# NVlabs/nvbio

Measured on NVIDIA H100. Metric: Mreads/s (150bp) seed+extend, higher is better.
Workload: dtype int32

## Files before the change

### include/nvbio_b200.h

```cpp
#ifndef NVBIO_B200_H
#define NVBIO_B200_H

#include <stddef.h>
#include <stdint.h>

#ifdef __cplusplus
extern "C" {
#endif

#define NVB_VERSION 100

#define NVB_OK              0
#define NVB_E_INVALID      -1
#define NVB_E_TEMP_SIZE    -2
#define NVB_E_CAPACITY     -3
#define NVB_E_UNSUPPORTED  -4

typedef struct nvb_uint2 { uint32_t x, y; } nvb_uint2;

#define NVB_SINK_MIN (-(1 << 30))


typedef struct nvb_fm_index {
    const void*     d_bwt_occ;
    const uint32_t* d_ssa;
    uint32_t        length;
    uint32_t        primary;
    uint32_t        L2[5];
    uint32_t        sa_interval;
    const nvb_uint2* d_ktab;
    uint32_t        ktab_k;
    uint32_t        ktab_located;
    const nvb_uint2* d_rows;
} nvb_fm_index;

typedef struct nvb_string_set {
    const uint32_t* d_words;
    uint32_t        bits;
    uint32_t        big_endian;
    const uint32_t* d_offsets;
    const uint32_t* d_lengths;
    uint32_t        stride;
    uint32_t        length;
} nvb_string_set;

#define NVB_GLOBAL      0
#define NVB_LOCAL       1
#define NVB_SEMI_GLOBAL 2

typedef struct nvb_gotoh_scheme {
    int32_t        match, mismatch;
    int32_t        pattern_gap_open, pattern_gap_ext;
    int32_t        text_gap_open, text_gap_ext;
    const int32_t* d_qual_table;
    int32_t        qual_table_min;
    int32_t        qual_table_max;
} nvb_gotoh_scheme;

int         nvb_version(void);
const char* nvb_error_string(int err);


int nvb_fm_rank(const nvb_fm_index* fmi, const uint32_t* d_k, const uint8_t* d_c, uint32_t n,
                uint32_t* d_out, void* stream);

int nvb_fm_rank4(const nvb_fm_index* fmi, const uint32_t* d_k, uint32_t n, uint32_t* d_out4, void* stream);

int nvb_dict_rank(const void* d_text, uint32_t word_bits, const void* d_occ, uint32_t index_bits, uint32_t K,
                  const void* d_i, const uint8_t* d_c, uint32_t n, void* d_out, void* stream);
int nvb_dict_rank4(const void* d_text, uint32_t word_bits, const void* d_occ, uint32_t index_bits, uint32_t K,
                   const void* d_i, uint32_t n, void* d_out4, void* stream);
int nvb_dict_build_occ(const void* d_text, uint32_t word_bits, uint64_t n_symbols, uint32_t K, uint32_t index_bits, void* d_occ, uint64_t h_counts[4],
                       void* d_temp, size_t* temp_bytes, void* stream);

#define NVB_MATCH_FORWARD_ORDER 1u
#define NVB_MATCH_COMPLEMENT    2u

int nvb_fm_match(const nvb_fm_index* fmi, const nvb_string_set* queries, uint32_t n, uint32_t flags,
                 nvb_uint2* d_ranges, void* stream);

int nvb_fm_match_approx(const nvb_fm_index* fmi, const nvb_string_set* queries, uint32_t n, uint32_t flags,
                        uint32_t exact_len, int find_exact, uint32_t max_out,
                        nvb_uint2* d_ranges, uint32_t* d_counts, uint32_t* d_range_sums, void* stream);

typedef struct nvb_seed_hit {
    uint32_t range_begin;
    uint32_t bits;
} nvb_seed_hit;
#define NVB_MAP_EXACT  0u
#define NVB_MAP_APPROX 1u
#define NVB_MAP_MAX_PUSHES 100u
typedef struct nvb_map_params {
    uint32_t algorithm;
    uint32_t seed_len, seed_freq;
    uint32_t max_hits, max_reseed, rep_seeds, subseed_len, min_read_len;
    uint32_t fw, rc;
} nvb_map_params;
int nvb_map_seeds(const nvb_fm_index* fmi, const nvb_string_set* reads, const uint32_t* d_queue, uint32_t n_queue, uint32_t retry,
                  const nvb_map_params* params, const uint32_t* d_seed_freq,
                  nvb_seed_hit* d_hits, uint32_t* d_counts, uint8_t* d_reseed, uint32_t* d_range_stats, void* stream);

int nvb_fm_locate_init(const nvb_fm_index* fmi, const uint32_t* d_rows, const uint32_t* d_idx, uint32_t n,
                       uint32_t* d_sampled_row, uint32_t* d_steps, void* stream);
int nvb_fm_locate_lookup(const nvb_fm_index* fmi, const uint32_t* d_sampled_row, const uint32_t* d_steps, const uint32_t* d_idx, uint32_t n,
                         uint32_t* d_pos, void* stream);
int nvb_fm_locate_sorted(const nvb_fm_index* fmi, const uint32_t* d_rows, uint32_t n, uint32_t* d_pos,
                         void* d_temp, size_t* temp_bytes, void* stream);

int nvb_fm_locate(const nvb_fm_index* fmi, const uint32_t* d_rows, uint32_t n, uint32_t* d_pos, void* stream);

int nvb_fm_filter_rank(const nvb_fm_index* fmi, const nvb_string_set* queries, uint32_t n, uint32_t flags,
                       nvb_uint2* d_ranges, uint64_t* d_slots, uint64_t* h_n_hits,
                       void* d_temp, size_t* temp_bytes, void* stream);

int nvb_fm_filter_locate(const nvb_fm_index* fmi, const nvb_uint2* d_ranges, const uint64_t* d_slots,
                         uint32_t n_queries, uint64_t begin, uint64_t end, nvb_uint2* d_hits, void* stream);


int nvb_banded_gotoh_score(int band_len, int type, const nvb_gotoh_scheme* scheme,
                           const nvb_string_set* patterns, const uint8_t* d_quals,
                           const nvb_string_set* texts, uint32_t n,
                           int32_t* d_score, nvb_uint2* d_sink,
                           void* d_temp, size_t* temp_bytes, void* stream);

int nvb_banded_gotoh_score_indirect(int band_len, int type, const nvb_gotoh_scheme* scheme,
                           const nvb_string_set* patterns, const uint8_t* d_quals,
                           const nvb_string_set* texts, const uint32_t* d_n, uint32_t n_max,
                           int32_t* d_score, nvb_uint2* d_sink,
                           void* d_temp, size_t* temp_bytes, void* stream);

int nvb_banded_gotoh_score_window(int band_len, int type, const nvb_gotoh_scheme* scheme,
                                  const nvb_string_set* patterns, const uint8_t* d_quals, const nvb_string_set* texts, uint32_t n,
                                  uint32_t window_begin, uint32_t window_end, const int32_t* d_min_score,
                                  int16_t* d_checkpoints, int32_t* d_score, nvb_uint2* d_sink, uint8_t* d_alive, void* stream);

int nvb_banded_gotoh_score_best2(int band_len, int type, const nvb_gotoh_scheme* scheme,
                                 const nvb_string_set* patterns, const uint8_t* d_quals, const nvb_string_set* texts, uint32_t n,
                                 uint32_t distinct_dist, int32_t* d_out6, void* stream);

int nvb_gotoh_score(int type, const nvb_gotoh_scheme* scheme, const nvb_string_set* patterns, const uint8_t* d_quals, const nvb_string_set* texts, uint32_t n,
                    int32_t* d_score, nvb_uint2* d_sink, void* d_temp, size_t* temp_bytes, void* stream);

int nvb_gotoh_score_indirect(int type, const nvb_gotoh_scheme* scheme, const nvb_string_set* patterns, const uint8_t* d_quals, const nvb_string_set* texts,
                             const uint32_t* d_n, uint32_t n_max,
                             int32_t* d_score, nvb_uint2* d_sink, void* d_temp, size_t* temp_bytes, void* stream);

int nvb_gotoh_traceback(int type, const nvb_gotoh_scheme* scheme, const nvb_string_set* patterns, const uint8_t* d_quals, const nvb_string_set* texts, uint32_t n,
                        int32_t* d_score, nvb_uint2* d_sink, nvb_uint2* d_source,
                        uint8_t* d_ops, uint32_t max_ops, uint32_t* d_n_ops,
                        void* d_temp, size_t* temp_bytes, void* stream);

int nvb_banded_gotoh_traceback(int band_len, int type, const nvb_gotoh_scheme* scheme,
                               const nvb_string_set* patterns, const uint8_t* d_quals, const nvb_string_set* texts, uint32_t n,
                               int32_t* d_score, nvb_uint2* d_sink, nvb_uint2* d_source,
                               uint8_t* d_ops, uint32_t max_ops, uint32_t* d_n_ops,
                               void* d_temp, size_t* temp_bytes, void* stream);


int nvb_fm_build_occ(const uint32_t* d_bwt, uint32_t n, void* d_bwt_occ, uint32_t h_L2[5],
                     void* d_temp, size_t* temp_bytes, void* stream);

int nvb_fm_build_bwt(const uint32_t* d_text, uint32_t n, uint32_t* d_bwt, uint32_t* h_primary,
                     uint32_t* d_ssa, uint32_t sa_interval, uint32_t* d_sa,
                     void* d_temp, size_t* temp_bytes, void* stream);

int nvb_fm_build_ktab(const nvb_fm_index* fmi, uint32_t k, nvb_uint2* d_ktab, void* stream);

int nvb_fm_build_ktab_located(const nvb_fm_index* fmi, uint32_t k, void* d_ktab16, void* stream);

int nvb_fm_build_ktab_context(const nvb_fm_index* fmi, uint32_t k, const uint32_t* d_text, void* d_ktab16, void* stream);

int nvb_fm_build_ktab_wide(const nvb_fm_index* fmi, uint32_t k, const uint32_t* d_text, void* d_ktab32, void* stream);

int nvb_fm_build_rows(const nvb_fm_index* fmi, const uint32_t* d_text, nvb_uint2* d_rows, void* stream);

typedef struct nvb_seed_extend_params {
    uint32_t seed_len;
    uint32_t seed_interval;
    uint32_t band_len;
    uint32_t type;
    uint32_t both_strands;
    uint32_t max_seed_hits;
    uint32_t dedup_jobs;
    nvb_gotoh_scheme scheme;
    const uint8_t* d_read_quals;
} nvb_seed_extend_params;

int nvb_seed_extend(const nvb_fm_index* fmi, const uint32_t* d_genome,
                    const nvb_string_set* reads, uint32_t n_reads,
                    const nvb_seed_extend_params* params, uint32_t hit_capacity,
                    int32_t* d_best_score, uint32_t* d_best_pos,
                    uint32_t* d_n_hits, uint32_t* d_hit_read, nvb_uint2* d_hit_window,
                    int32_t* d_hit_score, nvb_uint2* d_hit_sink,
                    void* d_temp, size_t* temp_bytes, void* stream);

typedef struct nvb_best_alignment_out {
    uint8_t*   d_ops;
    uint32_t   max_ops;
    uint32_t*  d_n_ops;
    nvb_uint2* d_begin;
    uint8_t*   d_strand;
} nvb_best_alignment_out;

int nvb_seed_extend_traceback(const nvb_fm_index* fmi, const uint32_t* d_genome,
                    const nvb_string_set* reads, uint32_t n_reads,
                    const nvb_seed_extend_params* params, uint32_t hit_capacity,
                    int32_t* d_best_score, uint32_t* d_best_pos,
                    uint32_t* d_n_hits, uint32_t* d_hit_read, nvb_uint2* d_hit_window,
                    int32_t* d_hit_score, nvb_uint2* d_hit_sink,
                    const nvb_best_alignment_out* best_alignment,
                    void* d_temp, size_t* temp_bytes, void* stream);

typedef struct nvb_mapq_params {
    const int32_t* d_min_score;
    uint32_t       max_read_len;
    int32_t        match_bonus;
} nvb_mapq_params;
typedef struct nvb_mapq_out {
    int32_t*  d_second_score;
    uint32_t* d_second_pos;
    uint8_t*  d_second_strand;
    uint8_t*  d_mapq;
} nvb_mapq_out;

int nvb_seed_extend_mapq(const nvb_fm_index* fmi, const uint32_t* d_genome,
                    const nvb_string_set* reads, uint32_t n_reads,
                    const nvb_seed_extend_params* params, uint32_t hit_capacity,
                    int32_t* d_best_score, uint32_t* d_best_pos,
                    uint32_t* d_n_hits, uint32_t* d_hit_read, nvb_uint2* d_hit_window,
                    int32_t* d_hit_score, nvb_uint2* d_hit_sink,
                    const nvb_best_alignment_out* best_alignment,
                    const nvb_mapq_params* mapq, const nvb_mapq_out* mapq_out,
                    void* d_temp, size_t* temp_bytes, void* stream);

typedef struct nvb_pair_params {
    uint32_t min_frag, max_frag;
    int32_t  min_mate_score;
    uint32_t rescue_capacity;
} nvb_pair_params;
typedef struct nvb_pair_out {
    int32_t*  d_pair_score;
    uint32_t* d_pair_flags;
    int32_t*  d_mate_score;
    uint32_t* d_mate_pos;
    uint8_t*  d_mate_strand;
    uint32_t* d_n_rescue;
} nvb_pair_out;
#define NVB_PAIR_UNPAIRED       0u
#define NVB_PAIR_CONCORDANT     1u
#define NVB_PAIR_RESCUED_MATE1  2u
#define NVB_PAIR_RESCUED_MATE2  4u

int nvb_seed_extend_paired(const nvb_fm_index* fmi, const uint32_t* d_genome,
                    const nvb_string_set* reads, uint32_t n_pairs,
                    const nvb_seed_extend_params* params, uint32_t hit_capacity,
                    const nvb_pair_params* pair_params, const nvb_pair_out* out,
                    uint32_t* d_n_hits, void* d_temp, size_t* temp_bytes, void* stream);

typedef struct nvb_pair_mapq_out {
    int32_t*  d_second_pair_score;
    uint32_t* d_second_mate_pos;
    uint8_t*  d_second_mate_strand;
    int32_t*  d_mate_second_score;
    uint8_t*  d_mate_mapq;
} nvb_pair_mapq_out;

int nvb_seed_extend_paired_mapq(const nvb_fm_index* fmi, const uint32_t* d_genome,
                    const nvb_string_set* reads, uint32_t n_pairs,
                    const nvb_seed_extend_params* params, uint32_t hit_capacity,
                    const nvb_pair_params* pair_params, const nvb_pair_out* out,
                    const nvb_mapq_params* mapq, const nvb_pair_mapq_out* mapq_out,
                    uint32_t* d_n_hits, void* d_temp, size_t* temp_bytes, void* stream);

int nvb_seed_extend_paired_traceback(const nvb_fm_index* fmi, const uint32_t* d_genome,
                    const nvb_string_set* reads, uint32_t n_pairs,
                    const nvb_seed_extend_params* params, uint32_t hit_capacity,
                    const nvb_pair_params* pair_params, const nvb_pair_out* out,
                    const nvb_best_alignment_out* mate_alignment,
                    const nvb_mapq_params* mapq, const nvb_pair_mapq_out* mapq_out,
                    uint32_t* d_n_hits, void* d_temp, size_t* temp_bytes, void* stream);

typedef struct nvb_finish_out {
    uint32_t* d_cigar;
    uint32_t  max_cigar;
    uint32_t* d_n_cigar;
    char*     d_md;
    uint32_t  max_md;
    uint32_t* d_md_len;
    uint32_t* d_edits;
} nvb_finish_out;

int nvb_finish_alignments(const uint32_t* d_genome, uint32_t genome_len,
                          const nvb_string_set* reads, uint32_t n,
                          const nvb_best_alignment_out* alignment,
                          const nvb_finish_out* out, void* stream);

typedef struct nvb_bam_in {
    nvb_string_set   reads;
    const uint8_t*   d_read_quals;
    const uint32_t*  d_n_ops;
    const nvb_uint2* d_begin;
    const uint8_t*   d_strand;
    nvb_finish_out   finish;
    const int32_t*   d_score;
    const uint8_t*   d_mapq;
    const int32_t*   d_second_score;
    const uint32_t*  d_pair_flags;
    const uint32_t*  d_contig_begin;
    uint32_t         n_contigs;
    const char*      d_names;
    const uint32_t*  d_name_offsets;
} nvb_bam_in;
typedef struct nvb_bam_out {
    uint8_t*  d_records;
    uint64_t  capacity;
    uint64_t* d_offsets;
    uint32_t* d_counts;
} nvb_bam_out;

int nvb_bam_records(const nvb_bam_in* in, uint32_t n, const nvb_bam_out* out, void* d_temp, size_t* temp_bytes, void* stream);

typedef struct nvb_bgzf_out {
    uint8_t*  d_out;
    uint64_t  capacity;
    uint64_t* d_block_offsets;
} nvb_bgzf_out;

// ... 32 lines not shown
```

### include/nvbio_b200_debug.h

```cpp
#ifndef NVBIO_B200_DEBUG_H
#define NVBIO_B200_DEBUG_H
#include <stdint.h>
#ifdef __cplusplus
extern "C" {
#endif

void nvb_debug_force_gotoh_path(int path);
int nvb_debug_gotoh_last_route(int* packed, uint32_t* n_int32);
void nvb_debug_full_minb(int minb);
void nvb_debug_full_warp(int mode);
void nvb_debug_full_traceback_warp(int on);
void nvb_debug_pair_format(int on);
void nvb_debug_pair_rows2(int on);
void nvb_debug_traceback_fast(int on);
void nvb_debug_pair_extra_smem(int bytes);

void nvb_debug_pipeline_path(int path);

void nvb_debug_seed_split(int on);

void nvb_debug_perfect_shortcut(int on);
int nvb_debug_dp_jobs(uint32_t* n);

int nvb_debug_mapq_eval(const int32_t* d_best, const uint8_t* d_has_second, const int32_t* d_second, const uint32_t* d_len,
                        const int32_t* d_match_bonus, const int32_t* d_min_score, uint32_t n, uint8_t* d_mapq, void* stream);

void nvb_debug_bgzf_grid(uint32_t ctas);

#ifdef __cplusplus
}
#endif
#endif
```

### nvbio_b200/_lib.py

```python
import ctypes as C
import os

_HERE = os.path.dirname(os.path.abspath(__file__))
LIB_PATH = os.environ.get("NVBIO_B200_LIB") or os.path.join(_HERE, "libnvbio_b200.so")

EXPORTS = [
    "nvb_version", "nvb_error_string",
    "nvb_fm_rank", "nvb_fm_rank4", "nvb_fm_match", "nvb_fm_match_approx", "nvb_fm_locate", "nvb_fm_filter_rank", "nvb_fm_filter_locate",
    "nvb_banded_gotoh_score", "nvb_banded_gotoh_score_indirect", "nvb_banded_gotoh_traceback", "nvb_gotoh_score", "nvb_gotoh_score_indirect", "nvb_banded_gotoh_score_window", "nvb_banded_gotoh_score_best2", "nvb_gotoh_traceback", "nvb_seed_extend_paired",
    "nvb_fm_build_occ", "nvb_fm_build_bwt", "nvb_fm_build_ktab", "nvb_fm_build_ktab_located", "nvb_fm_build_ktab_context", "nvb_fm_build_ktab_wide", "nvb_fm_build_rows", "nvb_seed_extend", "nvb_seed_extend_traceback", "nvb_seed_extend_mapq", "nvb_seed_extend_paired_mapq", "nvb_seed_extend_paired_traceback",
    "nvb_seed_extend_stage_ms",
    "nvb_dict_rank", "nvb_dict_rank4", "nvb_dict_build_occ",
    "nvb_map_seeds", "nvb_fm_locate_init", "nvb_fm_locate_lookup", "nvb_fm_locate_sorted",
    "nvb_pipeline_create", "nvb_pipeline_submit", "nvb_pipeline_wait", "nvb_pipeline_traffic", "nvb_pipeline_destroy",
    "nvb_finish_alignments", "nvb_bam_records", "nvb_bgzf_compress",
]
DEBUG_EXPORTS = [
    "nvb_debug_gotoh_last_route", "nvb_debug_force_gotoh_path", "nvb_debug_full_minb", "nvb_debug_full_warp", "nvb_debug_full_traceback_warp",
    "nvb_debug_pair_format", "nvb_debug_pair_rows2", "nvb_debug_traceback_fast", "nvb_debug_pair_extra_smem",
    "nvb_debug_pipeline_path", "nvb_debug_seed_split", "nvb_debug_perfect_shortcut", "nvb_debug_dp_jobs", "nvb_debug_mapq_eval",
    "nvb_debug_bgzf_grid",
]


class NvbError(RuntimeError):
    pass


class FmIndexStruct(C.Structure):
    _fields_ = [("d_bwt_occ", C.c_void_p), ("d_ssa", C.c_void_p), ("length", C.c_uint32),
                ("primary", C.c_uint32), ("L2", C.c_uint32 * 5), ("sa_interval", C.c_uint32),
                ("d_ktab", C.c_void_p), ("ktab_k", C.c_uint32), ("ktab_located", C.c_uint32), ("d_rows", C.c_void_p)]


class StringSetStruct(C.Structure):
    _fields_ = [("d_words", C.c_void_p), ("bits", C.c_uint32), ("big_endian", C.c_uint32),
                ("d_offsets", C.c_void_p), ("d_lengths", C.c_void_p), ("stride", C.c_uint32),
                ("length", C.c_uint32)]


class GotohSchemeStruct(C.Structure):
    _fields_ = [("match", C.c_int32), ("mismatch", C.c_int32), ("pattern_gap_open", C.c_int32),
                ("pattern_gap_ext", C.c_int32), ("text_gap_open", C.c_int32), ("text_gap_ext", C.c_int32),
                ("d_qual_table", C.c_void_p), ("qual_table_min", C.c_int32), ("qual_table_max", C.c_int32)]


class SeedExtendParamsStruct(C.Structure):
    _fields_ = [("seed_len", C.c_uint32), ("seed_interval", C.c_uint32), ("band_len", C.c_uint32),
                ("type", C.c_uint32), ("both_strands", C.c_uint32), ("max_seed_hits", C.c_uint32),
                ("dedup_jobs", C.c_uint32), ("scheme", GotohSchemeStruct), ("d_read_quals", C.c_void_p)]


class BestAlignmentOutStruct(C.Structure):
    _fields_ = [("d_ops", C.c_void_p), ("max_ops", C.c_uint32), ("d_n_ops", C.c_void_p), ("d_begin", C.c_void_p),
                ("d_strand", C.c_void_p)]


class FinishOutStruct(C.Structure):
    _fields_ = [("d_cigar", C.c_void_p), ("max_cigar", C.c_uint32), ("d_n_cigar", C.c_void_p), ("d_md", C.c_void_p), ("max_md", C.c_uint32),
                ("d_md_len", C.c_void_p), ("d_edits", C.c_void_p)]


class BamInStruct(C.Structure):
    _fields_ = [("reads", StringSetStruct), ("d_read_quals", C.c_void_p), ("d_n_ops", C.c_void_p), ("d_begin", C.c_void_p),
                ("d_strand", C.c_void_p), ("finish", FinishOutStruct), ("d_score", C.c_void_p), ("d_mapq", C.c_void_p),
                ("d_second_score", C.c_void_p), ("d_pair_flags", C.c_void_p), ("d_contig_begin", C.c_void_p), ("n_contigs", C.c_uint32),
                ("d_names", C.c_void_p), ("d_name_offsets", C.c_void_p)]


class BamOutStruct(C.Structure):
    _fields_ = [("d_records", C.c_void_p), ("capacity", C.c_uint64), ("d_offsets", C.c_void_p), ("d_counts", C.c_void_p)]


class BgzfOutStruct(C.Structure):
    _fields_ = [("d_out", C.c_void_p), ("capacity", C.c_uint64), ("d_block_offsets", C.c_void_p)]


class MapqParamsStruct(C.Structure):
    _fields_ = [("d_min_score", C.c_void_p), ("max_read_len", C.c_uint32), ("match_bonus", C.c_int32)]


class MapqOutStruct(C.Structure):
    _fields_ = [("d_second_score", C.c_void_p), ("d_second_pos", C.c_void_p), ("d_second_strand", C.c_void_p), ("d_mapq", C.c_void_p)]


class PairParamsStruct(C.Structure):
    _fields_ = [("min_frag", C.c_uint32), ("max_frag", C.c_uint32), ("min_mate_score", C.c_int32), ("rescue_capacity", C.c_uint32)]


class PairOutStruct(C.Structure):
    _fields_ = [("d_pair_score", C.c_void_p), ("d_pair_flags", C.c_void_p), ("d_mate_score", C.c_void_p), ("d_mate_pos", C.c_void_p),
                ("d_mate_strand", C.c_void_p), ("d_n_rescue", C.c_void_p)]


class PairMapqOutStruct(C.Structure):
    _fields_ = [("d_second_pair_score", C.c_void_p), ("d_second_mate_pos", C.c_void_p), ("d_second_mate_strand", C.c_void_p),
                ("d_mate_second_score", C.c_void_p), ("d_mate_mapq", C.c_void_p)]


class PipelineResultStruct(C.Structure):
    _fields_ = [("best_score", C.c_void_p), ("best_pos", C.c_void_p), ("n_hits", C.c_void_p), ("pair_score", C.c_void_p),
                ("pair_flags", C.c_void_p), ("mate_score", C.c_void_p), ("mate_pos", C.c_void_p), ("mate_strand", C.c_void_p),
                ("n_rescue", C.c_void_p), ("device_ms", C.c_float)]


_lib = None


def lib():
    global _lib
    if _lib is None:
        if not os.path.exists(LIB_PATH):
            raise NvbError("nvbio_b200: %s is missing -- run `python -m nvbio_b200.build` "
                           "(there is no CPU fallback)" % LIB_PATH)
        _lib = C.CDLL(LIB_PATH)
        _lib.nvb_error_string.restype = C.c_char_p
        _lib.nvb_pipeline_destroy.restype = None
        _lib.nvb_pipeline_traffic.restype = None
        for name in EXPORTS + DEBUG_EXPORTS:
            getattr(_lib, name)
    return _lib


def check(err, what=""):
    if err != 0:
        msg = lib().nvb_error_string(C.c_int(err)).decode()
        raise NvbError("%s failed: %s (%d)" % (what or "nvbio_b200 call", msg, err))
```

### nvbio_b200/csrc/fm_core.cuh

```cuda
#pragma once
#include "common.cuh"

namespace nvb {

struct __align__(32) FmBlock {
    uint32_t bwt[4];
    uint32_t occ[4];
};

struct FmIndex {
    const FmBlock*  blocks;
    const uint32_t* ssa;
    const uint2*    ktab;
    uint32_t n, primary;
    uint32_t L2[5];
    uint32_t sa_mask, sa_shift;
    uint32_t ktab_k;
    uint32_t ktab_located;
    const uint2*    rows;
    uint32_t ktab_wide;
    __host__ __device__ __forceinline__ uint32_t l2(uint32_t c) const {
        return (c == 0) ? L2[0] : (c == 1) ? L2[1] : (c == 2) ? L2[2] : L2[3];
    }
    __host__ __device__ __forceinline__ uint32_t count(uint32_t c) const {
        return (c == 0) ? L2[1] - L2[0] : (c == 1) ? L2[2] - L2[1] : (c == 2) ? L2[3] - L2[2] : L2[4] - L2[3];
    }
};

static inline bool valid_fmindex(const nvb_fm_index* f) {
    if (!f || !f->d_bwt_occ) return false;
    const uint32_t I = f->sa_interval;
    if (I != 0 && (I & (I - 1)) != 0) return false;
    if (f->d_ktab && (f->ktab_k < 1 || f->ktab_k > 16 || f->ktab_located > 5u)) return false;
    if (f->d_ktab && f->ktab_located >= 3u && (f->sa_interval != 1u || !f->d_ssa)) return false;
    if (f->d_ktab && f->ktab_located >= 4u && ((uintptr_t)f->d_ktab & 31u)) return false;
    if (f->d_ktab && (f->ktab_located == 3u || f->ktab_located == 5u) && !f->d_rows) return false;
    return true;
}
static inline FmIndex make_fmindex(const nvb_fm_index* f) {
    FmIndex r;
    r.blocks = (const FmBlock*)f->d_bwt_occ; r.ssa = f->d_ssa; r.n = f->length; r.primary = f->primary;
    for (int i = 0; i < 5; ++i) r.L2[i] = f->L2[i];
    const uint32_t I = f->sa_interval ? f->sa_interval : 16u;
    r.sa_shift = 0; while ((1u << r.sa_shift) < I) ++r.sa_shift;
    r.sa_mask = (1u << r.sa_shift) - 1u;
    r.ktab = (const uint2*)f->d_ktab; r.ktab_k = f->d_ktab ? f->ktab_k : 0u;
    const bool with_rows = f->d_ktab && (f->ktab_located == 3u || f->ktab_located == 5u);
    r.ktab_wide = (f->d_ktab && f->ktab_located >= 4u) ? 1u : 0u;
    r.ktab_located = f->d_ktab ? (f->ktab_located >= 2u ? 2u : f->ktab_located) : 0u;
    r.rows = with_rows ? (const uint2*)f->d_rows : nullptr;
    return r;
}

__host__ __device__ __forceinline__ uint32_t nvb_popc(uint32_t x) {
#ifdef __CUDA_ARCH__
    return __popc(x);
#else
    return (uint32_t)__builtin_popcount(x);
#endif
}

#ifndef NVB_FM_LD_QUAL
#define NVB_FM_LD_QUAL ".L2::64B"
#endif
__host__ __device__ __forceinline__ FmBlock load_block(const FmBlock* __restrict__ blocks, uint32_t k) {
#ifdef __CUDA_ARCH__
    FmBlock b;
    asm volatile("ld.global.nc" NVB_FM_LD_QUAL ".v4.u32 {%0,%1,%2,%3}, [%8];\n\t"
                 "ld.global.nc" NVB_FM_LD_QUAL ".v4.u32 {%4,%5,%6,%7}, [%8+16];"
                 : "=r"(b.bwt[0]), "=r"(b.bwt[1]), "=r"(b.bwt[2]), "=r"(b.bwt[3]),
                   "=r"(b.occ[0]), "=r"(b.occ[1]), "=r"(b.occ[2]), "=r"(b.occ[3])
                 : "l"(blocks + k));
    return b;
#else
    return blocks[k];
#endif
}
__host__ __device__ __forceinline__ void load_block_if(FmBlock& b, const FmBlock* __restrict__ blocks, uint32_t k, bool pred) {
#ifdef __CUDA_ARCH__
    asm volatile("{\n\t.reg .pred p;\n\tsetp.ne.u32 p, %9, 0;\n\t"
                 "@p ld.global.nc" NVB_FM_LD_QUAL ".v4.u32 {%0,%1,%2,%3}, [%8];\n\t"
                 "@p ld.global.nc" NVB_FM_LD_QUAL ".v4.u32 {%4,%5,%6,%7}, [%8+16];\n\t}"
                 : "+r"(b.bwt[0]), "+r"(b.bwt[1]), "+r"(b.bwt[2]), "+r"(b.bwt[3]),
                   "+r"(b.occ[0]), "+r"(b.occ[1]), "+r"(b.occ[2]), "+r"(b.occ[3])
                 : "l"(blocks + k), "r"((uint32_t)pred));
#else
    if (pred) b = blocks[k];
#endif
}

__host__ __device__ __forceinline__ uint32_t gather_u32(const uint32_t* __restrict__ p) {
#ifdef __CUDA_ARCH__
    uint32_t v; asm volatile("ld.global.nc" NVB_FM_LD_QUAL ".u32 %0, [%1];" : "=r"(v) : "l"(p)); return v;
#else
    return *p;
#endif
}
__host__ __device__ __forceinline__ uint4 gather_u4(const uint4* __restrict__ p) {
#ifdef __CUDA_ARCH__
    uint4 v; asm volatile("ld.global.nc" NVB_FM_LD_QUAL ".v4.u32 {%0,%1,%2,%3}, [%4];" : "=r"(v.x), "=r"(v.y), "=r"(v.z), "=r"(v.w) : "l"(p)); return v;
#else
    return *p;
#endif
}
__host__ __device__ __forceinline__ uint2 gather_u2(const uint2* __restrict__ p) {
#ifdef __CUDA_ARCH__
    uint2 v; asm volatile("ld.global.nc" NVB_FM_LD_QUAL ".v2.u32 {%0,%1}, [%2];" : "=r"(v.x), "=r"(v.y) : "l"(p)); return v;
#else
    return *p;
#endif
}

__host__ __device__ __forceinline__ uint32_t eq_flags(uint32_t w, uint32_t pat) {
    const uint32_t d = w ^ pat;
    return ~(d | (d >> 1)) & 0x55555555u;
}

__host__ __device__ __forceinline__ uint32_t block_rank(const FmBlock& b, uint32_t r, uint32_t c) {
    const uint32_t pat = c * 0x55555555u;
    const uint32_t nsym = r + 1;
    uint32_t cnt = (c == 0) ? b.occ[0] : (c == 1) ? b.occ[1] : (c == 2) ? b.occ[2] : b.occ[3];
#pragma unroll
    for (int q = 0; q < 4; ++q) {
        const int keep = (int)nsym - 16 * q;
        const uint32_t k = keep < 0 ? 0u : (keep > 16 ? 16u : (uint32_t)keep);
        const uint32_t mask = (uint32_t)(0xFFFFFFFF00000000ull >> (2 * k));
        cnt += nvb_popc(eq_flags(b.bwt[q], pat) & mask);
    }
    return cnt;
}

__host__ __device__ __forceinline__ uint32_t block_symbol(const FmBlock& b, uint32_t r) {
    const uint32_t q = r >> 4;
    const uint32_t w = (q == 0) ? b.bwt[0] : (q == 1) ? b.bwt[1] : (q == 2) ? b.bwt[2] : b.bwt[3];
    return (w >> (30u - 2u * (r & 15u))) & 3u;
}

template <typename W> struct dict_word {};
template <> struct dict_word<uint32_t> { static constexpr uint32_t SPW = 16u; static constexpr uint32_t ODD = 0x55555555u; };
template <> struct dict_word<uint64_t> { static constexpr uint32_t SPW = 32u; static constexpr uint64_t ODD = 0x5555555555555555ull; };

template <typename W>
__host__ __device__ __forceinline__ uint32_t word_rank(W w, uint32_t c, uint32_t keep) {
    constexpr uint32_t SPW = dict_word<W>::SPW;
    const W pat = (W)c * dict_word<W>::ODD;
    const W d = w ^ pat;
    W flags = ~(d | (d >> 1)) & dict_word<W>::ODD;
    flags &= (W)(~(W)0) << (2u * (SPW - keep));
#ifdef __CUDA_ARCH__
    return sizeof(W) == 8 ? (uint32_t)__popcll((unsigned long long)flags) : (uint32_t)__popc((uint32_t)flags);
#else
    return (uint32_t)__builtin_popcountll((unsigned long long)flags);
#endif
}
template <typename W, typename I>
__host__ __device__ __forceinline__ I dict_rank(const W* __restrict__ text, const I* __restrict__ occ, uint32_t K, I i, uint32_t c) {
    if (i == (I)(~(I)0)) return (I)0;
    constexpr uint32_t SPW = dict_word<W>::SPW;
    const uint64_t k = (uint64_t)(i / K);
    const uint32_t r = (uint32_t)(i - (I)(k * K));
    const uint32_t m = r / SPW;
    const uint64_t off = k * (K / SPW);
    I out = occ[k * 4u + c];
    for (uint32_t j = 0; j < m; ++j) out += word_rank<W>(text[off + j], c, SPW);
    return out + word_rank<W>(text[off + m], c, (r % SPW) + 1u);
}

__host__ __device__ __forceinline__ uint32_t fm_rank1(const FmIndex& f, uint32_t k, uint32_t c) {
    if (k == 0xFFFFFFFFu) return 0u;
    if (k == f.n) return f.count(c);
    if (k >= f.primary) --k;
    const FmBlock b = load_block(f.blocks, k >> 6);
    return block_rank(b, k & 63u, c);
}

__host__ __device__ __forceinline__ uint4 fm_rank4(const FmIndex& f, uint32_t k) {
    if (k == 0xFFFFFFFFu) return make_uint4(0u, 0u, 0u, 0u);
    if (k == f.n) return make_uint4(f.count(0), f.count(1), f.count(2), f.count(3));
    if (k >= f.primary) --k;
    const FmBlock b = load_block(f.blocks, k >> 6);
    const uint32_t r = k & 63u;
    return make_uint4(block_rank(b, r, 0), block_rank(b, r, 1), block_rank(b, r, 2), block_rank(b, r, 3));
}

__host__ __device__ __forceinline__ void fm_rank2(const FmIndex& f, uint32_t kx, uint32_t ky, uint32_t c,
                                                  uint32_t& rx, uint32_t& ry) {
    const bool need_x = (kx != 0xFFFFFFFFu) && (kx != f.n);
    const bool need_y = (ky != 0xFFFFFFFFu) && (ky != f.n);
    const uint32_t cnt = f.count(c);
    rx = (kx == f.n) ? cnt : 0u;
    ry = (ky == f.n) ? cnt : 0u;
    const uint32_t ax = kx - (kx >= f.primary ? 1u : 0u);
    const uint32_t ay = ky - (ky >= f.primary ? 1u : 0u);
    if (need_x || need_y) {
        const uint32_t bx = ax >> 6, by = ay >> 6;
        FmBlock b0 = load_block(f.blocks, need_x ? bx : by);
        FmBlock b1 = b0;
        load_block_if(b1, f.blocks, by, need_x && need_y && bx != by);
        const uint32_t tx = block_rank(b0, ax & 63u, c);
        const uint32_t ty = block_rank(b1, ay & 63u, c);
        if (need_x) rx = tx;
        if (need_y) ry = ty;
    }
// ... 165 lines not shown

constexpr uint32_t FM_ROWS_MAX = 8;

enum { FM_EMPTY = 0, FM_RANGE = 1, FM_LOCATED = 2, FM_DEFERRED = 3 };
enum { FM_WHOLE = 0, FM_DEFER = 1, FM_RESUME = 2 };
template <int BITS, bool BE, int MODE = FM_WHOLE>
__host__ __device__ __forceinline__ uint32_t fm_match_locate_one(const FmIndex& f, const uint32_t* __restrict__ genome,
                                                                 const uint32_t* __restrict__ words, uint32_t off, uint32_t len,
                                                                 uint32_t& ox, uint32_t& oy)
{
    SymReader<BITS, BE> rd(words);
    uint32_t x = 0, y = f.n, s = 0;
    uint32_t known_pos = 0u, known_pos2 = 0u, ctx2 = 0u; bool have_pos = false, have_two = false, two_ctx = false;
    uint4 e = make_uint4(0u, 0u, 0u, 0u), e_hi = make_uint4(0u, 0u, 0u, 0u);
    if (MODE == FM_RESUME) { x = ox; y = oy; s = (x == 0u && y == f.n) ? 0u : f.ktab_k; }
    if (MODE != FM_RESUME && f.ktab_k && len >= f.ktab_k) {
        uint32_t u = 0; bool has_n = false;
        if (BITS == 2 && BE) {
            u = be2_window(words, off + len - f.ktab_k, f.ktab_k) >> (32u - 2u * f.ktab_k);
        } else if (BITS == 4 && BE) {
            u = be4_window(words, off + len - f.ktab_k, f.ktab_k, has_n) >> (32u - 2u * f.ktab_k);
        } else {
            for (uint32_t j = 0; j < f.ktab_k; ++j) {
                const uint32_t c = rd.get(off + len - 1u - j);
                has_n |= (c > 3u);
                u |= (c & 3u) << (2u * j);
            }
        }
        if (!has_n) {
            if (f.ktab_located) {
                gather_ktab_entry(f, u, e, e_hi);
                x = e.x; y = e.y; known_pos = e.z; known_pos2 = e.w;
                if (ktab_two_row_marker(f, y)) { ctx2 = y; y = x + 1u; two_ctx = true; }
                have_pos = (x == y); have_two = (y == x + 1u);
            } else {
                const uint2 r = gather_u2(f.ktab + u);
                x = r.x; y = r.y;
            }
            s = f.ktab_k;
        }
    }
    const bool full_sa = (f.sa_shift == 0u) && genome != nullptr;
    auto prefix_matches = [&](const uint32_t pos, const uint32_t rem) -> bool {
        if (pos == 0xFFFFFFFFu || pos < rem) return false;
        const uint32_t p0 = pos - rem;
        bool same = true;
        if (BITS == 2 && BE) {
            for (uint32_t i = 0; i < rem; i += 16u) {
                const uint32_t cnt = rem - i < 16u ? rem - i : 16u;
                same &= ((be2_window(words, off + i, cnt) ^ be2_window(genome, p0 + i, cnt)) >> (32u - 2u * cnt)) == 0u;
            }
        } else if (BITS == 4 && BE) {
            bool n_left = false;
            for (uint32_t i = 0; i < rem; i += 16u) {
                const uint32_t cnt = rem - i < 16u ? rem - i : 16u;
                same &= ((be4_window(words, off + i, cnt, n_left) ^ be2_window(genome, p0 + i, cnt)) >> (32u - 2u * cnt)) == 0u;
            }
            same &= !n_left;
        } else {
            SymReader<2, true> tr(genome);
            for (uint32_t i = 0; i < rem; ++i) same &= (rd.get(off + i) == tr.get(p0 + i));
        }
        return same;
    };
    if (have_two && full_sa && s < len) {
        const uint32_t rem = len - s;
        bool m0, m1;
        if (two_ctx && rem <= 7u) {
            bool n_left = false;
            const uint32_t qw = unread_context<BITS, BE>(words, off, rem, n_left);
            m0 = !n_left && context_matches(qw, ctx2, known_pos, rem);
            m1 = !n_left && context_matches(qw, ctx2 >> 14, known_pos2, rem);
        } else {
            m0 = prefix_matches(known_pos, rem); m1 = prefix_matches(known_pos2, rem);
        }
        if (!m0 && !m1) return FM_EMPTY;
        if (m0 != m1) { ox = (m0 ? known_pos : known_pos2) - rem; oy = 0xFFFFFFFFu; return FM_LOCATED; }
    }
    if (MODE != FM_RESUME && f.ktab_wide && full_sa && s == f.ktab_k && s < len && y - x >= 2u && y - x < KTAB_WIDE_ROWS) {
        const uint32_t rem = len - s, cnt = rem < 16u ? rem : 16u;
        const bool three = (y - x == 2u);
        const uint32_t width = three ? 16u : 8u, wc = cnt < width ? cnt : width;
        bool n_left = false;
        const uint32_t qw = unread_context<BITS, BE>(words, off + rem - cnt, cnt, n_left);
        if (!n_left) {
            uint32_t full = 0u, near = 0u, hit = 0u;
#pragma unroll
            for (uint32_t i = 0; i < KTAB_WIDE_ROWS; ++i) {
                if (i > y - x) continue;
                const uint32_t c = ktab_wide_context(e, e_hi, three, i);
                if (context_equal(qw, c, wc)) { ++full; hit = i; }
                near += context_equal(qw, c, wc - 1u) ? 1u : 0u;
            }
            if (full == 0u) return FM_EMPTY;
            if (full == 1u && near == 1u && y - x <= 3u && rem <= width) {
                const uint32_t pos = ktab_wide_sa(e, e_hi, three, hit);
                if (pos == 0xFFFFFFFFu || pos < rem) return FM_EMPTY;
                ox = pos - rem; oy = 0xFFFFFFFFu;
                return FM_LOCATED;
            }
        }
    }
    if (MODE != FM_DEFER && f.rows && full_sa && s == f.ktab_k && s < len && y - x >= 2u && y - x < FM_ROWS_MAX && len - s <= 16u) {
        const uint32_t rem = len - s;
        bool n_left = false;
        const uint32_t qw = unread_context<BITS, BE>(words, off, rem, n_left);
        if (!n_left) {
            const uint32_t* ctx = (const uint32_t*)(f.rows + x) + 1;
            uint32_t c[FM_ROWS_MAX];
#pragma unroll
            for (uint32_t i = 0; i < FM_ROWS_MAX; ++i) c[i] = (i <= y - x) ? gather_u32(ctx + 2u * i) : 0u;
            uint32_t full = 0u, near = 0u, hit = 0u;
#pragma unroll
            for (uint32_t i = 0; i < FM_ROWS_MAX; ++i) {
                if (i > y - x) continue;
                if (context_equal(qw, c[i], rem)) { ++full; hit = i; }
                near += context_equal(qw, c[i], rem - 1u) ? 1u : 0u;
            }
            if (full == 0u) return FM_EMPTY;
            if (full == 1u && near == 1u) {
                const uint32_t pos = gather_u32((const uint32_t*)(f.rows + x + hit));
                if (pos == 0xFFFFFFFFu || pos < rem) return FM_EMPTY;
                ox = pos - rem; oy = 0xFFFFFFFFu;
                return FM_LOCATED;
            }
        }
    }
    if (MODE == FM_DEFER && s < len && x < y) { ox = x; oy = y; return FM_DEFERRED; }
    for (; s < len && x <= y; ++s) {
        if (full_sa && x == y) {
            const uint32_t rem = len - s;
            const uint32_t pos = have_pos ? known_pos : gather_u32(f.ssa + x);
            if (have_pos && f.ktab_located == 2u && rem <= 16u) {
                bool n_left = false;
                const uint32_t qw = unread_context<BITS, BE>(words, off, rem, n_left);
                if (n_left || !context_matches(qw, known_pos2, pos, rem)) return FM_EMPTY;
                ox = pos - rem; oy = 0xFFFFFFFFu;
                return FM_LOCATED;
            }
            if (!prefix_matches(pos, rem)) return FM_EMPTY;
            ox = pos - rem; oy = 0xFFFFFFFFu;
            return FM_LOCATED;
        }
        if (MODE == FM_DEFER) { ox = x; oy = y; return FM_DEFERRED; }
        const uint32_t c = rd.get(off + len - 1u - s);
        if (c > 3u) return FM_EMPTY;
        fm_step(f, c, x, y);
    }
    if (x > y) return FM_EMPTY;
    ox = x; oy = y;
    return FM_RANGE;
}

template <int BITS, bool BE>
__host__ __device__ inline uint32_t fm_map_approx_one(const FmIndex& f, const uint32_t* __restrict__ words,
                                                      uint32_t off, uint32_t len2, uint32_t len1, uint32_t flags, bool find_exact,
                                                      uint2* __restrict__ out, uint32_t max_out, uint32_t& range_sum)
{
    const bool fwd = (flags & NVB_MATCH_FORWARD_ORDER) != 0;
    const bool comp = (flags & NVB_MATCH_COMPLEMENT) != 0;
    SymReader<BITS, BE> rd(words);
    auto sym = [&](uint32_t i) -> uint32_t {
        const uint32_t c = rd.get(off + (fwd ? i : (len2 - 1u - i)));
        return (comp && c < 4u) ? 3u - c : c;
    };
    range_sum = 0;
    uint32_t n_out = 0;
    if (len1 > len2) len1 = len2;
    uint32_t n_pos = 0, n_cnt = 0;
    for (uint32_t i = 0; i < len2; ++i) {
        if (sym(i) > 3u) {
            if (i < len1 || n_cnt) return 0u;
            n_pos = i; ++n_cnt;
        }
    }
    if (n_cnt) len1 = n_pos;

    uint32_t bx = 0, by = f.n;
    for (uint32_t i = 0; i < len1 && bx <= by; ++i) fm_step(f, sym(i), bx, by);

    for (uint32_t i = len1; i < len2 && bx <= by; ++i) {
        const uint32_t c = sym(i);
        const uint4 lo = fm_rank4(f, bx - 1u), hi = fm_rank4(f, by);
        const uint32_t los[4] = { lo.x, lo.y, lo.z, lo.w }, his[4] = { hi.x, hi.y, hi.z, hi.w };
#pragma unroll
        for (uint32_t sub = 0; sub < 4; ++sub) {
            if (sub != c && his[sub] > los[sub]) {
                uint32_t x = f.l2(sub) + los[sub] + 1u, y = f.l2(sub) + his[sub];
                for (uint32_t k = i + 1u; k < len2 && x <= y; ++k) {
                    const uint32_t ck = sym(k);
                    if (ck > 3u) { x = 1u; y = 0u; break; }
                    fm_step(f, ck, x, y);
                }
                if (x <= y) {
                    if (n_out < max_out) out[n_out] = make_uint2(x, y);
                    ++n_out; range_sum += y - x + 1u;
                }
            }
        }
        if (c < 4u) { bx = f.l2(c) + los[c] + 1u; by = f.l2(c) + his[c]; }
        else { bx = 1u; by = 0u; break; }
    }
    if (find_exact && bx <= by) {
        if (n_out < max_out) out[n_out] = make_uint2(bx, by);
        ++n_out; range_sum += by - bx + 1u;
    }
    return n_out;
}

__host__ __device__ __forceinline__ uint32_t fm_locate_one(const FmIndex& f, uint32_t row) {
    uint32_t j = row, t = 0;
    while ((j & f.sa_mask) != 0u) {
        if (j != f.primary) {
            const uint32_t k = j < f.primary ? j : j - 1u;
            const FmBlock b = load_block(f.blocks, k >> 6);
            const uint32_t c = block_symbol(b, k & 63u);
            j = f.l2(c) + block_rank(b, k & 63u, c);
        } else {
            j = 0u;
        }
        ++t;
    }
    return gather_u32(f.ssa + (j >> f.sa_shift)) + t;
}

}
```

### nvbio_b200/csrc/fm_kernels.cu

```cuda
#include "fm_core.cuh"
#include <cub/device/device_scan.cuh>
#include <cub/iterator/transform_input_iterator.cuh>

namespace nvb {

constexpr int FM_BLOCKDIM = 128;

__global__ void __launch_bounds__(FM_BLOCKDIM)
fm_rank_kernel(const FmIndex f, const uint32_t* __restrict__ k, const uint8_t* __restrict__ c, uint32_t n,
               uint32_t* __restrict__ out)
{
    const uint32_t i = blockIdx.x * FM_BLOCKDIM + threadIdx.x;
    if (i >= n) return;
    out[i] = fm_rank1(f, k[i], c[i] & 3u);
}

__global__ void __launch_bounds__(FM_BLOCKDIM)
fm_rank4_kernel(const FmIndex f, const uint32_t* __restrict__ k, uint32_t n, uint4* __restrict__ out)
{
    const uint32_t i = blockIdx.x * FM_BLOCKDIM + threadIdx.x;
    if (i >= n) return;
    out[i] = fm_rank4(f, k[i]);
}

template <int BITS, bool BE>
__global__ void __launch_bounds__(FM_BLOCKDIM)
fm_match_kernel(const FmIndex f, const StrSet q, uint32_t n, uint32_t flags, uint2* __restrict__ out)
{
    const uint32_t i = blockIdx.x * FM_BLOCKDIM + threadIdx.x;
    if (i >= n) return;
    uint32_t x, y;
    fm_match_one<BITS, BE>(f, q.words, str_off(q, i), str_len(q, i), flags, x, y);
    out[i] = make_uint2(x, y);
}

template <int BITS, bool BE>
__global__ void __launch_bounds__(FM_BLOCKDIM)
fm_match_approx_kernel(const FmIndex f, const StrSet q, uint32_t n, uint32_t flags, uint32_t exact_len, bool find_exact, uint32_t max_out,
                       uint2* __restrict__ out, uint32_t* __restrict__ counts, uint32_t* __restrict__ sums)
{
    const uint32_t i = blockIdx.x * FM_BLOCKDIM + threadIdx.x;
    if (i >= n) return;
    uint32_t sum = 0;
    const uint32_t cnt = fm_map_approx_one<BITS, BE>(f, q.words, str_off(q, i), str_len(q, i), exact_len, flags, find_exact,
                                                     out + (size_t)i * max_out, max_out, sum);
    counts[i] = cnt;
    if (sums) sums[i] = sum;
}

__global__ void __launch_bounds__(FM_BLOCKDIM)
fm_locate_kernel(const FmIndex f, const uint32_t* __restrict__ rows, uint32_t n, uint32_t* __restrict__ out)
{
    const uint32_t i = blockIdx.x * FM_BLOCKDIM + threadIdx.x;
    if (i >= n) return;
    out[i] = fm_locate_one(f, rows[i]);
}

template <typename W, typename I>
__global__ void __launch_bounds__(FM_BLOCKDIM)
dict_rank_kernel(const W* __restrict__ text, const I* __restrict__ occ, uint32_t K, const I* __restrict__ idx, const uint8_t* __restrict__ c, uint32_t n,
                 I* __restrict__ out, int all4)
{
    const uint32_t t = blockIdx.x * FM_BLOCKDIM + threadIdx.x;
    if (t >= n) return;
    if (all4) { for (uint32_t s = 0; s < 4u; ++s) out[4u * (size_t)t + s] = dict_rank<W, I>(text, occ, K, idx[t], s); }
    else out[t] = dict_rank<W, I>(text, occ, K, idx[t], c[t] & 3u);
}

template <typename W, typename I>
__global__ void __launch_bounds__(256)
dict_block_counts_kernel(const W* __restrict__ text, uint64_t n_symbols, uint32_t K, uint64_t n_blocks, uint64_t lane_len, I* __restrict__ counts )
{
    const uint64_t k = (uint64_t)blockIdx.x * 256 + threadIdx.x;
    if (k > n_blocks) return;
    I cnt[4] = { 0, 0, 0, 0 };
    if (k < n_blocks) {
        constexpr uint32_t SPW = dict_word<W>::SPW;
        const uint64_t first = k * K;
        const uint64_t valid = (n_symbols - first) < K ? (n_symbols - first) : K;
        for (uint32_t j = 0; j * SPW < valid; ++j) {
            const uint32_t keep = (valid - (uint64_t)j * SPW) < SPW ? (uint32_t)(valid - (uint64_t)j * SPW) : SPW;
            const W w = text[k * (K / SPW) + j];
            for (uint32_t s = 0; s < 4u; ++s) cnt[s] += word_rank<W>(w, s, keep);
        }
    }
    for (uint32_t s = 0; s < 4u; ++s) counts[s * lane_len + k] = cnt[s];
}
template <typename I>
__global__ void __launch_bounds__(256)
dict_interleave_occ_kernel(const I* __restrict__ scan, uint64_t n_blocks, uint64_t lane_len, I* __restrict__ occ)
{
    const uint64_t k = (uint64_t)blockIdx.x * 256 + threadIdx.x;
    if (k >= n_blocks) return;
    for (uint32_t c = 0; c < 4u; ++c) occ[4u * k + c] = scan[c * lane_len + k];
}

__global__ void __launch_bounds__(FM_BLOCKDIM)
fm_ktab_level_kernel(const FmIndex f, uint2* __restrict__ tab, uint32_t prev_entries)
{
    const uint32_t v = blockIdx.x * FM_BLOCKDIM + threadIdx.x;
    if (v >= prev_entries) return;
    const uint2 r = tab[v];
#pragma unroll
    for (int c = 3; c >= 0; --c) {
        uint32_t x = r.x, y = r.y;
        if (x <= y) fm_step(f, (uint32_t)c, x, y);
        tab[(uint32_t)c * prev_entries + v] = make_uint2(x, y);
    }
}

template <uint32_t STRIDE>
__global__ void __launch_bounds__(FM_BLOCKDIM)
fm_ktab16_level_kernel(const FmIndex f, uint4* __restrict__ tab, uint32_t prev_entries)
{
    const uint32_t v = blockIdx.x * FM_BLOCKDIM + threadIdx.x;
    if (v >= prev_entries) return;
    const uint4 r = tab[(size_t)v * STRIDE];
#pragma unroll
    for (int c = 3; c >= 0; --c) {
        uint32_t x = r.x, y = r.y;
        if (x <= y) fm_step(f, (uint32_t)c, x, y);
        tab[((size_t)c * prev_entries + v) * STRIDE] = make_uint4(x, y, 0u, 0u);
    }
}
__global__ void __launch_bounds__(FM_BLOCKDIM)
fm_ktab16_locate_kernel(const FmIndex f, uint4* __restrict__ tab, uint64_t entries)
{
    const uint64_t v = (uint64_t)blockIdx.x * FM_BLOCKDIM + threadIdx.x;
    if (v >= entries) return;
    const uint4 e = tab[v];
    if (e.x == e.y)           tab[v].z = f.ssa[e.x];
    else if (e.y == e.x + 1u) { tab[v].z = f.ssa[e.x]; tab[v].w = f.ssa[e.y]; }
}

__global__ void __launch_bounds__(FM_BLOCKDIM)
fm_ktab16_context_kernel(const uint32_t* __restrict__ text, uint4* __restrict__ tab, uint64_t entries, uint32_t n_rows)
{
    const uint64_t v = (uint64_t)blockIdx.x * FM_BLOCKDIM + threadIdx.x;
    if (v >= entries) return;
    const uint4 e = tab[v];
    if (e.x == e.y) tab[v].w = text_before(text, e.z, 16u);
    else if (e.y == e.x + 1u && n_rows < KTAB_TWO_ROW_MARK)
        tab[v].y = KTAB_TWO_ROW_MARK | text_before(text, e.z, 7u) | (text_before(text, e.w, 7u) << 14);
}

__global__ void __launch_bounds__(FM_BLOCKDIM)
fm_rows_kernel(const uint32_t* __restrict__ sa, const uint32_t* __restrict__ text, uint2* __restrict__ rows, uint64_t n_rows)
{
    const uint64_t r = (uint64_t)blockIdx.x * FM_BLOCKDIM + threadIdx.x;
    if (r >= n_rows) return;
    const uint32_t pos = sa[r];
    rows[r] = make_uint2(pos, text_before(text, pos, 16u));
}

__global__ void __launch_bounds__(FM_BLOCKDIM)
fm_ktab32_fill_kernel(const uint32_t* __restrict__ sa, const uint32_t* __restrict__ text, uint4* __restrict__ tab, uint64_t entries, uint32_t n)
{
    const uint64_t v = (uint64_t)blockIdx.x * FM_BLOCKDIM + threadIdx.x;
    if (v >= entries) return;
    const uint4 e = tab[2u * v];
    uint32_t w[8];
    ktab_wide_fill(sa, text, n, e.x, e.y, w);
    tab[2u * v] = make_uint4(w[0], w[1], w[2], w[3]);
    tab[2u * v + 1u] = make_uint4(w[4], w[5], w[6], w[7]);
}

struct RangeSize {
    __host__ __device__ __forceinline__ uint64_t operator()(const uint2& r) const { return (uint64_t)(uint32_t)(1u + r.y - r.x); }
};

__device__ __forceinline__ uint32_t upper_bound_u64(const uint64_t* __restrict__ a, uint32_t n, uint64_t v)
{
    uint32_t lo = 0, hi = n;
    while (lo < hi) {
        const uint32_t mid = (lo + hi) >> 1;
        if (a[mid] <= v) lo = mid + 1; else hi = mid;
    }
    return lo;
}

__global__ void __launch_bounds__(FM_BLOCKDIM)
fm_filter_locate_kernel(const FmIndex f, const uint2* __restrict__ ranges, const uint64_t* __restrict__ slots,
                        uint32_t n_queries, uint64_t begin, uint64_t count, uint2* __restrict__ hits)
{
    const uint64_t t = (uint64_t)blockIdx.x * FM_BLOCKDIM + threadIdx.x;
    if (t >= count) return;
    const uint64_t h = begin + t;
    const uint32_t slot = upper_bound_u64(slots, n_queries, h);
    if (slot >= n_queries) { hits[t] = make_uint2(0xFFFFFFFFu, 0xFFFFFFFFu); return; }
    const uint64_t base = slot ? slots[slot - 1] : 0ull;
    const uint32_t row = ranges[slot].x + (uint32_t)(h - base);
    hits[t] = make_uint2(fm_locate_one(f, row), slot);
}

struct U4Add { __host__ __device__ __forceinline__ uint4 operator()(const uint4& a, const uint4& b) const {
    return make_uint4(a.x + b.x, a.y + b.y, a.z + b.z, a.w + b.w); } };

__global__ void __launch_bounds__(256)
occ_block_counts_kernel(const uint32_t* __restrict__ bwt, uint32_t n, uint32_t n_blocks, uint4* __restrict__ counts)
{
    const uint32_t k = blockIdx.x * 256 + threadIdx.x;
    if (k >= n_blocks) return;
    const uint4 w = reinterpret_cast<const uint4*>(bwt)[k];
    const uint32_t ws[4] = { w.x, w.y, w.z, w.w };
    const uint32_t valid = (n - k * 64u) < 64u ? (n - k * 64u) : 64u;
    uint32_t cnt[4] = { 0, 0, 0, 0 };
#pragma unroll
    for (int q = 0; q < 4; ++q) {
        const int keep = (int)valid - 16 * q;
        const uint32_t kk = keep < 0 ? 0u : (keep > 16 ? 16u : (uint32_t)keep);
        const uint32_t mask = (uint32_t)(0xFFFFFFFF00000000ull >> (2 * kk));
#pragma unroll
        for (uint32_t c = 0; c < 4; ++c) cnt[c] += __popc(eq_flags(ws[q], c * 0x55555555u) & mask);
    }
    counts[k] = make_uint4(cnt[0], cnt[1], cnt[2], cnt[3]);
}

__global__ void __launch_bounds__(256)
occ_interleave_kernel(const uint32_t* __restrict__ bwt, const uint4* __restrict__ occ_excl, uint32_t n, uint32_t n_blocks,
                      FmBlock* __restrict__ out)
{
    const uint32_t k = blockIdx.x * 256 + threadIdx.x;
    if (k >= n_blocks) return;
    uint4 w = reinterpret_cast<const uint4*>(bwt)[k];
    const uint32_t valid = (n - k * 64u) < 64u ? (n - k * 64u) : 64u;
    uint32_t ws[4] = { w.x, w.y, w.z, w.w };
#pragma unroll
    for (int q = 0; q < 4; ++q) {
        const int keep = (int)valid - 16 * q;
        const uint32_t kk = keep < 0 ? 0u : (keep > 16 ? 16u : (uint32_t)keep);
        ws[q] &= (uint32_t)(0xFFFFFFFF00000000ull >> (2 * kk));
    }
    const uint4 o = occ_excl[k];
    FmBlock b;
    b.bwt[0] = ws[0]; b.bwt[1] = ws[1]; b.bwt[2] = ws[2]; b.bwt[3] = ws[3];
    b.occ[0] = o.x; b.occ[1] = o.y; b.occ[2] = o.z; b.occ[3] = o.w;
    out[k] = b;
}

template <typename W, typename I>
static int dict_rank_launch(const void* text, const void* occ, uint32_t K, const void* idx, const uint8_t* c, uint32_t n, void* out, int all4, cudaStream_t s)
{
    dict_rank_kernel<W, I><<<(n + FM_BLOCKDIM - 1) / FM_BLOCKDIM, FM_BLOCKDIM, 0, s>>>((const W*)text, (const I*)occ, K, (const I*)idx, c, n, (I*)out, all4);
    NVB_LAUNCH_CHECK();
    return NVB_OK;
}
template <typename W, typename I>
static int dict_build_occ_impl(const void* d_text, uint64_t n_symbols, uint32_t K, void* d_occ, uint64_t h_counts[4], void* d_temp, size_t* temp_bytes, cudaStream_t s)
{
    const uint64_t n_blocks = (n_symbols + K - 1) / K;
    const uint64_t lane_len = n_blocks + 1;
    TempCarver tc(d_temp);
    I* counts = tc.take<I>(4 * lane_len);
    I* scan   = tc.take<I>(4 * lane_len);
    size_t scan_bytes = 0;
    NVB_CUDA_TRY(cub::DeviceScan::ExclusiveSum(nullptr, scan_bytes, counts, scan, (long long)lane_len, s));
    char* scan_tmp = tc.take<char>(scan_bytes);
    const size_t need = tc.total();
    if (!d_temp || *temp_bytes < need) { *temp_bytes = need; return NVB_E_TEMP_SIZE; }
    const uint32_t grid = (uint32_t)((lane_len + 255) / 256);
    dict_block_counts_kernel<W, I><<<grid, 256, 0, s>>>((const W*)d_text, n_symbols, K, n_blocks, lane_len, counts);
    NVB_LAUNCH_CHECK();
    for (uint32_t c = 0; c < 4u; ++c)
        NVB_CUDA_TRY(cub::DeviceScan::ExclusiveSum(scan_tmp, scan_bytes, counts + c * lane_len, scan + c * lane_len, (long long)lane_len, s));
    dict_interleave_occ_kernel<I><<<grid, 256, 0, s>>>(scan, n_blocks, lane_len, (I*)d_occ);
    NVB_LAUNCH_CHECK();
    if (h_counts) {
        for (int c = 0; c < 4; ++c) {
            I tot;
            NVB_CUDA_TRY(cudaMemcpyAsync(&tot, scan + c * lane_len + n_blocks, sizeof(I), cudaMemcpyDeviceToHost, s));
            NVB_CUDA_TRY(cudaStreamSynchronize(s));
            h_counts[c] = (uint64_t)tot;
        }
    }
    return NVB_OK;
}

}

using namespace nvb;

extern "C" {

int nvb_version(void) { return NVB_VERSION; }

const char* nvb_error_string(int err)
{
    switch (err) {
    case NVB_OK:            return "success";
    case NVB_E_INVALID:     return "nvbio_b200: invalid argument";
    case NVB_E_TEMP_SIZE:   return "nvbio_b200: temp storage missing or too small";
    case NVB_E_CAPACITY:    return "nvbio_b200: output capacity exceeded";
    case NVB_E_UNSUPPORTED: return "nvbio_b200: unsupported configuration";
    }
    return err > 0 ? cudaGetErrorString((cudaError_t)err) : "nvbio_b200: unknown error";
}

int nvb_fm_build_ktab(const nvb_fm_index* fmi, uint32_t k, nvb_uint2* d_ktab, void* stream)
{
    if (!valid_fmindex(fmi) || k < 1 || k > 16 || !d_ktab) return NVB_E_INVALID;
    nvb_fm_index plain = *fmi; plain.d_ktab = nullptr; plain.ktab_k = 0; plain.ktab_located = 0;
    const FmIndex f = make_fmindex(&plain);
    cudaStream_t s = as_stream(stream);
    const uint2 root = make_uint2(0u, fmi->length);
    NVB_CUDA_TRY(cudaMemcpyAsync(d_ktab, &root, sizeof(uint2), cudaMemcpyHostToDevice, s));
    NVB_CUDA_TRY(cudaStreamSynchronize(s));
    uint32_t prev = 1;
    for (uint32_t t = 1; t <= k; ++t, prev *= 4u) {
        fm_ktab_level_kernel<<<(prev + FM_BLOCKDIM - 1) / FM_BLOCKDIM, FM_BLOCKDIM, 0, s>>>(f, (uint2*)d_ktab, prev);
        NVB_LAUNCH_CHECK();
    }
    return NVB_OK;
}

int nvb_fm_build_ktab_located(const nvb_fm_index* fmi, uint32_t k, void* d_ktab16, void* stream)
{
    if (!valid_fmindex(fmi) || k < 1 || k > 16 || !d_ktab16 || ((uintptr_t)d_ktab16 & 15u)) return NVB_E_INVALID;
    if (fmi->sa_interval != 1u || !fmi->d_ssa) return NVB_E_UNSUPPORTED;
    nvb_fm_index plain = *fmi; plain.d_ktab = nullptr; plain.ktab_k = 0; plain.ktab_located = 0;
    const FmIndex f = make_fmindex(&plain);
    cudaStream_t s = as_stream(stream);
    const uint4 root = make_uint4(0u, fmi->length, 0u, 0u);
    NVB_CUDA_TRY(cudaMemcpyAsync(d_ktab16, &root, sizeof(uint4), cudaMemcpyHostToDevice, s));
    NVB_CUDA_TRY(cudaStreamSynchronize(s));
    uint32_t prev = 1;
    for (uint32_t t = 1; t <= k; ++t, prev *= 4u) {
        fm_ktab16_level_kernel<1><<<(prev + FM_BLOCKDIM - 1) / FM_BLOCKDIM, FM_BLOCKDIM, 0, s>>>(f, (uint4*)d_ktab16, prev);
        NVB_LAUNCH_CHECK();
    }
    const uint64_t entries = 1ull << (2u * k);
    fm_ktab16_locate_kernel<<<(uint32_t)((entries + FM_BLOCKDIM - 1) / FM_BLOCKDIM), FM_BLOCKDIM, 0, s>>>(f, (uint4*)d_ktab16, entries);
    NVB_LAUNCH_CHECK();
    return NVB_OK;
}

int nvb_fm_build_ktab_context(const nvb_fm_index* fmi, uint32_t k, const uint32_t* d_text, void* d_ktab16, void* stream)
{
    if (!d_text) return NVB_E_INVALID;
    const int r = nvb_fm_build_ktab_located(fmi, k, d_ktab16, stream);
    if (r != NVB_OK) return r;
    const uint64_t entries = 1ull << (2u * k);
    fm_ktab16_context_kernel<<<(uint32_t)((entries + FM_BLOCKDIM - 1) / FM_BLOCKDIM), FM_BLOCKDIM, 0, as_stream(stream)>>>(d_text, (uint4*)d_ktab16, entries, fmi->length);
    NVB_LAUNCH_CHECK();
    return NVB_OK;
}

int nvb_fm_build_ktab_wide(const nvb_fm_index* fmi, uint32_t k, const uint32_t* d_text, void* d_ktab32, void* stream)
{
    if (!valid_fmindex(fmi) || k < 1 || k > 16 || !d_text || !d_ktab32 || ((uintptr_t)d_ktab32 & 31u)) return NVB_E_INVALID;
    if (fmi->sa_interval != 1u || !fmi->d_ssa) return NVB_E_UNSUPPORTED;
    nvb_fm_index plain = *fmi; plain.d_ktab = nullptr; plain.ktab_k = 0; plain.ktab_located = 0;
    const FmIndex f = make_fmindex(&plain);
    cudaStream_t s = as_stream(stream);
    const uint4 root = make_uint4(0u, fmi->length, 0u, 0u);
    NVB_CUDA_TRY(cudaMemcpyAsync(d_ktab32, &root, sizeof(uint4), cudaMemcpyHostToDevice, s));
    NVB_CUDA_TRY(cudaStreamSynchronize(s));
    uint32_t prev = 1;
    for (uint32_t t = 1; t <= k; ++t, prev *= 4u) {
        fm_ktab16_level_kernel<2><<<(prev + FM_BLOCKDIM - 1) / FM_BLOCKDIM, FM_BLOCKDIM, 0, s>>>(f, (uint4*)d_ktab32, prev);
        NVB_LAUNCH_CHECK();
    }
    const uint64_t entries = 1ull << (2u * k);
    fm_ktab32_fill_kernel<<<(uint32_t)((entries + FM_BLOCKDIM - 1) / FM_BLOCKDIM), FM_BLOCKDIM, 0, s>>>(fmi->d_ssa, d_text, (uint4*)d_ktab32, entries, fmi->length);
    NVB_LAUNCH_CHECK();
    return NVB_OK;
}

int nvb_fm_build_rows(const nvb_fm_index* fmi, const uint32_t* d_text, nvb_uint2* d_rows, void* stream)
{
    if (!fmi || !fmi->d_bwt_occ || !d_text || !d_rows || ((uintptr_t)d_rows & 7u)) return NVB_E_INVALID;
    if (fmi->sa_interval != 1u || !fmi->d_ssa) return NVB_E_UNSUPPORTED;
    const uint64_t n_rows = (uint64_t)fmi->length + 1u;
    fm_rows_kernel<<<(uint32_t)((n_rows + FM_BLOCKDIM - 1) / FM_BLOCKDIM), FM_BLOCKDIM, 0, as_stream(stream)>>>(fmi->d_ssa, d_text, (uint2*)d_rows, n_rows);
    NVB_LAUNCH_CHECK();
    return NVB_OK;
}

int nvb_fm_rank(const nvb_fm_index* fmi, const uint32_t* d_k, const uint8_t* d_c, uint32_t n,
                uint32_t* d_out, void* stream)
{
    if (!valid_fmindex(fmi) || (n && (!d_k || !d_c || !d_out))) return NVB_E_INVALID;
    if (n == 0) return NVB_OK;
    fm_rank_kernel<<<(n + FM_BLOCKDIM - 1) / FM_BLOCKDIM, FM_BLOCKDIM, 0, as_stream(stream)>>>(make_fmindex(fmi), d_k, d_c, n, d_out);
    NVB_LAUNCH_CHECK();
    return NVB_OK;
}

int nvb_fm_rank4(const nvb_fm_index* fmi, const uint32_t* d_k, uint32_t n, uint32_t* d_out4, void* stream)
{
    if (!valid_fmindex(fmi) || (n && (!d_k || !d_out4))) return NVB_E_INVALID;
    if (n == 0) return NVB_OK;
    fm_rank4_kernel<<<(n + FM_BLOCKDIM - 1) / FM_BLOCKDIM, FM_BLOCKDIM, 0, as_stream(stream)>>>(make_fmindex(fmi), d_k, n, (uint4*)d_out4);
    NVB_LAUNCH_CHECK();
    return NVB_OK;
}

int nvb_fm_match(const nvb_fm_index* fmi, const nvb_string_set* queries, uint32_t n, uint32_t flags,
                 nvb_uint2* d_ranges, void* stream)
{
    if (!valid_fmindex(fmi) || !valid_strset(queries) || (n && !d_ranges)) return NVB_E_INVALID;
    if (n == 0) return NVB_OK;
    const FmIndex f = make_fmindex(fmi);
    const StrSet q = make_strset(queries);
    const uint32_t grid = (n + FM_BLOCKDIM - 1) / FM_BLOCKDIM;
#define CALL(B, E) fm_match_kernel<B, E><<<grid, FM_BLOCKDIM, 0, as_stream(stream)>>>(f, q, n, flags, (uint2*)d_ranges)
    NVB_DISPATCH_STREAM(q.bits, q.big_endian, CALL);
#undef CALL
    NVB_LAUNCH_CHECK();
    return NVB_OK;
}

int nvb_fm_match_approx(const nvb_fm_index* fmi, const nvb_string_set* queries, uint32_t n, uint32_t flags,
                        uint32_t exact_len, int find_exact, uint32_t max_out,
                        nvb_uint2* d_ranges, uint32_t* d_counts, uint32_t* d_range_sums, void* stream)
{
    if (!valid_fmindex(fmi) || !valid_strset(queries) || max_out == 0 || (n && (!d_ranges || !d_counts))) return NVB_E_INVALID;
    if (n == 0) return NVB_OK;
    nvb_fm_index plain = *fmi; plain.d_ktab = nullptr; plain.ktab_k = 0;
    const FmIndex f = make_fmindex(&plain);
    const StrSet q = make_strset(queries);
    const uint32_t grid = (n + FM_BLOCKDIM - 1) / FM_BLOCKDIM;
#define CALL(B, E) fm_match_approx_kernel<B, E><<<grid, FM_BLOCKDIM, 0, as_stream(stream)>>>(f, q, n, flags, exact_len, find_exact != 0, max_out, \
                                                                                           (uint2*)d_ranges, d_counts, d_range_sums)
    NVB_DISPATCH_STREAM(q.bits, q.big_endian, CALL);
#undef CALL
    NVB_LAUNCH_CHECK();
    return NVB_OK;
}

int nvb_fm_locate(const nvb_fm_index* fmi, const uint32_t* d_rows, uint32_t n, uint32_t* d_pos, void* stream)
{
    if (!valid_fmindex(fmi) || !fmi->d_ssa || (n && (!d_rows || !d_pos))) return NVB_E_INVALID;
    if (n == 0) return NVB_OK;
    fm_locate_kernel<<<(n + FM_BLOCKDIM - 1) / FM_BLOCKDIM, FM_BLOCKDIM, 0, as_stream(stream)>>>(make_fmindex(fmi), d_rows, n, d_pos);
    NVB_LAUNCH_CHECK();
    return NVB_OK;
}

int nvb_fm_filter_rank(const nvb_fm_index* fmi, const nvb_string_set* queries, uint32_t n, uint32_t flags,
                       nvb_uint2* d_ranges, uint64_t* d_slots, uint64_t* h_n_hits,
                       void* d_temp, size_t* temp_bytes, void* stream)
{
    if (!temp_bytes || (n && (!d_ranges || !d_slots))) return NVB_E_INVALID;
    if (h_n_hits) *h_n_hits = 0;
    if (n == 0) { *temp_bytes = 0; return NVB_OK; }
    cub::TransformInputIterator<uint64_t, RangeSize, const uint2*> sizes((const uint2*)d_ranges, RangeSize());
    size_t need = 0;
    NVB_CUDA_TRY(cub::DeviceScan::InclusiveSum(nullptr, need, sizes, d_slots, (int)n, as_stream(stream)));
    if (!d_temp || *temp_bytes < need) { *temp_bytes = need; return NVB_E_TEMP_SIZE; }
    const int r = nvb_fm_match(fmi, queries, n, flags, d_ranges, stream);
    if (r != NVB_OK) return r;
    NVB_CUDA_TRY(cub::DeviceScan::InclusiveSum(d_temp, need, sizes, d_slots, (int)n, as_stream(stream)));
    if (h_n_hits) {
        NVB_CUDA_TRY(cudaMemcpyAsync(h_n_hits, d_slots + (n - 1), sizeof(uint64_t), cudaMemcpyDeviceToHost, as_stream(stream)));
        NVB_CUDA_TRY(cudaStreamSynchronize(as_stream(stream)));
    }
    return NVB_OK;
}

int nvb_fm_filter_locate(const nvb_fm_index* fmi, const nvb_uint2* d_ranges, const uint64_t* d_slots,
                         uint32_t n_queries, uint64_t begin, uint64_t end, nvb_uint2* d_hits, void* stream)
{
    if (!valid_fmindex(fmi) || !fmi->d_ssa || !d_ranges || !d_slots || end < begin) return NVB_E_INVALID;
    const uint64_t count = end - begin;
    if (count == 0) return NVB_OK;
    if (!d_hits || count > 0x7FFFFFFFull * FM_BLOCKDIM) return NVB_E_INVALID;
    const uint32_t grid = (uint32_t)((count + FM_BLOCKDIM - 1) / FM_BLOCKDIM);
    fm_filter_locate_kernel<<<grid, FM_BLOCKDIM, 0, as_stream(stream)>>>(make_fmindex(fmi), (const uint2*)d_ranges, d_slots,
                                                                        n_queries, begin, count, (uint2*)d_hits);
    NVB_LAUNCH_CHECK();
    return NVB_OK;
}

static bool dict_args_ok(uint32_t word_bits, uint32_t index_bits, uint32_t K)
{
    if (!(word_bits == 32 || word_bits == 64) || !(index_bits == 32 || index_bits == 64)) return false;
    return K != 0 && K % (word_bits / 2u) == 0;
}
int nvb_dict_rank(const void* d_text, uint32_t word_bits, const void* d_occ, uint32_t index_bits, uint32_t K,
                  const void* d_i, const uint8_t* d_c, uint32_t n, void* d_out, void* stream)
{
    if (!dict_args_ok(word_bits, index_bits, K) || (n && (!d_text || !d_occ || !d_i || !d_c || !d_out))) return NVB_E_INVALID;
    if (n == 0) return NVB_OK;
    cudaStream_t s = as_stream(stream);
    if (word_bits == 32) return index_bits == 32 ? dict_rank_launch<uint32_t, uint32_t>(d_text, d_occ, K, d_i, d_c, n, d_out, 0, s)
                                                 : dict_rank_launch<uint32_t, uint64_t>(d_text, d_occ, K, d_i, d_c, n, d_out, 0, s);
    return index_bits == 32 ? dict_rank_launch<uint64_t, uint32_t>(d_text, d_occ, K, d_i, d_c, n, d_out, 0, s)
                            : dict_rank_launch<uint64_t, uint64_t>(d_text, d_occ, K, d_i, d_c, n, d_out, 0, s);
}
int nvb_dict_rank4(const void* d_text, uint32_t word_bits, const void* d_occ, uint32_t index_bits, uint32_t K,
                   const void* d_i, uint32_t n, void* d_out4, void* stream)
{
    if (!dict_args_ok(word_bits, index_bits, K) || (n && (!d_text || !d_occ || !d_i || !d_out4))) return NVB_E_INVALID;
    if (n == 0) return NVB_OK;
    cudaStream_t s = as_stream(stream);
    if (word_bits == 32) return index_bits == 32 ? dict_rank_launch<uint32_t, uint32_t>(d_text, d_occ, K, d_i, nullptr, n, d_out4, 1, s)
                                                 : dict_rank_launch<uint32_t, uint64_t>(d_text, d_occ, K, d_i, nullptr, n, d_out4, 1, s);
    return index_bits == 32 ? dict_rank_launch<uint64_t, uint32_t>(d_text, d_occ, K, d_i, nullptr, n, d_out4, 1, s)
                            : dict_rank_launch<uint64_t, uint64_t>(d_text, d_occ, K, d_i, nullptr, n, d_out4, 1, s);
}

int nvb_dict_build_occ(const void* d_text, uint32_t word_bits, uint64_t n_symbols, uint32_t K, uint32_t index_bits, void* d_occ, uint64_t h_counts[4],
                       void* d_temp, size_t* temp_bytes, void* stream)
{
    if (!dict_args_ok(word_bits, index_bits, K) || !temp_bytes || (n_symbols && (!d_text || !d_occ))) return NVB_E_INVALID;
    cudaStream_t s = as_stream(stream);
    if (word_bits == 32) return index_bits == 32 ? dict_build_occ_impl<uint32_t, uint32_t>(d_text, n_symbols, K, d_occ, h_counts, d_temp, temp_bytes, s)
                                                 : dict_build_occ_impl<uint32_t, uint64_t>(d_text, n_symbols, K, d_occ, h_counts, d_temp, temp_bytes, s);
    return index_bits == 32 ? dict_build_occ_impl<uint64_t, uint32_t>(d_text, n_symbols, K, d_occ, h_counts, d_temp, temp_bytes, s)
                            : dict_build_occ_impl<uint64_t, uint64_t>(d_text, n_symbols, K, d_occ, h_counts, d_temp, temp_bytes, s);
}

int nvb_fm_build_occ(const uint32_t* d_bwt, uint32_t n, void* d_bwt_occ, uint32_t h_L2[5],
                     void* d_temp, size_t* temp_bytes, void* stream)
{
    if (!temp_bytes || !h_L2 || (n && (!d_bwt || !d_bwt_occ))) return NVB_E_INVALID;
    const uint32_t n_blocks = (n + 63u) / 64u;
    TempCarver tc(d_temp);
    uint4* counts = tc.take<uint4>(n_blocks + 1);
    uint4* excl   = tc.take<uint4>(n_blocks + 1);
    size_t scan_bytes = 0;
    NVB_CUDA_TRY(cub::DeviceScan::ExclusiveScan(nullptr, scan_bytes, counts, excl, U4Add(), make_uint4(0, 0, 0, 0), (int)(n_blocks + 1), as_stream(stream)));
    char* scan_tmp = tc.take<char>(scan_bytes);
    const size_t need = tc.total();
    if (!d_temp || *temp_bytes < need) { *temp_bytes = need; return NVB_E_TEMP_SIZE; }
    cudaStream_t s = as_stream(stream);
    NVB_CUDA_TRY(cudaMemsetAsync(counts + n_blocks, 0, sizeof(uint4), s));
    if (n_blocks) {
        occ_block_counts_kernel<<<(n_blocks + 255) / 256, 256, 0, s>>>(d_bwt, n, n_blocks, counts);
        NVB_LAUNCH_CHECK();
// ... 15 lines not shown
```

### nvbio_b200/csrc/pipeline.cu

```cuda
#include "fm_core.cuh"
#include "gotoh_core.cuh"
#include "pipeline_core.cuh"
#include "gotoh_full_core.cuh"
#include <cub/agent/single_pass_scan_operators.cuh>
#include <cub/block/block_scan.cuh>
#include <cub/device/device_scan.cuh>
#include <cub/device/device_segmented_sort.cuh>
#include <mutex>

namespace nvb {

struct PipeGeom {
    uint32_t n_reads;
    uint32_t n_strings;
    uint32_t strands;
    uint32_t stride;
    uint32_t bits;
    uint32_t seeds_per_string;
    uint32_t seed_len, seed_interval;
    uint32_t band;
    uint32_t max_seed_hits;
    uint32_t genome_len;
};

template <int BITS>
__global__ void __launch_bounds__(256)
pipe_make_strings_kernel(const StrSet reads, const PipeGeom g, uint32_t* __restrict__ out_words, uint32_t* __restrict__ out_len)
{
    constexpr uint32_t SPW = 32 / BITS;
    const uint32_t words_per_string = g.stride / SPW;
    const uint64_t t = (uint64_t)blockIdx.x * 256 + threadIdx.x;
    if (t >= (uint64_t)g.n_strings * words_per_string) return;
    const uint32_t s = (uint32_t)(t / words_per_string), w = (uint32_t)(t % words_per_string);
    const uint32_t read = s / g.strands, strand = s % g.strands;
    const uint32_t off = str_off(reads, read), len = str_len(reads, read);
    if (w == 0) out_len[s] = len;
    uint32_t word = 0;
    for (uint32_t k = 0; k < SPW; ++k) {
        const uint32_t p = w * SPW + k;
        uint32_t c = 0;
        if (p < len) {
            if (strand == 0) c = sym_at_rt(reads.words, reads.bits, reads.big_endian, off + p);
            else { c = sym_at_rt(reads.words, reads.bits, reads.big_endian, off + (len - 1u - p)); c = (c < 4u) ? 3u - c : c; }
        }
        word |= c << (32u - BITS - BITS * k);
    }
    out_words[t] = word;
}

__global__ void __launch_bounds__(256)
pipe_make_quals_kernel(const StrSet reads, const PipeGeom g, const uint8_t* __restrict__ quals, uint8_t* __restrict__ out)
{
    const uint64_t t = (uint64_t)blockIdx.x * 256 + threadIdx.x;
    if (t >= (uint64_t)g.n_strings * g.stride) return;
    const uint32_t s = (uint32_t)(t / g.stride), p = (uint32_t)(t % g.stride);
    const uint32_t read = s / g.strands, strand = s % g.strands;
    const uint32_t off = str_off(reads, read), len = str_len(reads, read);
    out[t] = (p < len) ? quals[off + (strand == 0 ? p : len - 1u - p)] : (uint8_t)0;
}

__device__ __forceinline__ uint32_t load16_2bit_be(const uint32_t* __restrict__ words, uint32_t p , uint32_t cnt )
{
    const uint32_t w = p >> 4, sh = 2u * (p & 15u);
    const uint32_t a = words[w];
    if (sh == 0) return a;
    const uint32_t b = ((p & 15u) + cnt > 16u) ? words[w + 1] : 0u;
    return (a << sh) | (b >> (32u - sh));
}
__device__ __forceinline__ uint32_t revcomp16_2bit(uint32_t x)
{
    uint32_t y = __brev(~x);
    return ((y >> 1) & 0x55555555u) | ((y & 0x55555555u) << 1);
}
__global__ void __launch_bounds__(256)
pipe_make_strings_2bit_be_kernel(const StrSet reads, const PipeGeom g, uint32_t* __restrict__ out_words, uint32_t* __restrict__ out_len)
{
    const uint32_t words_per_string = g.stride / 16u;
    const uint64_t t = (uint64_t)blockIdx.x * 256 + threadIdx.x, total = (uint64_t)g.n_strings * words_per_string;
    if (t >= total) return;
    uint32_t s, w;
    if (total <= 0xFFFFFFFFull) { s = (uint32_t)t / words_per_string; w = (uint32_t)t - s * words_per_string; }
    else                        { s = (uint32_t)(t / words_per_string); w = (uint32_t)(t % words_per_string); }
    const uint32_t read = s / g.strands, strand = s % g.strands;
    const uint32_t off = str_off(reads, read), len = str_len(reads, read);
    if (w == 0) out_len[s] = len;
    const uint32_t first = w * 16u;
    uint32_t word = 0;
    if (first < len) {
        const uint32_t cnt = (len - first) < 16u ? (len - first) : 16u;
        if (strand == 0) {
            word = load16_2bit_be(reads.words, off + first, cnt);
        } else {
            const uint32_t lo = len - first - cnt;
            uint32_t x = load16_2bit_be(reads.words, off + lo, cnt);
            x = revcomp16_2bit(x);
            word = x << (2u * (16u - cnt));
        }
        if (cnt < 16u) word &= ~(0xFFFFFFFFu >> (2u * cnt));
    }
    out_words[t] = word;
}

__device__ __forceinline__ uint32_t seed_range_hits(uint2 range, uint32_t max_seed_hits)
{
    const uint32_t sz = (range.y == 0xFFFFFFFFu) ? 1u : ((range.x <= range.y) ? (range.y - range.x + 1u) : 0u);
    return sz < max_seed_hits ? sz : max_seed_hits;
}

__device__ __forceinline__ uint2 hit_window(uint32_t pos, uint32_t seed_begin, uint32_t len, const PipeGeom& g)
{
    const uint32_t diag = pos > seed_begin ? pos - seed_begin : 0u;
    const uint32_t gb = diag > g.band / 2u ? diag - g.band / 2u : 0u;
    const uint64_t ge64 = (uint64_t)gb + len + g.band;
    return make_uint2(gb, ge64 < g.genome_len ? (uint32_t)ge64 : g.genome_len);
}

__device__ __forceinline__ unsigned long long make_best_key(int32_t score, uint32_t index)
{
    return ((unsigned long long)((uint32_t)score ^ 0x80000000u) << 32) | (unsigned long long)(0xFFFFFFFFu - index);
}
__device__ __forceinline__ int32_t  best_key_score(unsigned long long key) { return (int32_t)((uint32_t)(key >> 32) ^ 0x80000000u); }
__device__ __forceinline__ uint32_t best_key_index(unsigned long long key) { return 0xFFFFFFFFu - (uint32_t)(key & 0xFFFFFFFFull); }

__device__ __forceinline__ bool job_aligned(uint2 sink) { return sink.x != 0xFFFFFFFFu; }

constexpr uint32_t SEED_BLOCK = 128;
constexpr uint32_t SEED_TODO_LISTS = 64;
constexpr uint32_t SEED_TODO_PITCH = 32;
constexpr uint32_t SEED_ITER = 8;
template <int BITS, bool DEFER>
__global__ void __launch_bounds__(SEED_BLOCK, 2048 / SEED_BLOCK)
pipe_seed_match_kernel(const FmIndex f, const PipeGeom g, const uint32_t* __restrict__ words, const uint32_t* __restrict__ slen,
                       const uint32_t* __restrict__ genome, uint2* __restrict__ ranges, uint32_t* __restrict__ sizes,
                       uint32_t* __restrict__ todo, uint32_t* __restrict__ todo_count)
{
    constexpr uint32_t ITER = DEFER ? SEED_ITER : 1u;
#pragma unroll 1
    for (uint32_t it = 0; it < ITER; ++it) {
        const uint32_t q = (blockIdx.x * ITER + it) * SEED_BLOCK + threadIdx.x;
        const bool live = q < g.n_strings * g.seeds_per_string;
        if (!DEFER && !live) return;
        uint32_t x = 1, y = 0;
        bool deferred = false;
        if (live) {
            const uint32_t s = q / g.seeds_per_string, k = q % g.seeds_per_string;
            const uint32_t len = slen[s];
            const uint32_t pos = k * g.seed_interval;
            if (pos + g.seed_len <= len) {
                if (genome) {
                    const uint32_t st = fm_match_locate_one<BITS, true, DEFER ? FM_DEFER : FM_WHOLE>(f, genome, words, s * g.stride + pos, g.seed_len, x, y);
                    if (st == FM_EMPTY) { x = 1; y = 0; }
                    deferred = DEFER && st == FM_DEFERRED;
                } else
                    fm_match_one<BITS, true>(f, words, s * g.stride + pos, g.seed_len, 0u, x, y);
            }
            ranges[q] = make_uint2(x, y);
            if (sizes && !deferred) sizes[q] = seed_range_hits(make_uint2(x, y), g.max_seed_hits);
        }
        if (DEFER) {
            const uint32_t m = __ballot_sync(0xFFFFFFFFu, deferred);
            if (m) {
                const uint32_t lane = threadIdx.x & 31u, list = blockIdx.x % SEED_TODO_LISTS;
                const uint32_t cap = ((gridDim.x + SEED_TODO_LISTS - 1u) / SEED_TODO_LISTS) * SEED_BLOCK * SEED_ITER;
                uint32_t base = 0;
                if (lane == 0) base = atomicAdd(todo_count + list * SEED_TODO_PITCH, (uint32_t)__popc(m));
                base = __shfl_sync(0xFFFFFFFFu, base, 0);
                if (deferred) todo[(size_t)list * cap + base + __popc(m & ((1u << lane) - 1u))] = q;
            }
        }
    }
}
template <int BITS>
__global__ void __launch_bounds__(SEED_BLOCK, 2048 / SEED_BLOCK)
pipe_seed_match_wide_kernel(const FmIndex f, const PipeGeom g, const uint32_t* __restrict__ words,
                            const uint32_t* __restrict__ genome, uint2* __restrict__ ranges, uint32_t* __restrict__ sizes,
                            const uint32_t* __restrict__ todo, const uint32_t* __restrict__ todo_count, const uint32_t seed_grid)
{
    const uint32_t list = blockIdx.x % SEED_TODO_LISTS, per_list = gridDim.x / SEED_TODO_LISTS;
    const uint32_t cap = ((seed_grid + SEED_TODO_LISTS - 1u) / SEED_TODO_LISTS) * SEED_BLOCK * SEED_ITER;
    const uint32_t n = todo_count[list * SEED_TODO_PITCH];
    for (uint32_t t = (blockIdx.x / SEED_TODO_LISTS) * SEED_BLOCK + threadIdx.x; t < n; t += per_list * SEED_BLOCK) {
        const uint32_t q = todo[(size_t)list * cap + t];
        const uint32_t s = q / g.seeds_per_string, k = q % g.seeds_per_string;
        const uint2 r = ranges[q];
        uint32_t x = r.x, y = r.y;
        if (fm_match_locate_one<BITS, true, FM_RESUME>(f, genome, words, s * g.stride + k * g.seed_interval, g.seed_len, x, y) == FM_EMPTY) { x = 1; y = 0; }
        ranges[q] = make_uint2(x, y);
        if (sizes) sizes[q] = seed_range_hits(make_uint2(x, y), g.max_seed_hits);
    }
}

__device__ __forceinline__ uint32_t upper_bound_u32(const uint32_t* __restrict__ a, uint32_t n, uint32_t v)
{
    uint32_t lo = 0, hi = n;
    while (lo < hi) { const uint32_t mid = (lo + hi) >> 1; if (a[mid] <= v) lo = mid + 1; else hi = mid; }
    return lo;
}

__global__ void pipe_count_kernel(const uint32_t* __restrict__ excl, const uint32_t* __restrict__ sizes, uint32_t n_queries, uint32_t capacity,
                                  uint32_t* __restrict__ counts)
{
    if (threadIdx.x == 0 && blockIdx.x == 0) {
        const uint32_t total = n_queries ? excl[n_queries - 1] + sizes[n_queries - 1] : 0u;
        counts[1] = total;
        counts[0] = total < capacity ? total : capacity;
    }
}

__global__ void __launch_bounds__(256)
pipe_expand_hits_kernel(const FmIndex f, const PipeGeom g, const uint2* __restrict__ ranges, const uint32_t* __restrict__ sizes,
                        const uint32_t* __restrict__ excl, const uint32_t* __restrict__ slen, const uint32_t* __restrict__ counts,
                        uint32_t* __restrict__ hit_string, uint32_t* __restrict__ p_off, uint32_t* __restrict__ p_len,
                        uint32_t* __restrict__ t_off, uint32_t* __restrict__ t_len)
{
    const uint32_t q = blockIdx.x * 256 + threadIdx.x;
    if (q >= g.n_strings * g.seeds_per_string) return;
    const uint32_t sz = sizes[q];
    if (sz == 0) return;
    const uint32_t base = excl[q], kept = counts[0];
    const uint32_t x = ranges[q].x;
    const uint32_t s = q / g.seeds_per_string, k = q % g.seeds_per_string;
    const uint32_t seed_begin = k * g.seed_interval;
    const uint32_t len = slen[s];
    for (uint32_t j = 0; j < sz; ++j) {
        const uint32_t h = base + j;
        if (h >= kept) break;
        const uint2 w = hit_window(fm_locate_one(f, x + j), seed_begin, len, g);
        hit_string[h] = s;
        p_off[h] = s * g.stride; p_len[h] = len;
        t_off[h] = w.x;          t_len[h] = w.y - w.x;
    }
}

struct Jobs { uint32_t *p_off, *p_len, *t_off, *t_len; };

constexpr uint32_t RJ_BLOCK = 128;
constexpr uint32_t RJ_STAGE = 640;
constexpr int      RJ_LOCAL = 6;
constexpr uint32_t RJ_CLAIMED = 0xFFFFFFFFu, RJ_CLAIMED_EMPTY = 0xFFFFFFFEu;
using RjTileState = cub::ScanTileState<uint32_t>;
using RjPrefixOp  = cub::TilePrefixCallbackOp<uint32_t, ::cuda::std::plus<uint32_t>, RjTileState>;

__global__ void __launch_bounds__(256)
pipe_resolve_init_kernel(RjTileState tiles, const uint32_t n_tiles, uint32_t* __restrict__ counts, uint32_t* __restrict__ dp_count)
{
    tiles.InitializeStatus((int)n_tiles);
    if (blockIdx.x == 0 && threadIdx.x == 0) { counts[2] = 0u; counts[3] = 0u; *dp_count = 0u; }
}

__global__ void __launch_bounds__(RJ_BLOCK, 8)
pipe_resolve_reads_kernel(const FmIndex f, const PipeGeom g, const uint2* __restrict__ ranges, const uint32_t* __restrict__ slen,
                          const uint32_t hit_capacity, RjTileState tiles, const uint32_t n_tiles, uint32_t* __restrict__ counts,
                          const int shortcut, const int32_t match, const int32_t mismatch, const int32_t max_gap_open,
                          const uint32_t* __restrict__ str_words, const uint32_t* __restrict__ genome,
                          uint32_t* __restrict__ j_string, uint32_t* __restrict__ j_first, const Jobs jobs,
                          int32_t* __restrict__ job_score, uint2* __restrict__ job_sink,
                          const Jobs dp, uint32_t* __restrict__ dp_job, uint32_t* __restrict__ dp_count,
                          unsigned long long* __restrict__ best_key, int32_t* best_score, uint32_t* best_pos, uint8_t* __restrict__ best_strand)
{
    using BlockScan = cub::BlockScan<uint32_t, RJ_BLOCK>;
    __shared__ struct { typename RjPrefixOp::TempStorage prefix; typename BlockScan::TempStorage scan; } s_tmp;
    __shared__ uint32_t st_string[RJ_STAGE], st_first[RJ_STAGE], st_toff[RJ_STAGE], st_tlen[RJ_STAGE], st_slot[RJ_STAGE];
    __shared__ unsigned long long s_key[RJ_BLOCK];
    __shared__ int32_t s_score[RJ_BLOCK];
    __shared__ uint32_t s_pos[RJ_BLOCK];
    __shared__ uint8_t s_strand[RJ_BLOCK];
    __shared__ uint32_t s_tile, s_cnt, s_base, s_dp_cnt, s_dp_base;
    if (threadIdx.x == 0) { s_tile = atomicAdd(counts + 3, 1u); s_cnt = 0u; s_dp_cnt = 0u; }
    s_key[threadIdx.x] = 0ull;
    __syncthreads();
    const uint32_t tile = s_tile, r0 = tile * RJ_BLOCK, r = r0 + threadIdx.x;
    const uint32_t per_read = g.strands * g.seeds_per_string;
    const bool live = r < g.n_reads;
    const uint2* rr = ranges + (size_t)r * per_read;

    uint32_t hits = 0, run = 0;
    if (live)
        for (uint32_t q = 0; q < per_read; ++q) hits += seed_range_hits(rr[q], g.max_seed_hits);
    if (tile == 0) {
        uint32_t aggregate;
        BlockScan(s_tmp.scan).ExclusiveSum(hits, run, aggregate);
        if (threadIdx.x == 0) tiles.SetInclusive(0, aggregate);
    } else {
        RjPrefixOp prefix(tiles, s_tmp.prefix, ::cuda::std::plus<uint32_t>{}, (int)tile);
        BlockScan(s_tmp.scan).ExclusiveSum(hits, run, prefix);
    }
    if (tile == n_tiles - 1u && threadIdx.x == RJ_BLOCK - 1u) {
        const uint32_t total = run + hits;
        counts[1] = total;
        counts[0] = total < hit_capacity ? total : hit_capacity;
    }

    if (live) {
        uint32_t lk_s[RJ_LOCAL], lk_b[RJ_LOCAL], lk_e[RJ_LOCAL];
        int n_local = 0;
        for (uint32_t strand = 0; strand < g.strands; ++strand) {
            const uint32_t s = r * g.strands + strand;
            const uint32_t len = slen[s];
            for (uint32_t k = 0; k < g.seeds_per_string; ++k) {
                const uint2 rq = rr[strand * g.seeds_per_string + k];
                const bool located = rq.y == 0xFFFFFFFFu;
                const uint32_t sz = seed_range_hits(rq, g.max_seed_hits);
                if (sz == 0u) continue;
                const uint32_t base = run, x = rq.x, seed_begin = k * g.seed_interval;
                run += sz;
                for (uint32_t j = 0; j < sz; ++j) {
                    const uint32_t h = base + j;
                    if (h >= hit_capacity) break;
                    const uint2 w = hit_window(located ? x : fm_locate_one(f, x + j), seed_begin, len, g);
                    bool seen = false;
#pragma unroll
                    for (int e = 0; e < RJ_LOCAL; ++e) seen |= (e < n_local) && lk_s[e] == s && lk_b[e] == w.x && lk_e[e] == w.y;
                    if (seen) continue;
#pragma unroll
                    for (int e = 0; e < RJ_LOCAL; ++e) if (e == n_local) { lk_s[e] = s; lk_b[e] = w.x; lk_e[e] = w.y; }
                    if (n_local < RJ_LOCAL) ++n_local;
                    const uint32_t slot = atomicAdd(&s_cnt, 1u);
                    if (slot < RJ_STAGE) { st_string[slot] = s; st_first[slot] = h; st_toff[slot] = w.x; st_tlen[slot] = w.y - w.x; }
                    else {
                        const uint32_t o = atomicAdd(counts + 2, 1u), d = atomicAdd(dp_count, 1u);
                        j_string[o] = s; j_first[o] = h;
                        jobs.p_off[o] = s * g.stride; jobs.p_len[o] = len; jobs.t_off[o] = w.x; jobs.t_len[o] = w.y - w.x;
                        dp.p_off[d] = s * g.stride; dp.p_len[d] = len; dp.t_off[d] = w.x; dp.t_len[d] = w.y - w.x; dp_job[d] = o;
                    }
// ... 410 lines not shown
    const uint32_t f = pair_flags[p];
    if (!pair_rescued(f)) return;
    const uint32_t r = (f == NVB_PAIR_RESCUED_MATE1 ? 0u : n_pairs) + p;
    bp_len[r] = 0; bt_len[r] = 0;
}

__global__ void __launch_bounds__(256)
pair_rescue_items_kernel(const uint32_t n_pairs, const uint32_t* __restrict__ pair_flags, const uint32_t* __restrict__ job_idx,
                         const uint8_t* __restrict__ mate_strand, uint2* __restrict__ items, uint32_t* __restrict__ n_items, uint8_t* __restrict__ ba_strand)
{
    const uint32_t p = blockIdx.x * 256 + threadIdx.x, lane = threadIdx.x & 31u;
    const uint32_t f = p < n_pairs ? pair_flags[p] : 0u;
    const bool rescued = pair_rescued(f);
    const uint32_t m = __ballot_sync(0xFFFFFFFFu, rescued);
    if (!m) return;
    uint32_t base = 0;
    if (lane == 0) base = atomicAdd(n_items, (uint32_t)__popc(m));
    base = __shfl_sync(0xFFFFFFFFu, base, 0);
    if (!rescued) return;
    const uint32_t o = f == NVB_PAIR_RESCUED_MATE1 ? 0u : 1u, out = o * n_pairs + p;
    items[base + __popc(m & ((1u << lane) - 1u))] = make_uint2(job_idx[2u * p + (1u - o)], out);
    if (ba_strand) ba_strand[out] = mate_strand[out];
}


__global__ void __launch_bounds__(256)
pair_cand_scatter_kernel(const PipeGeom g, const uint32_t* __restrict__ count, const uint32_t* __restrict__ c_string,
                         const uint32_t* __restrict__ t_off, const int32_t* __restrict__ score, const uint2* __restrict__ sink,
                         const uint32_t* __restrict__ str_len, const int32_t* __restrict__ min_score, const uint32_t* __restrict__ seg,
                         uint32_t* __restrict__ cursor, unsigned long long* __restrict__ key, uint32_t* __restrict__ val)
{
    const uint32_t n = *count;
    for (uint32_t j = blockIdx.x * 256 + threadIdx.x; j < n; j += gridDim.x * 256) {
        const uint32_t s = c_string[j], read = s / g.strands;
        if (!job_aligned(sink[j]) || score[j] < min_score[str_len[s]]) continue;
        const uint32_t slot = atomicAdd(cursor + read, 1u);
        if (!seg) continue;
        key[seg[read] + slot] = ((unsigned long long)(s % g.strands) << 32) | (t_off[j] + sink[j].x);
        val[seg[read] + slot] = j;
    }
}

__global__ void __launch_bounds__(256)
pair_cand_merge_kernel(const uint32_t n_reads, const uint32_t* __restrict__ seg, const uint32_t* __restrict__ cnt,
                       const unsigned long long* __restrict__ key, const uint32_t* __restrict__ val, const uint32_t* __restrict__ index,
                       const int32_t* __restrict__ score, uint32_t* __restrict__ m_end, int32_t* __restrict__ m_score, uint32_t* __restrict__ m_tie,
                       uint32_t* __restrict__ n_fw, uint32_t* __restrict__ n_merged)
{
    const uint32_t r = blockIdx.x * 256 + threadIdx.x;
    if (r >= n_reads) return;
    const uint32_t b = seg[r], n = cnt[r];
    uint32_t m = 0, fw = 0; unsigned long long prev = ~0ull;
    for (uint32_t k = b; k < b + n; ++k) {
        const unsigned long long kk = key[k];
        const uint32_t j = val[k], tie = index ? index[j] : j;
        const int32_t sc = score[j];
        if (kk == prev) {
            const uint32_t o = b + m - 1u;
            if (sc > m_score[o] || (sc == m_score[o] && tie < m_tie[o])) { m_score[o] = sc; m_tie[o] = tie; }
            continue;
        }
        prev = kk;
        m_end[b + m] = (uint32_t)kk; m_score[b + m] = sc; m_tie[b + m] = tie;
        ++m; if ((kk >> 32) == 0ull) ++fw;
    }
    n_fw[r] = fw; n_merged[r] = m;
}

__global__ void __launch_bounds__(256)
pair_second_kernel(const uint32_t n_pairs, const nvb_pair_params pp, const nvb_mapq_params mp, const uint32_t* __restrict__ str_len,
                   const uint32_t* __restrict__ seg, const uint32_t* __restrict__ n_fw, const uint32_t* __restrict__ n_merged,
                   const uint32_t* __restrict__ m_end, const int32_t* __restrict__ m_score, const uint32_t* __restrict__ m_tie,
                   const uint32_t* __restrict__ se_pos, const uint8_t* __restrict__ se_strand, const unsigned long long* __restrict__ best_key,
                   const uint32_t* __restrict__ want, const uint32_t* __restrict__ job_idx, const uint32_t* __restrict__ w_toff,
                   const int32_t* __restrict__ rs_score, const uint2* __restrict__ rs_sink,
                   const int32_t* __restrict__ pair_score, const uint32_t* __restrict__ pair_flags,
                   const uint32_t* __restrict__ mate_pos, const uint8_t* __restrict__ mate_strand,
                   int32_t* __restrict__ second_pair_score, uint32_t* __restrict__ second_mate_pos, uint8_t* __restrict__ second_mate_strand,
                   uint8_t* __restrict__ mate_mapq)
{
    const uint32_t p = blockIdx.x * 256 + threadIdx.x;
    if (p >= n_pairs) return;
    const uint32_t r0 = p, r1 = n_pairs + p;
    const uint32_t len[2] = {str_len[2u * r0], str_len[2u * r1]};
    PairSecond ps;
    ps.init(mate_pos[r0], mate_strand[r0], len[0], mate_pos[r1], mate_strand[r1], len[1]);
    const uint32_t flags = pair_flags[p];
    if (flags != NVB_PAIR_UNPAIRED) {
        MateCands m[2];
#pragma unroll
        for (int k = 0; k < 2; ++k) {
            const uint32_t r = k ? r1 : r0, b = seg[r];
            m[k].end = m_end + b; m[k].score = m_score + b; m[k].tie = m_tie + b; m[k].n_fw = n_fw[r]; m[k].n = n_merged[r]; m[k].len = len[k];
        }
        pair_combinations(m, pp.min_frag, pp.max_frag, ps);
        for (int a = 0; a < 2; ++a) {
            const uint32_t i = 2u * p + a, ra = a ? r1 : r0;
            if (!want[i]) continue;
            const uint32_t j = job_idx[i];
            if (j >= pp.rescue_capacity) continue;
            const int32_t rs = rs_score[j];
            if (rs < pp.min_mate_score || rs < mp.d_min_score[len[1 - a]]) continue;
            const unsigned long long key = best_key[ra];
            ps.offer_rescue(a, best_key_score(key) + rs, se_pos[ra], se_strand[ra], best_key_index(key), w_toff[i] + rs_sink[j].x);
        }
        const uint8_t q = (uint8_t)bowtie_mapq2(pair_score[p], ps.has, ps.score, (int32_t)(len[0] + len[1]) * mp.match_bonus,
                                                mp.d_min_score[len[0]] + mp.d_min_score[len[1]], mp.match_bonus == 0);
        mate_mapq[r0] = q; mate_mapq[r1] = q;
    }
    second_pair_score[p] = ps.score;
#pragma unroll
    for (int k = 0; k < 2; ++k) {
        if (second_mate_pos) second_mate_pos[k * n_pairs + p] = ps.end[k];
        if (second_mate_strand) second_mate_strand[k * n_pairs + p] = (uint8_t)ps.strand[k];
    }
}

}

using namespace nvb;

struct StageEvents { cudaEvent_t ev[8]; bool ready, valid; };
static StageEvents g_stage[NVB_MAX_DEVICES];
static std::mutex  g_stage_mutex;
static int default_stage_events(StageEvents** out)
{
    int dev = 0;
    NVB_CUDA_TRY(cudaGetDevice(&dev));
    if (dev < 0 || dev >= NVB_MAX_DEVICES) return NVB_E_UNSUPPORTED;
    std::lock_guard<std::mutex> lock(g_stage_mutex);
    StageEvents& S = g_stage[dev];
    if (!S.ready) {
        for (int i = 0; i < 8; ++i) NVB_CUDA_TRY(cudaEventCreate(&S.ev[i]));
        S.ready = true;
    }
    *out = &S;
    return NVB_OK;
}

extern "C" int nvb_seed_extend_stage_ms(float ms[7])
{
    if (!ms) return NVB_E_INVALID;
    StageEvents* SE = nullptr;
    { const int r = default_stage_events(&SE); if (r != NVB_OK) return r; }
    if (!SE->valid) return NVB_E_INVALID;
    NVB_CUDA_TRY(cudaEventSynchronize(SE->ev[7]));
    for (int i = 0; i < 7; ++i) NVB_CUDA_TRY(cudaEventElapsedTime(&ms[i], SE->ev[i], SE->ev[i + 1]));
    return NVB_OK;
}

static int g_perfect_shortcut = 1;
static const uint32_t* g_last_dp_count = nullptr;
static int g_seed_split = 1;
static int g_pipe_path = 0;

#define NVB_TRY(expr) do { const int _r = (expr); if (_r != NVB_OK) return _r; } while (0)
static int size_only(int r) { return r == NVB_E_TEMP_SIZE ? NVB_OK : r; }
static int launched() { return (int)cudaGetLastError(); }

static Jobs take_jobs(TempCarver& tc, size_t n) { return Jobs{tc.take<uint32_t>(n), tc.take<uint32_t>(n), tc.take<uint32_t>(n), tc.take<uint32_t>(n)}; }
struct JobViews { nvb_string_set pats, txts; };

struct PipeCall {
    PipeGeom g; cudaStream_t s; const nvb_seed_extend_params* P; FmIndex f; StrSet rd; const uint32_t* genome;
    uint32_t nq, hit_capacity;
    bool dedup, per_read, eligible;
    bool seed_split;
    int32_t* best_score; uint32_t* best_pos; int32_t* hit_score; nvb_uint2* hit_sink;
    const nvb_best_alignment_out* BA; const nvb_pair_params* PP; const nvb_pair_out* PO;
    const nvb_mapq_params* MP; const nvb_mapq_out* MO; const nvb_pair_mapq_out* PMO;
    nvb_mapq_out se_mo;
    StageEvents* SE;
    uint32_t *str_words, *str_len; uint8_t* str_quals;
    uint2* ranges; uint32_t *sizes, *excl, *counts, *seed_todo, *seed_todo_n;
    char* rj_tiles; size_t rj_tile_bytes;
    uint32_t *j_string, *j_first;
    uint32_t *leader, *flag, *job_idx;
    Jobs jobs; int32_t* job_score; uint2* job_sink;
    Jobs dp; uint32_t *dp_job, *dp_count; int32_t* dp_score; uint2* dp_sink;
    uint32_t* hit_string; Jobs hits; int32_t* h_score; uint2* h_sink;
    unsigned long long* best_key; uint8_t* rb_strand;
    char *scan_tmp, *gotoh_tmp; size_t scan_bytes, gotoh_bytes;
    Jobs best; int32_t* b_score; uint2 *b_sink, *b_source; char* tb_tmp; size_t tb_bytes;
    uint32_t *pw_want, *pw_idx, *pw_pstr, *pw_toff, *pw_tlen, *pcounts;
    Jobs rescue; int32_t* rs_score; uint2* rs_sink; char *pscan_tmp, *full_tmp; size_t pscan_bytes, full_bytes;
    uint2* rt_items; uint32_t* rt_count; char* rt_pool; size_t rt_pool_bytes;
    unsigned long long* second_key;
    uint32_t *pc_cnt, *pc_seg, *pc_fw, *pc_n, *pc_val[2], *pc_end, *pc_tie, *se_pos;
    unsigned long long* pc_key[2]; int32_t* pc_score; char *pc_scan_tmp, *pc_sort_tmp; size_t pc_scan_bytes, pc_sort_bytes;

    int stage(int i) const { return (int)cudaEventRecord(SE->ev[i], s); }

    JobViews job_views(const Jobs& j, uint32_t txt_len) const
    {
        return {{str_words ? str_words : (const uint32_t*)16,  g.bits, 1u,         j.p_off,   j.p_len,   0u,     rd.length},
                {genome,                                       2u,     1u,         j.t_off,   j.t_len,   0u,     txt_len}};
    }

    int score_jobs(const Jobs& j, const uint32_t* d_n, int32_t* score, uint2* sink) const
    {
        const JobViews v = job_views(j, rd.length + g.band);
        size_t bytes = gotoh_bytes;
        return nvb_banded_gotoh_score_indirect(g.band, P->type, &P->scheme, &v.pats, str_quals, &v.txts, d_n, hit_capacity,
                                               score, (nvb_uint2*)sink, gotoh_tmp, &bytes, s);
    }

    int carve(void* d_temp, size_t& need)
    {
        const uint32_t cap = hit_capacity, n_reads = g.n_reads;
        const JobViews sv = job_views(Jobs{}, rd.length + g.band);
        NVB_TRY(size_only(nvb_banded_gotoh_score(g.band, P->type, &P->scheme, &sv.pats, nullptr, &sv.txts, cap, nullptr, nullptr, nullptr,
                                                 &gotoh_bytes, s)));
        TempCarver tc(d_temp);
        str_words = tc.take<uint32_t>((size_t)g.n_strings * (g.stride / (32u / g.bits)) + 4);
        str_len   = tc.take<uint32_t>(g.n_strings);
        str_quals = P->d_read_quals ? tc.take<uint8_t>((size_t)g.n_strings * g.stride + 16) : nullptr;
        ranges = tc.take<uint2>(nq);
        if (!per_read) { sizes = tc.take<uint32_t>(nq); excl = tc.take<uint32_t>(nq); }
        if (seed_split) seed_todo = tc.take<uint32_t>((size_t)nq + (SEED_TODO_LISTS + 1u) * SEED_BLOCK * SEED_ITER);
        counts = tc.take<uint32_t>(4); seed_todo_n = tc.take<uint32_t>(SEED_TODO_LISTS * SEED_TODO_PITCH);
        if (per_read) {
            NVB_CUDA_TRY(RjTileState::AllocationSize((int)((n_reads + RJ_BLOCK - 1u) / RJ_BLOCK), rj_tile_bytes));
            rj_tiles = tc.take<char>(rj_tile_bytes);
        }
        if (per_read) { j_string = tc.take<uint32_t>(cap); j_first = tc.take<uint32_t>(cap); }
        else if (dedup) { leader = tc.take<uint32_t>(cap); flag = tc.take<uint32_t>(cap); job_idx = tc.take<uint32_t>(cap); }
        if (dedup) { jobs = take_jobs(tc, cap); job_score = tc.take<int32_t>(cap); job_sink = tc.take<uint2>(cap); }
        if (per_read) {
            dp = take_jobs(tc, cap); dp_job = tc.take<uint32_t>(cap); dp_score = tc.take<int32_t>(cap); dp_sink = tc.take<uint2>(cap);
            dp_count = tc.take<uint32_t>(4);
        }
        if (!per_read) { hit_string = tc.take<uint32_t>(cap); hits = take_jobs(tc, cap); }
        h_score = hit_score ? hit_score : (per_read ? nullptr : tc.take<int32_t>(cap));
        h_sink  = hit_sink ? (uint2*)hit_sink : (per_read ? nullptr : tc.take<uint2>(cap));
        best_key = tc.take<unsigned long long>(n_reads); rb_strand = tc.take<uint8_t>((size_t)n_reads + 16);
        scan_bytes = 0;
        if (!per_read) NVB_CUDA_TRY(cub::DeviceScan::ExclusiveSum(nullptr, scan_bytes, sizes, excl, (int)nq, s));
        if (dedup && !per_read && cap) {
            size_t scan2_bytes = 0;
            NVB_CUDA_TRY(cub::DeviceScan::ExclusiveSum(nullptr, scan2_bytes, flag, job_idx, (int)cap, s));
            if (scan2_bytes > scan_bytes) scan_bytes = scan2_bytes;
        }
        scan_tmp  = tc.take<char>(scan_bytes);
        gotoh_tmp = tc.take<char>(gotoh_bytes);
        if (BA) {
            best = take_jobs(tc, n_reads);
            b_score = tc.take<int32_t>(n_reads); b_sink = tc.take<uint2>(n_reads); b_source = tc.take<uint2>(n_reads);
            NVB_TRY(size_only(nvb_banded_gotoh_traceback(g.band, P->type, &P->scheme, &sv.pats, nullptr, &sv.txts, n_reads,
                                                         nullptr, nullptr, nullptr, nullptr, BA->max_ops, nullptr, nullptr, &tb_bytes, s)));
            tb_tmp = tc.take<char>(tb_bytes);
        }
        if (PP) {
            const uint32_t rcap = PP->rescue_capacity;
            pw_want = tc.take<uint32_t>(n_reads); pw_idx = tc.take<uint32_t>(n_reads); pw_pstr = tc.take<uint32_t>(n_reads);
            pw_toff = tc.take<uint32_t>(n_reads); pw_tlen = tc.take<uint32_t>(n_reads); pcounts = tc.take<uint32_t>(4);
            rescue = take_jobs(tc, rcap); rs_score = tc.take<int32_t>(rcap); rs_sink = tc.take<uint2>(rcap);
            NVB_CUDA_TRY(cub::DeviceScan::ExclusiveSum(nullptr, pscan_bytes, pw_want, pw_idx, (int)n_reads, s));
            pscan_tmp = tc.take<char>(pscan_bytes);
            const JobViews v = job_views(Jobs{}, PP->max_frag);
            NVB_TRY(size_only(nvb_gotoh_score_indirect(P->type, &P->scheme, &v.pats, nullptr, &v.txts, (const uint32_t*)16, rcap, nullptr, nullptr,
                                                       nullptr, &full_bytes, s)));
            full_tmp = tc.take<char>(full_bytes);
            if (BA) {
                NVB_TRY(full_warp_traceback(P->type, rd.length, PP->max_frag, nullptr, &rt_pool_bytes, s));
                rt_items = tc.take<uint2>((size_t)n_reads / 2u + 1u); rt_count = tc.take<uint32_t>(4); rt_pool = tc.take<char>(rt_pool_bytes);
            }
        }
        if (MO) second_key = tc.take<unsigned long long>(n_reads);
        if (PMO) {
            if (!PMO->d_mate_second_score) se_mo.d_second_score = tc.take<int32_t>(n_reads);
            pc_cnt = tc.take<uint32_t>((size_t)n_reads + 1); pc_seg = tc.take<uint32_t>((size_t)n_reads + 1);
            pc_fw = tc.take<uint32_t>(n_reads); pc_n = tc.take<uint32_t>(n_reads); se_pos = tc.take<uint32_t>(n_reads);
            for (int k = 0; k < 2; ++k) { pc_key[k] = tc.take<unsigned long long>(cap); pc_val[k] = tc.take<uint32_t>(cap); }
            pc_end = tc.take<uint32_t>(cap); pc_score = tc.take<int32_t>(cap); pc_tie = tc.take<uint32_t>(cap);
            NVB_CUDA_TRY(cub::DeviceScan::ExclusiveSum(nullptr, pc_scan_bytes, pc_cnt, pc_seg, (int)n_reads + 1, s));
            pc_scan_tmp = tc.take<char>(pc_scan_bytes);
            pc_sort_bytes = 0;
            if (cap) NVB_CUDA_TRY(cub::DeviceSegmentedSort::SortPairs(nullptr, pc_sort_bytes, pc_key[0], pc_key[1], pc_val[0], pc_val[1], (int)cap,
                                                                     (int)n_reads, pc_seg, pc_seg + 1, s));
            pc_sort_tmp = tc.take<char>(pc_sort_bytes);
        }
        need = tc.total();
        return NVB_OK;
    }

    int make_strings() const
    {
        const uint32_t grid = (uint32_t)(((uint64_t)g.n_strings * (g.stride / (32u / g.bits)) + 255) / 256);
        if (g.bits == 2 && rd.big_endian) pipe_make_strings_2bit_be_kernel<<<grid, 256, 0, s>>>(rd, g, str_words, str_len);
        else if (g.bits == 2)             pipe_make_strings_kernel<2><<<grid, 256, 0, s>>>(rd, g, str_words, str_len);
        else                              pipe_make_strings_kernel<4><<<grid, 256, 0, s>>>(rd, g, str_words, str_len);
        NVB_LAUNCH_CHECK();
        if (str_quals) pipe_make_quals_kernel<<<(uint32_t)(((uint64_t)g.n_strings * g.stride + 255) / 256), 256, 0, s>>>(rd, g, P->d_read_quals, str_quals);
        return launched();
    }

    int match_seeds() const
    {
        const uint32_t grid = (nq + SEED_BLOCK - 1) / SEED_BLOCK;
        const uint32_t* loc_genome = (per_read && f.sa_shift == 0u) ? genome : nullptr;
        if (seed_split) {
            NVB_CUDA_TRY(cudaMemsetAsync(seed_todo_n, 0, SEED_TODO_LISTS * SEED_TODO_PITCH * sizeof(uint32_t), s));
            const uint32_t grid1 = (grid + SEED_ITER - 1u) / SEED_ITER;
            if (g.bits == 2) pipe_seed_match_kernel<2, true><<<grid1, SEED_BLOCK, 0, s>>>(f, g, str_words, str_len, loc_genome, ranges, sizes, seed_todo, seed_todo_n);
            else             pipe_seed_match_kernel<4, true><<<grid1, SEED_BLOCK, 0, s>>>(f, g, str_words, str_len, loc_genome, ranges, sizes, seed_todo, seed_todo_n);
            NVB_LAUNCH_CHECK();
            const uint32_t wgrid = (sm_count() * 16u + SEED_TODO_LISTS - 1u) / SEED_TODO_LISTS * SEED_TODO_LISTS;
            if (g.bits == 2) pipe_seed_match_wide_kernel<2><<<wgrid, SEED_BLOCK, 0, s>>>(f, g, str_words, loc_genome, ranges, sizes, seed_todo, seed_todo_n, grid1);
            else             pipe_seed_match_wide_kernel<4><<<wgrid, SEED_BLOCK, 0, s>>>(f, g, str_words, loc_genome, ranges, sizes, seed_todo, seed_todo_n, grid1);
        } else {
            if (g.bits == 2) pipe_seed_match_kernel<2, false><<<grid, SEED_BLOCK, 0, s>>>(f, g, str_words, str_len, loc_genome, ranges, sizes, nullptr, nullptr);
            else             pipe_seed_match_kernel<4, false><<<grid, SEED_BLOCK, 0, s>>>(f, g, str_words, str_len, loc_genome, ranges, sizes, nullptr, nullptr);
        }
        return launched();
    }

    int extend_per_read() const
    {
        const nvb_gotoh_scheme& SC = P->scheme;
        const uint32_t cap = hit_capacity, n_tiles = (g.n_reads + RJ_BLOCK - 1u) / RJ_BLOCK;
        RjTileState tiles;
        NVB_CUDA_TRY(tiles.Init((int)n_tiles, rj_tiles, rj_tile_bytes));
        pipe_resolve_init_kernel<<<(n_tiles + 255u) / 256u, 256, 0, s>>>(tiles, n_tiles, counts, dp_count);
        NVB_LAUNCH_CHECK();
        const int shortcut = eligible ? g_perfect_shortcut : 0;
        const int32_t max_gap_open = SC.pattern_gap_open > SC.text_gap_open ? SC.pattern_gap_open : SC.text_gap_open;
        pipe_resolve_reads_kernel<<<n_tiles, RJ_BLOCK, 0, s>>>(f, g, ranges, str_len, cap, tiles, n_tiles, counts, shortcut, SC.match,
                SC.mismatch, max_gap_open, str_words, genome, j_string, j_first, jobs, job_score, job_sink, dp, dp_job, dp_count,
                best_key, best_score, best_pos, rb_strand);
        NVB_LAUNCH_CHECK();
        g_last_dp_count = dp_count;
        NVB_TRY(stage(4)); NVB_TRY(stage(5));
        const uint32_t hgrid = (cap + 255) / 256, jgrid = hgrid < sm_count() * 16u ? hgrid : sm_count() * 16u;
        if (cap) {
            NVB_TRY(score_jobs(dp, dp_count, dp_score, dp_sink));
            pipe_scatter_dp_kernel<<<jgrid, 256, 0, s>>>(g, dp_count, dp_job, dp_score, dp_sink, j_string, j_first, job_score, job_sink, best_key);
            NVB_LAUNCH_CHECK();
        }
        NVB_TRY(stage(6));
        if (cap) {
            pipe_finalize_dp_kernel<<<jgrid, 256, 0, s>>>(g, dp_count, dp_job, dp_score, dp_sink, dp.t_off, j_string, j_first, best_key,
                                                          best_score, best_pos, rb_strand);
            NVB_LAUNCH_CHECK();
        }
        return launched();
    }

    int extend_per_hit() const
    {
        const uint32_t cap = hit_capacity, hgrid = (cap + 255) / 256;
        if (cap) {
            pipe_expand_hits_kernel<<<(nq + 255) / 256, 256, 0, s>>>(f, g, ranges, sizes, excl, str_len, counts,
                                                                     hit_string, hits.p_off, hits.p_len, hits.t_off, hits.t_len);
            NVB_LAUNCH_CHECK();
        }
        NVB_TRY(stage(4));
        if (dedup && cap) {
            pipe_find_leaders_kernel<<<hgrid, 256, 0, s>>>(counts, hit_string, hits.t_off, hits.t_len, leader, flag);
            NVB_LAUNCH_CHECK();
            size_t bytes = scan_bytes;
            NVB_CUDA_TRY(cub::DeviceScan::ExclusiveSum(scan_tmp, bytes, flag, job_idx, (int)cap, s));
            pipe_job_count_kernel<<<1, 32, 0, s>>>(job_idx, flag, counts);
            NVB_LAUNCH_CHECK();
            pipe_compact_jobs_kernel<<<hgrid, 256, 0, s>>>(counts, flag, job_idx, hits.p_off, hits.p_len, hits.t_off, hits.t_len,
                                                           jobs.p_off, jobs.p_len, jobs.t_off, jobs.t_len);
            NVB_LAUNCH_CHECK();
        }
        NVB_TRY(stage(5));
        NVB_CUDA_TRY(cudaMemsetAsync(best_key, 0, sizeof(unsigned long long) * g.n_reads, s));
        if (cap && dedup) {
            NVB_TRY(score_jobs(jobs, counts + 2, job_score, job_sink));
            pipe_scatter_scores_kernel<<<hgrid, 256, 0, s>>>(g, counts, leader, job_idx, job_score, job_sink, hit_string, h_score, h_sink, best_key);
            NVB_LAUNCH_CHECK();
        } else if (cap)
            NVB_TRY(score_jobs(hits, counts, h_score, h_sink));
        NVB_TRY(stage(6));
        if (cap && !dedup) {
            pipe_reduce_kernel<<<hgrid, 256, 0, s>>>(g, counts, hit_string, h_score, h_sink, best_key);
            NVB_LAUNCH_CHECK();
        }
        pipe_finalize_kernel<<<(g.n_reads + 255) / 256, 256, 0, s>>>(g, best_key, hits.t_off, h_sink, hit_string, best_score, best_pos, rb_strand);
        return launched();
    }

    int best_traceback() const
    {
        const uint32_t rgrid = (g.n_reads + 255) / 256;
        if (per_read) {
            pipe_empty_jobs_kernel<<<rgrid, 256, 0, s>>>(g.n_reads, best.p_off, best.p_len, best.t_off, best.t_len, BA->d_strand);
            NVB_LAUNCH_CHECK();
            const uint32_t hgrid = (hit_capacity + 255) / 256, jgrid = hgrid < sm_count() * 16u ? hgrid : sm_count() * 16u;
            if (jgrid) {
                pipe_read_best_jobs_kernel<<<jgrid, 256, 0, s>>>(g, counts, j_string, j_first, job_score, best_key, jobs.p_off, jobs.p_len,
                                                                 jobs.t_off, jobs.t_len, best.p_off, best.p_len, best.t_off, best.t_len, BA->d_strand);
                NVB_LAUNCH_CHECK();
            }
        } else {
            pipe_best_jobs_kernel<<<rgrid, 256, 0, s>>>(g, best_key, hit_string, hits.p_off, hits.p_len, hits.t_off, hits.t_len,
                                                        best.p_off, best.p_len, best.t_off, best.t_len, BA->d_strand);
            NVB_LAUNCH_CHECK();
        }
        if (PP) {
            const uint32_t n_pairs = g.n_reads / 2u;
            pair_empty_rescued_jobs_kernel<<<(n_pairs + 255) / 256, 256, 0, s>>>(n_pairs, PO->d_pair_flags, best.p_len, best.t_len);
            NVB_LAUNCH_CHECK();
        }
        const JobViews v = job_views(best, rd.length + g.band);
        size_t bytes = tb_bytes;
        NVB_TRY(nvb_banded_gotoh_traceback(g.band, P->type, &P->scheme, &v.pats, str_quals, &v.txts, g.n_reads, b_score, (nvb_uint2*)b_sink,
                                           (nvb_uint2*)b_source, BA->d_ops, BA->max_ops, BA->d_n_ops, tb_tmp, &bytes, s));
        pipe_best_begin_kernel<<<rgrid, 256, 0, s>>>(g, best_key, best.t_off, b_source, BA->d_n_ops, (uint2*)BA->d_begin);
        return launched();
    }

    int second_best() const
    {
        const uint32_t cap = hit_capacity, hgrid = (cap + 255) / 256;
        NVB_CUDA_TRY(cudaMemsetAsync(second_key, 0, sizeof(unsigned long long) * g.n_reads, s));
        if (cap) {
            const uint32_t* n   = per_read ? counts + 2 : counts;
            const uint32_t* cs  = per_read ? j_string : hit_string;
            const uint32_t* idx = per_read ? j_first : nullptr;
            const uint32_t* to  = per_read ? jobs.t_off : hits.t_off;
            const int32_t* sc   = per_read ? job_score : h_score;
            const uint2* sk     = per_read ? job_sink : h_sink;
            const uint32_t grid = hgrid < sm_count() * 16u ? hgrid : sm_count() * 16u;
            pipe_second_reduce_kernel<<<grid, 256, 0, s>>>(g, n, cs, idx, to, sc, sk, str_len, best_pos, rb_strand, MP->d_min_score, second_key);
            NVB_LAUNCH_CHECK();
            if (MO->d_second_pos || MO->d_second_strand) {
                pipe_second_finalize_kernel<<<grid, 256, 0, s>>>(g, n, cs, idx, to, sc, sk, second_key, MO->d_second_pos, MO->d_second_strand);
                NVB_LAUNCH_CHECK();
            }
        }
        pipe_mapq_kernel<<<(g.n_reads + 255) / 256, 256, 0, s>>>(g, *MP, str_len, best_score, second_key, MO->d_second_score, MO->d_second_pos,
                                                                MO->d_second_strand, MO->d_mapq);
        return launched();
    }

    int pair_candidates() const
    {
        const uint32_t cap = hit_capacity, n_reads = g.n_reads;
        NVB_CUDA_TRY(cudaMemcpyAsync(se_pos, best_pos, sizeof(uint32_t) * n_reads, cudaMemcpyDeviceToDevice, s));
        NVB_CUDA_TRY(cudaMemsetAsync(pc_cnt, 0, sizeof(uint32_t) * ((size_t)n_reads + 1), s));
        if (cap) {
            const uint32_t* n  = per_read ? counts + 2 : counts;
            const uint32_t* cs = per_read ? j_string : hit_string;
            const uint32_t* to = per_read ? jobs.t_off : hits.t_off;
            const int32_t* sc  = per_read ? job_score : h_score;
            const uint2* sk    = per_read ? job_sink : h_sink;
            const uint32_t hgrid = (cap + 255) / 256, grid = hgrid < sm_count() * 16u ? hgrid : sm_count() * 16u;
            pair_cand_scatter_kernel<<<grid, 256, 0, s>>>(g, n, cs, to, sc, sk, str_len, MP->d_min_score, nullptr, pc_cnt, nullptr, nullptr);
            NVB_LAUNCH_CHECK();
            size_t bytes = pc_scan_bytes;
            NVB_CUDA_TRY(cub::DeviceScan::ExclusiveSum(pc_scan_tmp, bytes, pc_cnt, pc_seg, (int)n_reads + 1, s));
            NVB_CUDA_TRY(cudaMemsetAsync(pc_cnt, 0, sizeof(uint32_t) * n_reads, s));
            pair_cand_scatter_kernel<<<grid, 256, 0, s>>>(g, n, cs, to, sc, sk, str_len, MP->d_min_score, pc_seg, pc_cnt, pc_key[0], pc_val[0]);
            NVB_LAUNCH_CHECK();
            bytes = pc_sort_bytes;
            NVB_CUDA_TRY(cub::DeviceSegmentedSort::SortPairs(pc_sort_tmp, bytes, pc_key[0], pc_key[1], pc_val[0], pc_val[1], (int)cap, (int)n_reads,
                                                             pc_seg, pc_seg + 1, s));
        } else
            NVB_CUDA_TRY(cudaMemsetAsync(pc_seg, 0, sizeof(uint32_t) * ((size_t)n_reads + 1), s));
        pair_cand_merge_kernel<<<(n_reads + 255) / 256, 256, 0, s>>>(n_reads, pc_seg, pc_cnt, pc_key[1], pc_val[1], per_read ? j_first : nullptr,
                                                                      per_read ? job_score : h_score, pc_end, pc_score, pc_tie, pc_fw, pc_n);
        return launched();
    }

    int pair_second() const
    {
        const uint32_t n_pairs = g.n_reads / 2u;
        pair_second_kernel<<<(n_pairs + 255) / 256, 256, 0, s>>>(n_pairs, *PP, *MP, str_len, pc_seg, pc_fw, pc_n, pc_end, pc_score, pc_tie,
                                                                  se_pos, rb_strand, best_key, pw_want, pw_idx, pw_toff, rs_score, rs_sink,
                                                                  PO->d_pair_score, PO->d_pair_flags, PO->d_mate_pos, PO->d_mate_strand,
                                                                  PMO->d_second_pair_score, PMO->d_second_mate_pos, PMO->d_second_mate_strand,
                                                                  PMO->d_mate_mapq);
        return launched();
    }

    int paired_rescue() const
    {
        const uint32_t n_reads = g.n_reads, n_pairs = n_reads / 2u, cap = PP->rescue_capacity;
        const uint32_t pgrid = (n_pairs + 255) / 256, sgrid = (n_reads + 255) / 256;
        pair_classify_kernel<<<pgrid, 256, 0, s>>>(g, n_pairs, *PP, best_score, best_pos, rb_strand, str_len, pw_want, pw_pstr, pw_toff, pw_tlen,
                                                    PO->d_pair_score, PO->d_pair_flags, PO->d_mate_score, PO->d_mate_pos, PO->d_mate_strand);
        NVB_LAUNCH_CHECK();
        size_t bytes = pscan_bytes;
        NVB_CUDA_TRY(cub::DeviceScan::ExclusiveSum(pscan_tmp, bytes, pw_want, pw_idx, (int)n_reads, s));
        pipe_count_kernel<<<1, 32, 0, s>>>(pw_idx, pw_want, n_reads, cap, pcounts);
        NVB_LAUNCH_CHECK();
        if (cap) {
            pair_compact_kernel<<<sgrid, 256, 0, s>>>(g, n_reads, cap, pw_want, pw_idx, pw_pstr, pw_toff, pw_tlen, str_len,
                                                      rescue.p_off, rescue.p_len, rescue.t_off, rescue.t_len);
            NVB_LAUNCH_CHECK();
            const JobViews v = job_views(rescue, PP->max_frag);
            size_t fb = full_bytes;
            NVB_TRY(nvb_gotoh_score_indirect(P->type, &P->scheme, &v.pats, str_quals, &v.txts, pcounts, cap, rs_score, (nvb_uint2*)rs_sink, full_tmp, &fb, s));
        }
        pair_finalize_kernel<<<pgrid, 256, 0, s>>>(n_pairs, *PP, pw_want, pw_idx, pw_toff, rs_score, rs_sink, PO->d_pair_score, PO->d_pair_flags,
                                                    PO->d_mate_score, PO->d_mate_pos, PO->d_mate_strand);
        NVB_LAUNCH_CHECK();
        if (PO->d_n_rescue) NVB_CUDA_TRY(cudaMemcpyAsync(PO->d_n_rescue, pcounts, 2 * sizeof(uint32_t), cudaMemcpyDeviceToDevice, s));
        return NVB_OK;
    }

    int rescue_traceback() const
    {
        const uint32_t n_pairs = g.n_reads / 2u;
        NVB_CUDA_TRY(cudaMemsetAsync(rt_count, 0, sizeof(uint32_t), s));
        pair_rescue_items_kernel<<<(n_pairs + 255) / 256, 256, 0, s>>>(n_pairs, PO->d_pair_flags, pw_idx, PO->d_mate_strand, rt_items, rt_count,
                                                                       BA->d_strand);
        NVB_LAUNCH_CHECK();
        const JobViews v = job_views(rescue, PP->max_frag);
        FullTbArgs a;
        a.S = make_scheme(&P->scheme); a.pat = make_strset(&v.pats); a.txt = make_strset(&v.txts); a.quals = str_quals;
        a.score = rs_score; a.sink = rs_sink; a.items = rt_items; a.n_items = rt_count;
        a.o.ops = BA->d_ops; a.o.n_ops = BA->d_n_ops; a.o.source = (uint2*)BA->d_begin; a.o.max_ops = BA->max_ops; a.o.absolute = 1u;
        a.pool = rt_pool;
        size_t bytes = rt_pool_bytes;
        return full_warp_traceback(P->type, rd.length, PP->max_frag, &a, &bytes, s);
    }
};

static int seed_extend_impl(const nvb_fm_index* fmi, const uint32_t* d_genome,
                    const nvb_string_set* reads, uint32_t n_reads,
                    const nvb_seed_extend_params* P, uint32_t hit_capacity,
                    int32_t* d_best_score, uint32_t* d_best_pos,
                    uint32_t* d_n_hits, uint32_t* d_hit_read, nvb_uint2* d_hit_window,
                    int32_t* d_hit_score, nvb_uint2* d_hit_sink,
                    const nvb_best_alignment_out* BA,
                    const nvb_pair_params* PP, const nvb_pair_out* PO,
                    const nvb_mapq_params* MP, const nvb_mapq_out* MO, const nvb_pair_mapq_out* PMO,
                    void* d_temp, size_t* temp_bytes, void* stream)
{
    if (PP) {
        if (!PO || !PO->d_pair_score || !PO->d_pair_flags || !PO->d_mate_score || !PO->d_mate_pos || !PO->d_mate_strand) return NVB_E_INVALID;
        if (!P || !P->both_strands || (n_reads & 1u) || PP->max_frag == 0 || PP->min_frag > PP->max_frag) return NVB_E_INVALID;
    }
    if (BA && (!BA->d_ops || !BA->d_n_ops || !BA->d_begin || BA->max_ops == 0)) return NVB_E_INVALID;
    if (!valid_fmindex(fmi) || !fmi->d_ssa || !d_genome || !valid_strset(reads) || !P || !temp_bytes) return NVB_E_INVALID;
    if (reads->bits == 8) return NVB_E_UNSUPPORTED;
    if (P->seed_len == 0 || P->seed_interval == 0 || P->max_seed_hits == 0) return NVB_E_INVALID;
    if (n_reads && (!d_best_score || !d_best_pos)) return NVB_E_INVALID;
    const uint32_t max_len = reads->length;
    if (max_len < P->seed_len) return NVB_E_INVALID;

    PipeCall c = {};
    PipeGeom& g = c.g;
    g.n_reads = n_reads; g.strands = P->both_strands ? 2u : 1u; g.n_strings = n_reads * g.strands;
    g.bits = reads->bits;
    const uint32_t spw = 32u / g.bits;
    g.stride = (max_len + spw - 1u) / spw * spw;
    g.seeds_per_string = (max_len - P->seed_len) / P->seed_interval + 1u;
    g.seed_len = P->seed_len; g.seed_interval = P->seed_interval; g.band = P->band_len;
    g.max_seed_hits = P->max_seed_hits; g.genome_len = fmi->length;
    if ((uint64_t)g.n_strings * g.stride > 0xFFFFFFFFull) return NVB_E_UNSUPPORTED;
    const uint64_t nq64 = (uint64_t)g.n_strings * g.seeds_per_string;
    if (nq64 > 0x7FFFFFFFull) return NVB_E_UNSUPPORTED;
    if (nq64 * (uint64_t)P->max_seed_hits > 0xFFFFFFFFull) return NVB_E_UNSUPPORTED;

    const cudaStream_t s = c.s = as_stream(stream);
    c.P = P; c.f = make_fmindex(fmi); c.rd = make_strset(reads); c.genome = d_genome; c.nq = (uint32_t)nq64; c.hit_capacity = hit_capacity;
    c.best_score = d_best_score; c.best_pos = d_best_pos; c.hit_score = d_hit_score; c.hit_sink = d_hit_sink; c.BA = BA; c.PP = PP; c.PO = PO; c.MP = MP; c.MO = MO;
    if (PMO) {
        c.PMO = PMO;
        c.se_mo.d_second_score = PMO->d_mate_second_score; c.se_mo.d_mapq = PMO->d_mate_mapq;
        c.MO = &c.se_mo;
    }
    c.dedup = P->dedup_jobs != 0;
    c.per_read = c.dedup && g_pipe_path != 1 && !d_hit_read && !d_hit_window && !d_hit_score && !d_hit_sink;
    const nvb_gotoh_scheme& SC = P->scheme;
    c.eligible = c.per_read && P->type == NVB_LOCAL && g.bits == 2 && P->band_len <= 32 && !SC.d_qual_table && SC.match > 0 && SC.mismatch < 0 &&
                 SC.pattern_gap_open < 0 && SC.pattern_gap_ext <= 0 && SC.text_gap_open < 0 && SC.text_gap_ext <= 0;
    c.seed_split = c.per_read && c.f.sa_shift == 0u && c.f.ktab_k && g.seed_len > c.f.ktab_k && g_seed_split;
    size_t need = 0;
    NVB_TRY(c.carve(d_temp, need));
    if (!d_temp || *temp_bytes < need) { *temp_bytes = need; return NVB_E_TEMP_SIZE; }
    if (n_reads == 0) return NVB_OK;

    NVB_TRY(default_stage_events(&c.SE));
    NVB_TRY(c.stage(0));
    NVB_TRY(c.make_strings()); NVB_TRY(c.stage(1));
    NVB_TRY(c.match_seeds());  NVB_TRY(c.stage(2));
    if (!c.per_read) {
        size_t scan_bytes = c.scan_bytes;
        NVB_CUDA_TRY(cub::DeviceScan::ExclusiveSum(c.scan_tmp, scan_bytes, c.sizes, c.excl, (int)c.nq, s));
        pipe_count_kernel<<<1, 32, 0, s>>>(c.excl, c.sizes, c.nq, hit_capacity, c.counts);
        NVB_LAUNCH_CHECK();
    }
    NVB_TRY(c.stage(3));
    NVB_TRY(c.per_read ? c.extend_per_read() : c.extend_per_hit());
    if (hit_capacity && (d_hit_read || d_hit_window)) {
        pipe_export_hits_kernel<<<(hit_capacity + 255) / 256, 256, 0, s>>>(g, c.counts, c.hit_string, c.hits.t_off, c.hits.t_len, d_hit_read, (uint2*)d_hit_window);
        NVB_LAUNCH_CHECK();
    }
    if (BA && !PP) NVB_TRY(c.best_traceback());
    if (c.MO) NVB_TRY(c.second_best());
    if (PMO) NVB_TRY(c.pair_candidates());
    if (PP) NVB_TRY(c.paired_rescue());
    if (BA && PP) { NVB_TRY(c.best_traceback()); NVB_TRY(c.rescue_traceback()); }
    if (PMO) NVB_TRY(c.pair_second());
    if (!c.dedup) NVB_CUDA_TRY(cudaMemcpyAsync(c.counts + 2, c.counts, sizeof(uint32_t), cudaMemcpyDeviceToDevice, s));
    if (d_n_hits) NVB_CUDA_TRY(cudaMemcpyAsync(d_n_hits, c.counts, 3 * sizeof(uint32_t), cudaMemcpyDeviceToDevice, s));
    NVB_TRY(c.stage(7));
    c.SE->valid = true;
    return NVB_OK;
}

extern "C" void nvb_debug_pipeline_path(int path) { g_pipe_path = path; }
extern "C" void nvb_debug_seed_split(int on) { g_seed_split = on; }
extern "C" void nvb_debug_perfect_shortcut(int on) { g_perfect_shortcut = on; }
extern "C" int nvb_debug_dp_jobs(uint32_t* n)
{
    if (!n || !g_last_dp_count) return NVB_E_INVALID;
    NVB_CUDA_TRY(cudaDeviceSynchronize());
    NVB_CUDA_TRY(cudaMemcpy(n, g_last_dp_count, sizeof(uint32_t), cudaMemcpyDeviceToHost));
    return NVB_OK;
}

extern "C" int nvb_seed_extend(const nvb_fm_index* fmi, const uint32_t* d_genome,
                    const nvb_string_set* reads, uint32_t n_reads,
                    const nvb_seed_extend_params* P, uint32_t hit_capacity,
                    int32_t* d_best_score, uint32_t* d_best_pos,
                    uint32_t* d_n_hits, uint32_t* d_hit_read, nvb_uint2* d_hit_window,
                    int32_t* d_hit_score, nvb_uint2* d_hit_sink,
                    void* d_temp, size_t* temp_bytes, void* stream)
{
    return seed_extend_impl(fmi, d_genome, reads, n_reads, P, hit_capacity, d_best_score, d_best_pos, d_n_hits, d_hit_read, d_hit_window,
                            d_hit_score, d_hit_sink, nullptr, nullptr, nullptr, nullptr, nullptr, nullptr, d_temp, temp_bytes, stream);
}

extern "C" int nvb_seed_extend_traceback(const nvb_fm_index* fmi, const uint32_t* d_genome,
                    const nvb_string_set* reads, uint32_t n_reads,
                    const nvb_seed_extend_params* P, uint32_t hit_capacity,
                    int32_t* d_best_score, uint32_t* d_best_pos,
                    uint32_t* d_n_hits, uint32_t* d_hit_read, nvb_uint2* d_hit_window,
                    int32_t* d_hit_score, nvb_uint2* d_hit_sink,
                    const nvb_best_alignment_out* best_alignment,
                    void* d_temp, size_t* temp_bytes, void* stream)
{
    if (!best_alignment) return NVB_E_INVALID;
    return seed_extend_impl(fmi, d_genome, reads, n_reads, P, hit_capacity, d_best_score, d_best_pos, d_n_hits, d_hit_read, d_hit_window,
                            d_hit_score, d_hit_sink, best_alignment, nullptr, nullptr, nullptr, nullptr, nullptr, d_temp, temp_bytes, stream);
}

extern "C" int nvb_seed_extend_paired(const nvb_fm_index* fmi, const uint32_t* d_genome,
                    const nvb_string_set* reads, uint32_t n_pairs,
                    const nvb_seed_extend_params* P, uint32_t hit_capacity,
                    const nvb_pair_params* pair_params, const nvb_pair_out* out,
                    uint32_t* d_n_hits, void* d_temp, size_t* temp_bytes, void* stream)
{
    if (!pair_params || !out || n_pairs > 0x3FFFFFFFu || !temp_bytes) return NVB_E_INVALID;
    return seed_extend_impl(fmi, d_genome, reads, 2u * n_pairs, P, hit_capacity, out->d_mate_score, out->d_mate_pos, d_n_hits, nullptr, nullptr,
                            nullptr, nullptr, nullptr, pair_params, out, nullptr, nullptr, nullptr, d_temp, temp_bytes, stream);
}

extern "C" int nvb_seed_extend_mapq(const nvb_fm_index* fmi, const uint32_t* d_genome,
                    const nvb_string_set* reads, uint32_t n_reads,
                    const nvb_seed_extend_params* P, uint32_t hit_capacity,
                    int32_t* d_best_score, uint32_t* d_best_pos,
                    uint32_t* d_n_hits, uint32_t* d_hit_read, nvb_uint2* d_hit_window,
                    int32_t* d_hit_score, nvb_uint2* d_hit_sink,
                    const nvb_best_alignment_out* best_alignment,
                    const nvb_mapq_params* mapq, const nvb_mapq_out* mapq_out,
                    void* d_temp, size_t* temp_bytes, void* stream)
{
    if (!mapq || !mapq_out || !mapq->d_min_score || !mapq_out->d_second_score || !mapq_out->d_mapq) return NVB_E_INVALID;
    if (!reads || mapq->max_read_len < reads->length) return NVB_E_INVALID;
    return seed_extend_impl(fmi, d_genome, reads, n_reads, P, hit_capacity, d_best_score, d_best_pos, d_n_hits, d_hit_read, d_hit_window,
                            d_hit_score, d_hit_sink, best_alignment, nullptr, nullptr, mapq, mapq_out, nullptr, d_temp, temp_bytes, stream);
}

extern "C" int nvb_seed_extend_paired_mapq(const nvb_fm_index* fmi, const uint32_t* d_genome,
                    const nvb_string_set* reads, uint32_t n_pairs,
                    const nvb_seed_extend_params* P, uint32_t hit_capacity,
                    const nvb_pair_params* pair_params, const nvb_pair_out* out,
                    const nvb_mapq_params* mapq, const nvb_pair_mapq_out* mapq_out,
                    uint32_t* d_n_hits, void* d_temp, size_t* temp_bytes, void* stream)
{
    if (!pair_params || !out || n_pairs > 0x3FFFFFFFu || !temp_bytes) return NVB_E_INVALID;
    if (!mapq || !mapq_out || !mapq->d_min_score || !mapq_out->d_second_pair_score || !mapq_out->d_mate_mapq) return NVB_E_INVALID;
    if (!reads || mapq->max_read_len < reads->length) return NVB_E_INVALID;
    return seed_extend_impl(fmi, d_genome, reads, 2u * n_pairs, P, hit_capacity, out->d_mate_score, out->d_mate_pos, d_n_hits, nullptr, nullptr,
                            nullptr, nullptr, nullptr, pair_params, out, mapq, nullptr, mapq_out, d_temp, temp_bytes, stream);
}

extern "C" int nvb_seed_extend_paired_traceback(const nvb_fm_index* fmi, const uint32_t* d_genome,
                    const nvb_string_set* reads, uint32_t n_pairs,
                    const nvb_seed_extend_params* P, uint32_t hit_capacity,
                    const nvb_pair_params* pair_params, const nvb_pair_out* out,
                    const nvb_best_alignment_out* mate_alignment,
                    const nvb_mapq_params* mapq, const nvb_pair_mapq_out* mapq_out,
                    uint32_t* d_n_hits, void* d_temp, size_t* temp_bytes, void* stream)
{
    if (!pair_params || !out || n_pairs > 0x3FFFFFFFu || !temp_bytes || !reads) return NVB_E_INVALID;
    const nvb_best_alignment_out* BA = mate_alignment;
    if (!BA || !BA->d_ops || !BA->d_n_ops || !BA->d_begin || BA->max_ops == 0) return NVB_E_INVALID;
    if ((mapq == nullptr) != (mapq_out == nullptr)) return NVB_E_INVALID;
    if (mapq) {
        if (!mapq->d_min_score || !mapq_out->d_second_pair_score || !mapq_out->d_mate_mapq) return NVB_E_INVALID;
        if (mapq->max_read_len < reads->length) return NVB_E_INVALID;
    }
    if (reads->length > FULL_TB_MAX_M) return NVB_E_UNSUPPORTED;
    return seed_extend_impl(fmi, d_genome, reads, 2u * n_pairs, P, hit_capacity, out->d_mate_score, out->d_mate_pos, d_n_hits, nullptr, nullptr,
                            nullptr, nullptr, BA, pair_params, out, mapq, nullptr, mapq_out, d_temp, temp_bytes, stream);
}

extern "C" int nvb_debug_mapq_eval(const int32_t* d_best, const uint8_t* d_has_second, const int32_t* d_second, const uint32_t* d_len,
                                   const int32_t* d_match_bonus, const int32_t* d_min_score, uint32_t n, uint8_t* d_mapq, void* stream)
{
    if (!n) return NVB_OK;
    if (!d_best || !d_has_second || !d_second || !d_len || !d_match_bonus || !d_min_score || !d_mapq) return NVB_E_INVALID;
    debug_mapq_eval_kernel<<<(n + 255) / 256, 256, 0, as_stream(stream)>>>(d_best, d_has_second, d_second, d_len, d_match_bonus, d_min_score, n, d_mapq);
    return launched();
}
```

### nvbio_b200/fmindex.py

```python
import ctypes as C
from typing import Optional
import numpy as np
import torch
from ._lib import lib, check, FmIndexStruct, NvbError
from .strings import PackedStringSet

MATCH_FORWARD_ORDER = 1
MATCH_COMPLEMENT = 2


ROWS_HEADROOM = 4 << 30


def _stream():
    return C.c_void_p(torch.cuda.current_stream().cuda_stream)


def _np_u32(t: torch.Tensor) -> np.ndarray:
    return t.detach().cpu().numpy().view(np.uint32)


def _dev_u32(a: np.ndarray, device) -> torch.Tensor:
    return torch.from_numpy(np.ascontiguousarray(a, dtype=np.uint32).view(np.int32)).to(device)


class FMIndexDevice:

    def __init__(self, bwt_occ: torch.Tensor, ssa: Optional[torch.Tensor], L2, length: int, primary: int,
                 sa_interval: int = 16, ktab: Optional[torch.Tensor] = None, ktab_k: int = 0):
        assert bwt_occ.is_cuda and bwt_occ.data_ptr() % 32 == 0
        self.bwt_occ, self.ssa = bwt_occ, ssa
        self.L2 = [int(v) for v in L2]
        self.length, self.primary = int(length), int(primary)
        self.sa_interval = int(sa_interval)
        self.ktab, self.ktab_k = ktab, int(ktab_k)
        self.ktab_located = 0
        self.ktab_wide = False
        self.rows = None

    def struct(self) -> FmIndexStruct:
        s = FmIndexStruct()
        s.d_bwt_occ = self.bwt_occ.data_ptr()
        s.d_ssa = self.ssa.data_ptr() if self.ssa is not None else None
        s.length, s.primary = self.length, self.primary
        for i in range(5):
            s.L2[i] = self.L2[i]
        s.sa_interval = self.sa_interval
        s.d_ktab = self.ktab.data_ptr() if self.ktab is not None else None
        s.ktab_k = self.ktab_k if self.ktab is not None else 0
        s.ktab_located = int(self.ktab_located) if self.ktab is not None else 0
        if s.ktab_located == 2 and self.ktab_wide:
            s.ktab_located = 4
        if s.ktab_located in (2, 4) and self.rows is not None:
            s.ktab_located, s.d_rows = s.ktab_located + 1, self.rows.data_ptr()
        return s

    @property
    def device(self):
        return self.bwt_occ.device

    def nbytes(self):
        return (self.bwt_occ.numel() * 4 + (self.ssa.numel() * 4 if self.ssa is not None else 0) +
                (self.ktab.numel() * 4 if self.ktab is not None else 0) + (self.rows.numel() * 4 if self.rows is not None else 0))

    def build_ktab(self, k: int = 12, located: bool = False, text: Optional[torch.Tensor] = None):
        self.ktab = None
        self.rows = None
        self.ktab_wide = False
        full_text = located and text is not None and self.sa_interval == 1 and self.ssa is not None
        wide = False
        if full_text:
            l2 = torch.cuda.get_device_properties(self.device).L2_cache_size
            free, _ = torch.cuda.mem_get_info(self.device)
            wide = 4 ** k * 16 > l2 and 4 ** k * 32 + ROWS_HEADROOM <= free
        tab = torch.empty((4 ** k, 8 if wide else (4 if located else 2)), dtype=torch.int32, device=self.device)
        s = self.struct()
        if wide:
            assert text.is_cuda and text.dtype == torch.int32
            check(lib().nvb_fm_build_ktab_wide(C.byref(s), C.c_uint32(k), C.c_void_p(text.data_ptr()), C.c_void_p(tab.data_ptr()), _stream()),
                  "nvb_fm_build_ktab_wide")
        elif located and text is not None:
            assert text.is_cuda and text.dtype == torch.int32
            check(lib().nvb_fm_build_ktab_context(C.byref(s), C.c_uint32(k), C.c_void_p(text.data_ptr()), C.c_void_p(tab.data_ptr()), _stream()),
                  "nvb_fm_build_ktab_context")
        elif located:
            check(lib().nvb_fm_build_ktab_located(C.byref(s), C.c_uint32(k), C.c_void_p(tab.data_ptr()), _stream()), "nvb_fm_build_ktab_located")
        else:
            check(lib().nvb_fm_build_ktab(C.byref(s), C.c_uint32(k), C.c_void_p(tab.data_ptr()), _stream()), "nvb_fm_build_ktab")
        self.ktab, self.ktab_k, self.ktab_located = tab, k, (2 if (located and text is not None) else (1 if located else 0))
        self.ktab_wide = wide
        if full_text:
            need = (self.length + 1) * 8
            free, _ = torch.cuda.mem_get_info(self.device)
            if need + ROWS_HEADROOM <= free:
                rows = torch.empty((self.length + 1, 2), dtype=torch.int32, device=self.device)
                check(lib().nvb_fm_build_rows(C.byref(self.struct()), C.c_void_p(text.data_ptr()), C.c_void_p(rows.data_ptr()), _stream()),
                      "nvb_fm_build_rows")
                self.rows = rows
        return self

    @staticmethod
    def from_host(bwt_occ: np.ndarray, ssa: Optional[np.ndarray], L2, length, primary, device="cuda", sa_interval=16):
        return FMIndexDevice(_dev_u32(bwt_occ, device), None if ssa is None else _dev_u32(ssa, device), L2, length, primary,
                             sa_interval=sa_interval)

    @staticmethod
    def from_bwt(bwt_words: torch.Tensor, n: int, primary: int, ssa: Optional[torch.Tensor], sa_interval: int = 16):
        L = lib()
        n_blocks = (n + 63) // 64
        bwt_occ = torch.empty(n_blocks * 8, dtype=torch.int32, device=bwt_words.device)
        L2 = (C.c_uint32 * 5)()
        tb = C.c_size_t(0)
        r = L.nvb_fm_build_occ(C.c_void_p(bwt_words.data_ptr()), C.c_uint32(n), C.c_void_p(bwt_occ.data_ptr()), L2,
                               None, C.byref(tb), _stream())
        if r != -2:
            check(r, "nvb_fm_build_occ(size query)")
        temp = torch.empty(max(tb.value, 1), dtype=torch.uint8, device=bwt_words.device)
        check(L.nvb_fm_build_occ(C.c_void_p(bwt_words.data_ptr()), C.c_uint32(n), C.c_void_p(bwt_occ.data_ptr()), L2,
                                 C.c_void_p(temp.data_ptr()), C.byref(tb), _stream()), "nvb_fm_build_occ")
        return FMIndexDevice(bwt_occ, ssa, list(L2), n, primary, sa_interval=sa_interval)

    @staticmethod
    def from_text(text_words: torch.Tensor, n: int, want_sa: bool = False, sa_interval: int = 16):
        L = lib()
        dev = text_words.device
        bwt = torch.empty(((n + 63) // 64) * 4, dtype=torch.int32, device=dev)
        ssa = torch.empty((n + sa_interval) // sa_interval, dtype=torch.int32, device=dev)
        sa = torch.empty(n + 1, dtype=torch.int32, device=dev) if want_sa else None
        primary = C.c_uint32(0)
        tb = C.c_size_t(0)
        args = (C.c_void_p(text_words.data_ptr()), C.c_uint32(n), C.c_void_p(bwt.data_ptr()), C.byref(primary),
                C.c_void_p(ssa.data_ptr()), C.c_uint32(sa_interval), C.c_void_p(sa.data_ptr()) if sa is not None else None)
        r = L.nvb_fm_build_bwt(*args, None, C.byref(tb), _stream())
        if r != -2:
            check(r, "nvb_fm_build_bwt(size query)")
        temp = torch.empty(tb.value, dtype=torch.uint8, device=dev)
        check(L.nvb_fm_build_bwt(*args, C.c_void_p(temp.data_ptr()), C.byref(tb), _stream()), "nvb_fm_build_bwt")
        del temp
        idx = FMIndexDevice.from_bwt(bwt, n, int(primary.value), ssa, sa_interval=sa_interval)
        return idx, sa

    def to_host(self):
        return dict(bwt_occ=_np_u32(self.bwt_occ), ssa=None if self.ssa is None else _np_u32(self.ssa),
                    L2=np.array(self.L2, dtype=np.uint32), n=self.length, primary=self.primary, sa_interval=self.sa_interval)


def rank(fmi: FMIndexDevice, k: torch.Tensor, c: torch.Tensor) -> torch.Tensor:
    n = k.numel()
    out = torch.empty(n, dtype=torch.int32, device=k.device)
    s = fmi.struct()
    check(lib().nvb_fm_rank(C.byref(s), C.c_void_p(k.data_ptr()), C.c_void_p(c.data_ptr()), C.c_uint32(n),
                            C.c_void_p(out.data_ptr()), _stream()), "nvb_fm_rank")
    return out


def rank4(fmi: FMIndexDevice, k: torch.Tensor) -> torch.Tensor:
    n = k.numel()
    out = torch.empty((n, 4), dtype=torch.int32, device=k.device)
    s = fmi.struct()
    check(lib().nvb_fm_rank4(C.byref(s), C.c_void_p(k.data_ptr()), C.c_uint32(n), C.c_void_p(out.data_ptr()), _stream()), "nvb_fm_rank4")
    return out


def match(fmi: FMIndexDevice, queries: PackedStringSet, flags: int = 0, out: Optional[torch.Tensor] = None) -> torch.Tensor:
    n = queries.count
    if out is None:
        out = torch.empty((n, 2), dtype=torch.int32, device=fmi.device)
    s, q = fmi.struct(), queries.struct()
    check(lib().nvb_fm_match(C.byref(s), C.byref(q), C.c_uint32(n), C.c_uint32(flags),
                             C.c_void_p(out.data_ptr()), _stream()), "nvb_fm_match")
    return out


def match_approx(fmi: FMIndexDevice, queries: PackedStringSet, exact_len: int, find_exact: bool = True, max_out: int = 64, flags: int = 0):
    n = queries.count
    dev = fmi.device
    ranges = torch.zeros((n, max_out, 2), dtype=torch.int32, device=dev)
    counts = torch.empty(n, dtype=torch.int32, device=dev)
    sums = torch.empty(n, dtype=torch.int32, device=dev)
    s, q = fmi.struct(), queries.struct()
    check(lib().nvb_fm_match_approx(C.byref(s), C.byref(q), C.c_uint32(n), C.c_uint32(flags), C.c_uint32(exact_len),
                                    C.c_int(1 if find_exact else 0), C.c_uint32(max_out), C.c_void_p(ranges.data_ptr()),
                                    C.c_void_p(counts.data_ptr()), C.c_void_p(sums.data_ptr()), _stream()), "nvb_fm_match_approx")
    return ranges, counts, sums


def locate(fmi: FMIndexDevice, rows: torch.Tensor) -> torch.Tensor:
    n = rows.numel()
    out = torch.empty(n, dtype=torch.int32, device=rows.device)
    s = fmi.struct()
    check(lib().nvb_fm_locate(C.byref(s), C.c_void_p(rows.data_ptr()), C.c_uint32(n), C.c_void_p(out.data_ptr()), _stream()),
          "nvb_fm_locate")
    return out


def dict_rank(text_words: torch.Tensor, occ: torch.Tensor, K: int, i: torch.Tensor, c: Optional[torch.Tensor] = None) -> torch.Tensor:
    wb = 32 if text_words.dtype == torch.int32 else 64
    ib = 32 if occ.dtype == torch.int32 else 64
    assert i.dtype == occ.dtype
    n = i.numel()
    if c is None:
        out = torch.empty((n, 4), dtype=occ.dtype, device=i.device)
        check(lib().nvb_dict_rank4(C.c_void_p(text_words.data_ptr()), C.c_uint32(wb), C.c_void_p(occ.data_ptr()), C.c_uint32(ib), C.c_uint32(K),
                                   C.c_void_p(i.data_ptr()), C.c_uint32(n), C.c_void_p(out.data_ptr()), _stream()), "nvb_dict_rank4")
        return out
    out = torch.empty(n, dtype=occ.dtype, device=i.device)
    check(lib().nvb_dict_rank(C.c_void_p(text_words.data_ptr()), C.c_uint32(wb), C.c_void_p(occ.data_ptr()), C.c_uint32(ib), C.c_uint32(K),
                              C.c_void_p(i.data_ptr()), C.c_void_p(c.data_ptr()), C.c_uint32(n), C.c_void_p(out.data_ptr()), _stream()), "nvb_dict_rank")
    return out


def dict_build_occ(text_words: torch.Tensor, n_symbols: int, K: int, index_bits: int = 32):
    wb = 32 if text_words.dtype == torch.int32 else 64
    n_blocks = (n_symbols + K - 1) // K
    occ = torch.empty(n_blocks * 4, dtype=torch.int32 if index_bits == 32 else torch.int64, device=text_words.device)
    counts = (C.c_uint64 * 4)()
# ... 123 lines not shown
```

### nvbio_b200/pipeline.py

```python
import ctypes as C
import ctypes.util
from dataclasses import dataclass, field
from typing import Optional
import torch
import numpy as np
from ._lib import (lib, check, SeedExtendParamsStruct, BestAlignmentOutStruct, PairParamsStruct, PairOutStruct, MapqParamsStruct, MapqOutStruct,
                   PairMapqOutStruct)
from .strings import PackedStringSet
from .fmindex import FMIndexDevice
from . import aln


@dataclass
class SeedExtendParams:
    seed_len: int = 20
    seed_interval: int = 10
    band_len: int = 31
    type: int = aln.LOCAL
    both_strands: bool = True
    max_seed_hits: int = 100
    dedup_jobs: bool = True
    scheme: object = field(default_factory=lambda: aln.SimpleGotohScheme(2, -2, -5, -3))
    read_quals: Optional[torch.Tensor] = None

    def struct(self) -> SeedExtendParamsStruct:
        p = SeedExtendParamsStruct()
        p.seed_len, p.seed_interval, p.band_len, p.type = self.seed_len, self.seed_interval, self.band_len, self.type
        p.both_strands = 1 if self.both_strands else 0
        p.max_seed_hits = self.max_seed_hits
        p.dedup_jobs = 1 if self.dedup_jobs else 0
        p.scheme = self.scheme.struct()
        p.d_read_quals = self.read_quals.data_ptr() if self.read_quals is not None else None
        return p


_libm = None


def simple_func(kind: str, const: float, coeff: float, x) -> np.ndarray:
    global _libm
    if kind not in ("L", "G", "S"):
        raise ValueError("SimpleFunc type must be 'L', 'G' or 'S', not %r" % (kind,))
    if kind != "L" and _libm is None:
        _libm = C.CDLL(ctypes.util.find_library("m"))
        for f in (_libm.logf, _libm.sqrtf):
            f.restype, f.argtypes = C.c_float, [C.c_float]
    k, m = np.float32(const), np.float32(coeff)
    out = []
    for v in np.asarray(x, dtype=np.int64).reshape(-1):
        fx = np.float32(v)
        if kind == "G":
            fx = np.float32(_libm.logf(float(fx)))
        elif kind == "S":
            fx = np.float32(_libm.sqrtf(float(fx)))
        with np.errstate(invalid="ignore", over="ignore"):
            y = k + m * fx
        if np.isnan(y):
            raise ValueError("SimpleFunc %s,%g,%g is not a number at x = %d" % (kind, const, coeff, v))
        out.append(int(max(min(float(y), 2.0 ** 31 - 1), -(2.0 ** 31 - 1))))
    return np.array(out, dtype=np.int32)


@dataclass
class MapqParams:
    min_score: torch.Tensor
    match_bonus: int

    @property
    def max_read_len(self) -> int:
        return self.min_score.numel() - 1

    @classmethod
    def from_score_min(cls, kind: str, const: float, coeff: float, max_read_len: int, match_bonus: int, device="cuda") -> "MapqParams":
        tab = simple_func(kind, const, coeff, np.arange(max_read_len + 1))
        return cls(torch.from_numpy(tab).to(device), int(match_bonus))

    @classmethod
    def local(cls, max_read_len: int, device="cuda") -> "MapqParams":
        return cls.from_score_min("G", 0.0, 10.0, max_read_len, 2, device)

    @classmethod
    def end_to_end(cls, max_read_len: int, device="cuda") -> "MapqParams":
        return cls.from_score_min("L", -0.6, -0.6, max_read_len, 0, device)

    def struct(self) -> MapqParamsStruct:
        assert self.min_score.dtype == torch.int32 and self.min_score.is_cuda and self.min_score.is_contiguous()
        p = MapqParamsStruct()
        p.d_min_score, p.max_read_len, p.match_bonus = self.min_score.data_ptr(), self.max_read_len, self.match_bonus
        return p


class SeedExtendWorkspace:

    def __init__(self, fmi: FMIndexDevice, genome: torch.Tensor, reads: PackedStringSet, params: SeedExtendParams,
                 hit_capacity: int, keep_hits: bool = False, traceback: bool = False, mapq: Optional[MapqParams] = None):
        dev = fmi.device
        n = reads.count
        self.best_score = torch.empty(n, dtype=torch.int32, device=dev)
        self.best_pos = torch.empty(n, dtype=torch.int32, device=dev)
        self.n_hits = torch.zeros(3, dtype=torch.int32, device=dev)
        self.hit_capacity = hit_capacity
        self.hit_read = self.hit_window = self.hit_score = self.hit_sink = None
        if keep_hits:
            self.hit_read = torch.empty(hit_capacity, dtype=torch.int32, device=dev)
            self.hit_window = torch.empty((hit_capacity, 2), dtype=torch.int32, device=dev)
            self.hit_score = torch.empty(hit_capacity, dtype=torch.int32, device=dev)
            self.hit_sink = torch.empty((hit_capacity, 2), dtype=torch.int32, device=dev)
        self.best_ops = self.best_n_ops = self.best_begin = self.best_strand = None
        self.max_ops = 2 * reads.length + params.band_len
        if traceback:
            self.best_ops = torch.zeros((n, self.max_ops), dtype=torch.uint8, device=dev)
            self.best_n_ops = torch.zeros(n, dtype=torch.int32, device=dev)
            self.best_begin = torch.empty((n, 2), dtype=torch.int32, device=dev)
            self.best_strand = torch.empty(n, dtype=torch.uint8, device=dev)
        self.mapq_params = mapq
        self.second_score = self.second_pos = self.second_strand = self.mapq = None
        if mapq is not None:
            self.second_score = torch.empty(n, dtype=torch.int32, device=dev)
            self.second_pos = torch.empty(n, dtype=torch.int32, device=dev)
            self.second_strand = torch.empty(n, dtype=torch.uint8, device=dev)
            self.mapq = torch.empty(n, dtype=torch.uint8, device=dev)
        tb = C.c_size_t(0)
        r = _call(fmi, genome, reads, params, self, None, tb)
        if r != -2:
            check(r, "nvb_seed_extend(size query)")
        self.temp = torch.empty(tb.value, dtype=torch.uint8, device=dev)
        self.temp_bytes = tb.value


def _p(t):
    return C.c_void_p(t.data_ptr()) if t is not None else None


def _call(fmi, genome, reads, params, ws, temp, tb):
    s, rd, ps = fmi.struct(), reads.struct(), params.struct()
    ba = None
    if ws.best_ops is not None:
        ba = BestAlignmentOutStruct()
        ba.d_ops, ba.max_ops, ba.d_n_ops = ws.best_ops.data_ptr(), ws.max_ops, ws.best_n_ops.data_ptr()
        ba.d_begin, ba.d_strand = ws.best_begin.data_ptr(), ws.best_strand.data_ptr()
    if ws.mapq is not None:
        mp = ws.mapq_params.struct()
        mo = MapqOutStruct()
        mo.d_second_score, mo.d_second_pos = ws.second_score.data_ptr(), ws.second_pos.data_ptr()
        mo.d_second_strand, mo.d_mapq = ws.second_strand.data_ptr(), ws.mapq.data_ptr()
        return lib().nvb_seed_extend_mapq(C.byref(s), _p(genome), C.byref(rd), C.c_uint32(reads.count), C.byref(ps),
                                          C.c_uint32(ws.hit_capacity), _p(ws.best_score), _p(ws.best_pos), _p(ws.n_hits),
                                          _p(ws.hit_read), _p(ws.hit_window), _p(ws.hit_score), _p(ws.hit_sink),
                                          C.byref(ba) if ba is not None else None, C.byref(mp), C.byref(mo),
                                          _p(temp), C.byref(tb), C.c_void_p(torch.cuda.current_stream().cuda_stream))
    if ba is not None:
        return lib().nvb_seed_extend_traceback(C.byref(s), _p(genome), C.byref(rd), C.c_uint32(reads.count), C.byref(ps),
                                               C.c_uint32(ws.hit_capacity), _p(ws.best_score), _p(ws.best_pos), _p(ws.n_hits),
                                               _p(ws.hit_read), _p(ws.hit_window), _p(ws.hit_score), _p(ws.hit_sink), C.byref(ba),
                                               _p(temp), C.byref(tb), C.c_void_p(torch.cuda.current_stream().cuda_stream))
    return lib().nvb_seed_extend(C.byref(s), _p(genome), C.byref(rd), C.c_uint32(reads.count), C.byref(ps),
                                 C.c_uint32(ws.hit_capacity), _p(ws.best_score), _p(ws.best_pos), _p(ws.n_hits),
                                 _p(ws.hit_read), _p(ws.hit_window), _p(ws.hit_score), _p(ws.hit_sink),
                                 _p(temp), C.byref(tb), C.c_void_p(torch.cuda.current_stream().cuda_stream))


def seed_extend(fmi: FMIndexDevice, genome: torch.Tensor, reads: PackedStringSet, params: SeedExtendParams,
                workspace: Optional[SeedExtendWorkspace] = None, hit_capacity: Optional[int] = None, keep_hits: bool = False,
                traceback: bool = False, mapq: Optional[MapqParams] = None):
    if workspace is None:
        if hit_capacity is None:
            hit_capacity = 32 * reads.count + 1024
        workspace = SeedExtendWorkspace(fmi, genome, reads, params, hit_capacity, keep_hits, traceback, mapq)
    elif mapq is not None:
        if workspace.mapq is None:
            raise ValueError("seed_extend(mapq=...): the workspace was created without mapq outputs")
        workspace.mapq_params = mapq
    tb = C.c_size_t(workspace.temp_bytes)
    check(_call(fmi, genome, reads, params, workspace, workspace.temp, tb), "nvb_seed_extend")
    return workspace


PAIR_UNPAIRED, PAIR_CONCORDANT, PAIR_RESCUED_MATE1, PAIR_RESCUED_MATE2 = 0, 1, 2, 4


@dataclass
class PairParams:
    min_frag: int = 0
    max_frag: int = 500
    min_mate_score: int = 60
    rescue_capacity: Optional[int] = None

    def struct(self, n_pairs) -> PairParamsStruct:
        p = PairParamsStruct()
        p.min_frag, p.max_frag, p.min_mate_score = self.min_frag, self.max_frag, self.min_mate_score
        p.rescue_capacity = 2 * n_pairs if self.rescue_capacity is None else self.rescue_capacity
        return p


class PairedWorkspace:

    def __init__(self, fmi, genome, reads: PackedStringSet, params: SeedExtendParams, pair: PairParams, hit_capacity: int,
                 mapq: Optional[MapqParams] = None, traceback: bool = False, max_ops: Optional[int] = None):
        dev = fmi.device
        assert reads.count % 2 == 0
        self.n_pairs = n = reads.count // 2
        self.hit_capacity = hit_capacity
        self.pair_score = torch.empty(n, dtype=torch.int32, device=dev)
        self.pair_flags = torch.empty(n, dtype=torch.int32, device=dev)
        self.mate_score = torch.empty((2, n), dtype=torch.int32, device=dev)
        self.mate_pos = torch.empty((2, n), dtype=torch.int32, device=dev)
        self.mate_strand = torch.empty((2, n), dtype=torch.uint8, device=dev)
        self.n_rescue = torch.zeros(2, dtype=torch.int32, device=dev)
        self.n_hits = torch.zeros(3, dtype=torch.int32, device=dev)
        self.mapq_params = mapq
        self.second_pair_score = self.second_mate_pos = self.second_mate_strand = self.mate_second_score = self.mate_mapq = None
        if mapq is not None:
            self.second_pair_score = torch.empty(n, dtype=torch.int32, device=dev)
            self.second_mate_pos = torch.empty((2, n), dtype=torch.int32, device=dev)
            self.second_mate_strand = torch.empty((2, n), dtype=torch.uint8, device=dev)
            self.mate_second_score = torch.empty((2, n), dtype=torch.int32, device=dev)
            self.mate_mapq = torch.empty((2, n), dtype=torch.uint8, device=dev)
        self.mate_ops = self.mate_n_ops = self.mate_begin = None
        self.max_ops = 2 * reads.length + params.band_len if max_ops is None else max_ops
        if traceback:
            self.mate_ops = torch.zeros((2, n, self.max_ops), dtype=torch.uint8, device=dev)
            self.mate_n_ops = torch.zeros((2, n), dtype=torch.int32, device=dev)
            self.mate_begin = torch.empty((2, n, 2), dtype=torch.int32, device=dev)
        tb = C.c_size_t(0)
        r = _call_paired(fmi, genome, reads, params, pair, self, None, tb)
        if r != -2:
            check(r, "nvb_seed_extend_paired(size query)")
        self.temp = torch.empty(tb.value, dtype=torch.uint8, device=dev)
        self.temp_bytes = tb.value


def _call_paired(fmi, genome, reads, params, pair, ws, temp, tb):
    s, rd, ps, pp = fmi.struct(), reads.struct(), params.struct(), pair.struct(ws.n_pairs)
    po = PairOutStruct()
    po.d_pair_score, po.d_pair_flags = ws.pair_score.data_ptr(), ws.pair_flags.data_ptr()
    po.d_mate_score, po.d_mate_pos, po.d_mate_strand = ws.mate_score.data_ptr(), ws.mate_pos.data_ptr(), ws.mate_strand.data_ptr()
    po.d_n_rescue = ws.n_rescue.data_ptr()
    stream = C.c_void_p(torch.cuda.current_stream().cuda_stream)
    mp = mo = None
    if ws.mate_mapq is not None:
        mp = ws.mapq_params.struct()
        mo = PairMapqOutStruct()
        mo.d_second_pair_score, mo.d_second_mate_pos = ws.second_pair_score.data_ptr(), ws.second_mate_pos.data_ptr()
        mo.d_second_mate_strand, mo.d_mate_second_score = ws.second_mate_strand.data_ptr(), ws.mate_second_score.data_ptr()
        mo.d_mate_mapq = ws.mate_mapq.data_ptr()
    if ws.mate_ops is not None:
        ba = BestAlignmentOutStruct()
        ba.d_ops, ba.max_ops, ba.d_n_ops = ws.mate_ops.data_ptr(), ws.max_ops, ws.mate_n_ops.data_ptr()
        ba.d_begin, ba.d_strand = ws.mate_begin.data_ptr(), None
        return lib().nvb_seed_extend_paired_traceback(C.byref(s), _p(genome), C.byref(rd), C.c_uint32(ws.n_pairs), C.byref(ps),
                                                      C.c_uint32(ws.hit_capacity), C.byref(pp), C.byref(po), C.byref(ba),
                                                      C.byref(mp) if mp is not None else None, C.byref(mo) if mo is not None else None,
                                                      _p(ws.n_hits), _p(temp), C.byref(tb), stream)
    if mo is not None:
        return lib().nvb_seed_extend_paired_mapq(C.byref(s), _p(genome), C.byref(rd), C.c_uint32(ws.n_pairs), C.byref(ps),
                                                 C.c_uint32(ws.hit_capacity), C.byref(pp), C.byref(po), C.byref(mp), C.byref(mo),
                                                 _p(ws.n_hits), _p(temp), C.byref(tb), stream)
    return lib().nvb_seed_extend_paired(C.byref(s), _p(genome), C.byref(rd), C.c_uint32(ws.n_pairs), C.byref(ps), C.c_uint32(ws.hit_capacity),
                                        C.byref(pp), C.byref(po), _p(ws.n_hits), _p(temp), C.byref(tb), stream)


def seed_extend_paired(fmi: FMIndexDevice, genome: torch.Tensor, reads: PackedStringSet, params: SeedExtendParams, pair: PairParams,
                       workspace: Optional[PairedWorkspace] = None, hit_capacity: Optional[int] = None, mapq: Optional[MapqParams] = None,
                       traceback: bool = False):
    if workspace is None:
        if hit_capacity is None:
            hit_capacity = 32 * reads.count + 1024
        workspace = PairedWorkspace(fmi, genome, reads, params, pair, hit_capacity, mapq, traceback)
    elif traceback and workspace.mate_ops is None:
        raise ValueError("seed_extend_paired(traceback=True): the workspace was created without traceback outputs")
    elif mapq is not None:
        if workspace.mate_mapq is None:
            raise ValueError("seed_extend_paired(mapq=...): the workspace was created without mapq outputs")
        workspace.mapq_params = mapq
    tb = C.c_size_t(workspace.temp_bytes)
    check(_call_paired(fmi, genome, reads, params, pair, workspace, workspace.temp, tb), "nvb_seed_extend_paired")
    return workspace


STAGES = ("strings", "seed_match", "hit_slots", "locate_windows", "dedup", "extend", "reduce")


def last_stage_ms():
    ms = (C.c_float * 7)()
    check(lib().nvb_seed_extend_stage_ms(ms), "nvb_seed_extend_stage_ms")
    return dict(zip(STAGES, [float(v) for v in ms]))


def _host_view(ptr, count, dtype):
    nbytes = count * torch.tensor([], dtype=dtype).element_size()
    buf = (C.c_char * nbytes).from_address(ptr)
    return torch.frombuffer(buf, dtype=dtype, count=count)


class StreamingSeedExtend:

    def __init__(self, fmi: FMIndexDevice, genome: torch.Tensor, params: SeedExtendParams, n_reads: int, read_len: int,
                 words_per_read: int, hit_capacity: Optional[int] = None, depth: int = 2, bits: int = 2, pair: Optional["PairParams"] = None):
        self.fmi, self.genome, self.params, self.pair = fmi, genome, params, pair
        self.n_reads, self.read_len, self.wpr, self.bits, self.depth = n_reads, read_len, words_per_read, bits, depth
        if hit_capacity is None:
            hit_capacity = 32 * n_reads + 1024
        self._params_struct = params.struct()
        s = fmi.struct()
        pp = pair.struct(n_reads // 2) if pair is not None else None
        self._h = C.c_void_p()
        with torch.cuda.device(fmi.device):
            check(lib().nvb_pipeline_create(C.byref(s), C.c_void_p(genome.data_ptr()), C.byref(self._params_struct),
                                            C.byref(pp) if pp is not None else None,
                                            C.c_uint32(n_reads), C.c_uint32(read_len), C.c_uint32(words_per_read), C.c_uint32(bits),
                                            C.c_uint32(hit_capacity), C.c_uint32(depth), C.byref(self._h)), "nvb_pipeline_create")
        h2d, d2h = C.c_size_t(0), C.c_size_t(0)
        lib().nvb_pipeline_traffic(self._h, C.byref(h2d), C.byref(d2h))
        self.h2d_bytes, self.d2h_bytes = int(h2d.value), int(d2h.value)
        self._keep = {}
        self.last_device_ms = None

    def submit(self, host_words: torch.Tensor) -> int:
        assert not host_words.is_cuda and host_words.is_contiguous() and host_words.numel() == self.n_reads * self.wpr
        t = C.c_uint32(0)
        check(lib().nvb_pipeline_submit(self._h, C.c_void_p(host_words.data_ptr()), C.byref(t)), "nvb_pipeline_submit")
        self._keep[int(t.value)] = host_words
        return int(t.value)

    def result(self, ticket: int):
        from ._lib import PipelineResultStruct
        r = PipelineResultStruct()
        check(lib().nvb_pipeline_wait(self._h, C.c_uint32(ticket), C.byref(r)), "nvb_pipeline_wait")
        self._keep.pop(ticket, None)
        self.last_device_ms = float(r.device_ms)
        n = self.n_reads
        if self.pair is None:
            return _host_view(r.best_score, n, torch.int32), _host_view(r.best_pos, n, torch.int32), _host_view(r.n_hits, 3, torch.int32)
        return dict(pair_score=_host_view(r.pair_score, n // 2, torch.int32), pair_flags=_host_view(r.pair_flags, n // 2, torch.int32),
                    mate_score=_host_view(r.mate_score, n, torch.int32).view(2, n // 2), mate_pos=_host_view(r.mate_pos, n, torch.int32).view(2, n // 2),
                    mate_strand=_host_view(r.mate_strand, n, torch.uint8).view(2, n // 2), n_rescue=_host_view(r.n_rescue, 2, torch.int32),
                    n_hits=_host_view(r.n_hits, 3, torch.int32))

    def close(self):
        if self._h:
            lib().nvb_pipeline_destroy(self._h)
            self._h = C.c_void_p()

    def __del__(self):
        try:
            self.close()
        except Exception:
            pass
```

Baseline: 399.3.

## Anchor interior seed lookups on unique genome L-mers from first/last seeds

Precomputes a bitmap of genome positions whose seed-length L-mer is unique, built by comparing adjacent suffix-array entries. The first and last seed of each read are located first in a new kernel. Interior seeds then predict their genome position from a unique anchor and verify it with a direct text comparison plus the uniqueness bit, skipping the FM-index backward search when the check passes. This adds an extra kernel, a per-read anchor buffer and a genome-sized bitmap, and only pays off when most reads map to unique regions without indels between seeds.

```diff
diff --git a/include/nvbio_b200.h b/include/nvbio_b200.h
--- a/include/nvbio_b200.h
+++ b/include/nvbio_b200.h
@@ -32,6 +32,8 @@
     uint32_t        ktab_k;
     uint32_t        ktab_located;
     const nvb_uint2* d_rows;
+    const uint32_t* d_unique;
+    uint32_t        unique_len;
 } nvb_fm_index;
 
 typedef struct nvb_string_set {
@@ -173,6 +175,8 @@
 int nvb_fm_build_ktab_wide(const nvb_fm_index* fmi, uint32_t k, const uint32_t* d_text, void* d_ktab32, void* stream);
 
 int nvb_fm_build_rows(const nvb_fm_index* fmi, const uint32_t* d_text, nvb_uint2* d_rows, void* stream);
+
+int nvb_fm_build_unique(const nvb_fm_index* fmi, uint32_t L, const uint32_t* d_text, uint32_t* d_bits, void* stream);
 
 typedef struct nvb_seed_extend_params {
     uint32_t seed_len;
diff --git a/include/nvbio_b200_debug.h b/include/nvbio_b200_debug.h
--- a/include/nvbio_b200_debug.h
+++ b/include/nvbio_b200_debug.h
@@ -18,6 +18,8 @@
 void nvb_debug_pipeline_path(int path);
 
 void nvb_debug_seed_split(int on);
+void nvb_debug_seed_anchor(int on);
+int nvb_debug_seed_anchor_used(void);
 
 void nvb_debug_perfect_shortcut(int on);
 int nvb_debug_dp_jobs(uint32_t* n);
diff --git a/nvbio_b200/_lib.py b/nvbio_b200/_lib.py
--- a/nvbio_b200/_lib.py
+++ b/nvbio_b200/_lib.py
@@ -8,7 +8,7 @@
     "nvb_version", "nvb_error_string",
     "nvb_fm_rank", "nvb_fm_rank4", "nvb_fm_match", "nvb_fm_match_approx", "nvb_fm_locate", "nvb_fm_filter_rank", "nvb_fm_filter_locate",
     "nvb_banded_gotoh_score", "nvb_banded_gotoh_score_indirect", "nvb_banded_gotoh_traceback", "nvb_gotoh_score", "nvb_gotoh_score_indirect", "nvb_banded_gotoh_score_window", "nvb_banded_gotoh_score_best2", "nvb_gotoh_traceback", "nvb_seed_extend_paired",
-    "nvb_fm_build_occ", "nvb_fm_build_bwt", "nvb_fm_build_ktab", "nvb_fm_build_ktab_located", "nvb_fm_build_ktab_context", "nvb_fm_build_ktab_wide", "nvb_fm_build_rows", "nvb_seed_extend", "nvb_seed_extend_traceback", "nvb_seed_extend_mapq", "nvb_seed_extend_paired_mapq", "nvb_seed_extend_paired_traceback",
+    "nvb_fm_build_occ", "nvb_fm_build_bwt", "nvb_fm_build_ktab", "nvb_fm_build_ktab_located", "nvb_fm_build_ktab_context", "nvb_fm_build_ktab_wide", "nvb_fm_build_rows", "nvb_fm_build_unique", "nvb_seed_extend", "nvb_seed_extend_traceback", "nvb_seed_extend_mapq", "nvb_seed_extend_paired_mapq", "nvb_seed_extend_paired_traceback",
     "nvb_seed_extend_stage_ms",
     "nvb_dict_rank", "nvb_dict_rank4", "nvb_dict_build_occ",
     "nvb_map_seeds", "nvb_fm_locate_init", "nvb_fm_locate_lookup", "nvb_fm_locate_sorted",
@@ -18,7 +18,7 @@
 DEBUG_EXPORTS = [
     "nvb_debug_gotoh_last_route", "nvb_debug_force_gotoh_path", "nvb_debug_full_minb", "nvb_debug_full_warp", "nvb_debug_full_traceback_warp",
     "nvb_debug_pair_format", "nvb_debug_pair_rows2", "nvb_debug_traceback_fast", "nvb_debug_pair_extra_smem",
-    "nvb_debug_pipeline_path", "nvb_debug_seed_split", "nvb_debug_perfect_shortcut", "nvb_debug_dp_jobs", "nvb_debug_mapq_eval",
+    "nvb_debug_pipeline_path", "nvb_debug_seed_split", "nvb_debug_seed_anchor", "nvb_debug_seed_anchor_used", "nvb_debug_perfect_shortcut", "nvb_debug_dp_jobs", "nvb_debug_mapq_eval",
     "nvb_debug_bgzf_grid",
 ]
 
@@ -30,7 +30,8 @@
 class FmIndexStruct(C.Structure):
     _fields_ = [("d_bwt_occ", C.c_void_p), ("d_ssa", C.c_void_p), ("length", C.c_uint32),
                 ("primary", C.c_uint32), ("L2", C.c_uint32 * 5), ("sa_interval", C.c_uint32),
-                ("d_ktab", C.c_void_p), ("ktab_k", C.c_uint32), ("ktab_located", C.c_uint32), ("d_rows", C.c_void_p)]
+                ("d_ktab", C.c_void_p), ("ktab_k", C.c_uint32), ("ktab_located", C.c_uint32), ("d_rows", C.c_void_p),
+                ("d_unique", C.c_void_p), ("unique_len", C.c_uint32)]
 
 
 class StringSetStruct(C.Structure):
diff --git a/nvbio_b200/csrc/fm_core.cuh b/nvbio_b200/csrc/fm_core.cuh
--- a/nvbio_b200/csrc/fm_core.cuh
+++ b/nvbio_b200/csrc/fm_core.cuh
@@ -19,6 +19,8 @@
     uint32_t ktab_located;
     const uint2*    rows;
     uint32_t ktab_wide;
+    const uint32_t* unique;
+    uint32_t unique_len;
     __host__ __device__ __forceinline__ uint32_t l2(uint32_t c) const {
         return (c == 0) ? L2[0] : (c == 1) ? L2[1] : (c == 2) ? L2[2] : L2[3];
     }
@@ -31,10 +33,11 @@
     if (!f || !f->d_bwt_occ) return false;
     const uint32_t I = f->sa_interval;
     if (I != 0 && (I & (I - 1)) != 0) return false;
-    if (f->d_ktab && (f->ktab_k < 1 || f->ktab_k > 16 || f->ktab_located > 5u)) return false;
+    if (f->d_ktab && (f->ktab_k < 1 || f->ktab_k > 16 || f->ktab_located > 6u)) return false;
     if (f->d_ktab && f->ktab_located >= 3u && (f->sa_interval != 1u || !f->d_ssa)) return false;
     if (f->d_ktab && f->ktab_located >= 4u && ((uintptr_t)f->d_ktab & 31u)) return false;
-    if (f->d_ktab && (f->ktab_located == 3u || f->ktab_located == 5u) && !f->d_rows) return false;
+    if (f->d_ktab && (f->ktab_located == 3u || f->ktab_located >= 5u) && !f->d_rows) return false;
+    if (f->d_ktab && f->ktab_located == 6u && (!f->d_unique || f->unique_len < 1u || f->unique_len > 32u)) return false;
     return true;
 }
 static inline FmIndex make_fmindex(const nvb_fm_index* f) {
@@ -45,10 +48,13 @@
     r.sa_shift = 0; while ((1u << r.sa_shift) < I) ++r.sa_shift;
     r.sa_mask = (1u << r.sa_shift) - 1u;
     r.ktab = (const uint2*)f->d_ktab; r.ktab_k = f->d_ktab ? f->ktab_k : 0u;
-    const bool with_rows = f->d_ktab && (f->ktab_located == 3u || f->ktab_located == 5u);
+    const bool with_rows = f->d_ktab && (f->ktab_located == 3u || f->ktab_located >= 5u);
+    const bool with_unique = f->d_ktab && f->ktab_located == 6u;
     r.ktab_wide = (f->d_ktab && f->ktab_located >= 4u) ? 1u : 0u;
     r.ktab_located = f->d_ktab ? (f->ktab_located >= 2u ? 2u : f->ktab_located) : 0u;
     r.rows = with_rows ? (const uint2*)f->d_rows : nullptr;
+    r.unique = with_unique ? f->d_unique : nullptr;
+    r.unique_len = with_unique ? f->unique_len : 0u;
     return r;
 }
 
@@ -520,6 +526,72 @@
     return FM_RANGE;
 }
 
+constexpr uint32_t NO_ANCHOR = 0xFFFFFFFFu;
+__host__ __device__ __forceinline__ uint32_t unique_init_word(uint32_t w, uint32_t n, uint32_t L)
+{
+    const uint32_t cnt = n >= L ? n - L + 1u : 0u;
+    const uint64_t lo = 32ull * w;
+    if (lo + 32u <= cnt) return 0xFFFFFFFFu;
+    if (lo >= cnt) return 0u;
+    return (1u << (cnt - (uint32_t)lo)) - 1u;
+}
+__host__ __device__ __forceinline__ bool lmer_shared(const uint32_t* __restrict__ text, uint32_t n, uint32_t a, uint32_t b, uint32_t L)
+{
+    if (n < L || a == 0xFFFFFFFFu || b == 0xFFFFFFFFu || a > n - L || b > n - L) return false;
+    bool same = true;
+    for (uint32_t i = 0; i < L; i += 16u) {
+        const uint32_t cnt = L - i < 16u ? L - i : 16u;
+        same &= ((be2_window(text, a + i, cnt) ^ be2_window(text, b + i, cnt)) >> (32u - 2u * cnt)) == 0u;
+    }
+    return same;
+}
+
+__host__ __device__ __forceinline__ uint32_t last_anchor_seed(uint32_t len, uint32_t L, uint32_t I)
+{
+    return len >= L ? (len - L) / I : 0u;
+}
+__host__ __device__ __forceinline__ uint32_t anchor_candidate(uint2 anchor, uint32_t k, uint32_t k_last, uint32_t I, uint32_t n, uint32_t L)
+{
+    const bool left = k <= k_last - k;
+    uint32_t a = left ? anchor.x : anchor.y, ka = left ? 0u : k_last;
+    if (a == NO_ANCHOR) { a = left ? anchor.y : anchor.x; ka = left ? k_last : 0u; }
+    if (a == NO_ANCHOR) return NO_ANCHOR;
+    uint64_t p;
+    if (k < ka) {
+        const uint32_t d = I * (ka - k);
+        if (a < d) return NO_ANCHOR;
+        p = a - d;
+    } else {
+        p = (uint64_t)a + (uint64_t)I * (k - ka);
+    }
+    return (p + L <= n) ? (uint32_t)p : NO_ANCHOR;
+}
+__host__ __device__ __forceinline__ bool seed_on_unique_lmer(const FmIndex& f, const uint32_t* __restrict__ genome, const uint32_t* __restrict__ words,
+                                                             uint32_t off, uint32_t p)
+{
+    const uint32_t L = f.unique_len;
+#ifdef __CUDA_ARCH__
+    const uint32_t bitw = __ldg(f.unique + (p >> 5));
+#else
+    const uint32_t bitw = f.unique[p >> 5];
+#endif
+    bool same = true;
+    for (uint32_t i = 0; i < L; i += 16u) {
+        const uint32_t cnt = L - i < 16u ? L - i : 16u;
+        same &= ((be2_window(words, off + i, cnt) ^ be2_window(genome, p + i, cnt)) >> (32u - 2u * cnt)) == 0u;
+    }
+    return same && ((bitw >> (p & 31u)) & 1u);
+}
+template <int MODE>
+__host__ __device__ __forceinline__ uint32_t fm_match_locate_anchored(const FmIndex& f, const uint32_t* __restrict__ genome,
+                                                                      const uint32_t* __restrict__ words, uint32_t off, uint32_t p,
+                                                                      uint32_t& ox, uint32_t& oy, bool& claimed)
+{
+    claimed = p != NO_ANCHOR && seed_on_unique_lmer(f, genome, words, off, p);
+    if (claimed) { ox = p; oy = 0xFFFFFFFFu; return FM_LOCATED; }
+    return fm_match_locate_one<2, true, MODE>(f, genome, words, off, f.unique_len, ox, oy);
+}
+
 template <int BITS, bool BE>
 __host__ __device__ inline uint32_t fm_map_approx_one(const FmIndex& f, const uint32_t* __restrict__ words,
                                                       uint32_t off, uint32_t len2, uint32_t len1, uint32_t flags, bool find_exact,
diff --git a/nvbio_b200/csrc/fm_kernels.cu b/nvbio_b200/csrc/fm_kernels.cu
--- a/nvbio_b200/csrc/fm_kernels.cu
+++ b/nvbio_b200/csrc/fm_kernels.cu
@@ -151,6 +151,24 @@
     if (r >= n_rows) return;
     const uint32_t pos = sa[r];
     rows[r] = make_uint2(pos, text_before(text, pos, 16u));
+}
+
+__global__ void __launch_bounds__(FM_BLOCKDIM)
+fm_unique_init_kernel(uint32_t* __restrict__ bits, uint32_t n_words, uint32_t n, uint32_t L)
+{
+    const uint32_t w = blockIdx.x * FM_BLOCKDIM + threadIdx.x;
+    if (w < n_words) bits[w] = unique_init_word(w, n, L);
+}
+__global__ void __launch_bounds__(FM_BLOCKDIM)
+fm_unique_pairs_kernel(const uint32_t* __restrict__ sa, const uint32_t* __restrict__ text, uint32_t* __restrict__ bits, uint32_t n, uint32_t L)
+{
+    const uint32_t r = blockIdx.x * FM_BLOCKDIM + threadIdx.x;
+    if (r >= n) return;
+    const uint32_t a = sa[r], b = sa[r + 1u];
+    if (lmer_shared(text, n, a, b, L)) {
+        atomicAnd(bits + (a >> 5), ~(1u << (a & 31u)));
+        atomicAnd(bits + (b >> 5), ~(1u << (b & 31u)));
+    }
 }
 
 __global__ void __launch_bounds__(FM_BLOCKDIM)
@@ -376,6 +394,23 @@
     return NVB_OK;
 }
 
+int nvb_fm_build_unique(const nvb_fm_index* fmi, uint32_t L, const uint32_t* d_text, uint32_t* d_bits, void* stream)
+{
+    if (!fmi || !fmi->d_bwt_occ || L < 1u || L > 32u || !d_text || !d_bits || ((uintptr_t)d_bits & 3u)) return NVB_E_INVALID;
+    if (fmi->sa_interval != 1u || !fmi->d_ssa) return NVB_E_UNSUPPORTED;
+    const uint32_t n = fmi->length, n_words = (uint32_t)(((uint64_t)n + 31u) / 32u);
+    cudaStream_t s = as_stream(stream);
+    if (n_words) {
+        fm_unique_init_kernel<<<(n_words + FM_BLOCKDIM - 1) / FM_BLOCKDIM, FM_BLOCKDIM, 0, s>>>(d_bits, n_words, n, L);
+        NVB_LAUNCH_CHECK();
+    }
+    if (n) {
+        fm_unique_pairs_kernel<<<(uint32_t)(((uint64_t)n + FM_BLOCKDIM - 1) / FM_BLOCKDIM), FM_BLOCKDIM, 0, s>>>(fmi->d_ssa, d_text, d_bits, n, L);
+        NVB_LAUNCH_CHECK();
+    }
+    return NVB_OK;
+}
+
 int nvb_fm_rank(const nvb_fm_index* fmi, const uint32_t* d_k, const uint8_t* d_c, uint32_t n,
                 uint32_t* d_out, void* stream)
 {
diff --git a/nvbio_b200/csrc/pipeline.cu b/nvbio_b200/csrc/pipeline.cu
--- a/nvbio_b200/csrc/pipeline.cu
+++ b/nvbio_b200/csrc/pipeline.cu
@@ -132,7 +132,7 @@
 __global__ void __launch_bounds__(SEED_BLOCK, 2048 / SEED_BLOCK)
 pipe_seed_match_kernel(const FmIndex f, const PipeGeom g, const uint32_t* __restrict__ words, const uint32_t* __restrict__ slen,
                        const uint32_t* __restrict__ genome, uint2* __restrict__ ranges, uint32_t* __restrict__ sizes,
-                       uint32_t* __restrict__ todo, uint32_t* __restrict__ todo_count)
+                       uint32_t* __restrict__ todo, uint32_t* __restrict__ todo_count, const uint4* __restrict__ anchors)
 {
     constexpr uint32_t ITER = DEFER ? SEED_ITER : 1u;
 #pragma unroll 1
@@ -146,9 +146,22 @@
             const uint32_t s = q / g.seeds_per_string, k = q % g.seeds_per_string;
             const uint32_t len = slen[s];
             const uint32_t pos = k * g.seed_interval;
-            if (pos + g.seed_len <= len) {
+            const uint32_t k_last = last_anchor_seed(len, g.seed_len, g.seed_interval);
+            const bool anchored = BITS == 2 && DEFER && anchors;
+            uint4 a = make_uint4(1u, 0u, 1u, 0u);
+            if (anchored) a = anchors[s];
+            if (anchored && k == 0u) { x = a.x; y = a.y; }
+            else if (anchored && k == k_last) { x = a.z; y = a.w; }
+            else if (pos + g.seed_len <= len) {
                 if (genome) {
-                    const uint32_t st = fm_match_locate_one<BITS, true, DEFER ? FM_DEFER : FM_WHOLE>(f, genome, words, s * g.stride + pos, g.seed_len, x, y);
+                    uint32_t st;
+                    if (anchored) {
+                        bool claimed;
+                        const uint2 at = make_uint2(a.y == 0xFFFFFFFFu ? a.x : NO_ANCHOR, a.w == 0xFFFFFFFFu ? a.z : NO_ANCHOR);
+                        const uint32_t p = anchor_candidate(at, k, k_last, g.seed_interval, g.genome_len, g.seed_len);
+                        st = fm_match_locate_anchored<DEFER ? FM_DEFER : FM_WHOLE>(f, genome, words, s * g.stride + pos, p, x, y, claimed);
+                    } else
+                        st = fm_match_locate_one<BITS, true, DEFER ? FM_DEFER : FM_WHOLE>(f, genome, words, s * g.stride + pos, g.seed_len, x, y);
                     if (st == FM_EMPTY) { x = 1; y = 0; }
                     deferred = DEFER && st == FM_DEFERRED;
                 } else
@@ -170,6 +183,43 @@
         }
     }
 }
+__global__ void __launch_bounds__(SEED_BLOCK, 2048 / SEED_BLOCK)
+pipe_seed_anchor_kernel(const FmIndex f, const PipeGeom g, const uint32_t* __restrict__ words, const uint32_t* __restrict__ slen,
+                        const uint32_t* __restrict__ genome, uint2* __restrict__ anchors,
+                        uint32_t* __restrict__ todo, uint32_t* __restrict__ todo_count, const uint32_t seed_grid)
+{
+    const uint32_t t = blockIdx.x * SEED_BLOCK + threadIdx.x;
+    uint32_t q = 0;
+    bool deferred = false;
+    if (t < 2u * g.n_strings) {
+        const uint32_t s = t >> 1, j = t & 1u;
+        const uint32_t len = slen[s];
+        const uint32_t k_last = last_anchor_seed(len, g.seed_len, g.seed_interval);
+        const uint32_t k = j ? k_last : 0u;
+        q = s * g.seeds_per_string + k;
+        uint32_t x = 1, y = 0;
+        if ((j == 0u || k_last != 0u) && len >= g.seed_len) {
+            const uint32_t st = fm_match_locate_one<2, true, FM_DEFER>(f, genome, words, s * g.stride + k * g.seed_interval, g.seed_len, x, y);
+            if (st == FM_EMPTY) { x = 1; y = 0; }
+            deferred = st == FM_DEFERRED;
+        }
+        anchors[t] = make_uint2(x, y);
+    }
+    const uint32_t m = __ballot_sync(0xFFFFFFFFu, deferred);
+    if (m) {
+        const uint32_t list = (q / (SEED_BLOCK * SEED_ITER)) % SEED_TODO_LISTS;
+        const uint32_t same = __match_any_sync(0xFFFFFFFFu, deferred ? list : 0xFFFFFFFFu) & m;
+        if (deferred) {
+            const uint32_t lane = threadIdx.x & 31u, leader = __ffs(same) - 1u;
+            const uint32_t cap = ((seed_grid + SEED_TODO_LISTS - 1u) / SEED_TODO_LISTS) * SEED_BLOCK * SEED_ITER;
+            uint32_t base = 0;
+            if (lane == leader) base = atomicAdd(todo_count + list * SEED_TODO_PITCH, (uint32_t)__popc(same));
+            base = __shfl_sync(same, base, leader);
+            todo[(size_t)list * cap + base + __popc(same & ((1u << lane) - 1u))] = q;
+        }
+    }
+}
+
 template <int BITS>
 __global__ void __launch_bounds__(SEED_BLOCK, 2048 / SEED_BLOCK)
 pipe_seed_match_wide_kernel(const FmIndex f, const PipeGeom g, const uint32_t* __restrict__ words,
@@ -886,6 +936,8 @@
 static int g_perfect_shortcut = 1;
 static const uint32_t* g_last_dp_count = nullptr;
 static int g_seed_split = 1;
+static int g_seed_anchor = 1;
+static int g_seed_anchor_used = 0;
 static int g_pipe_path = 0;
 
 #define NVB_TRY(expr) do { const int _r = (expr); if (_r != NVB_OK) return _r; } while (0)
@@ -900,6 +952,7 @@
     uint32_t nq, hit_capacity;
     bool dedup, per_read, eligible;
     bool seed_split;
+    bool anchored;
     int32_t* best_score; uint32_t* best_pos; int32_t* hit_score; nvb_uint2* hit_sink;
     const nvb_best_alignment_out* BA; const nvb_pair_params* PP; const nvb_pair_out* PO;
     const nvb_mapq_params* MP; const nvb_mapq_out* MO; const nvb_pair_mapq_out* PMO;
@@ -907,6 +960,7 @@
     StageEvents* SE;
     uint32_t *str_words, *str_len; uint8_t* str_quals;
     uint2* ranges; uint32_t *sizes, *excl, *counts, *seed_todo, *seed_todo_n;
+    uint2* anchors;
     char* rj_tiles; size_t rj_tile_bytes;
     uint32_t *j_string, *j_first;
     uint32_t *leader, *flag, *job_idx;
@@ -953,6 +1007,7 @@
         if (!per_read) { sizes = tc.take<uint32_t>(nq); excl = tc.take<uint32_t>(nq); }
         if (seed_split) seed_todo = tc.take<uint32_t>((size_t)nq + (SEED_TODO_LISTS + 1u) * SEED_BLOCK * SEED_ITER);
         counts = tc.take<uint32_t>(4); seed_todo_n = tc.take<uint32_t>(SEED_TODO_LISTS * SEED_TODO_PITCH);
+        if (anchored) anchors = tc.take<uint2>(2ull * g.n_strings);
         if (per_read) {
             NVB_CUDA_TRY(RjTileState::AllocationSize((int)((n_reads + RJ_BLOCK - 1u) / RJ_BLOCK), rj_tile_bytes));
             rj_tiles = tc.take<char>(rj_tile_bytes);
@@ -1036,15 +1091,21 @@
         if (seed_split) {
             NVB_CUDA_TRY(cudaMemsetAsync(seed_todo_n, 0, SEED_TODO_LISTS * SEED_TODO_PITCH * sizeof(uint32_t), s));
             const uint32_t grid1 = (grid + SEED_ITER - 1u) / SEED_ITER;
-            if (g.bits == 2) pipe_seed_match_kernel<2, true><<<grid1, SEED_BLOCK, 0, s>>>(f, g, str_words, str_len, loc_genome, ranges, sizes, seed_todo, seed_todo_n);
-            else             pipe_seed_match_kernel<4, true><<<grid1, SEED_BLOCK, 0, s>>>(f, g, str_words, str_len, loc_genome, ranges, sizes, seed_todo, seed_todo_n);
+            if (anchored) {
+                pipe_seed_anchor_kernel<<<(2u * g.n_strings + SEED_BLOCK - 1u) / SEED_BLOCK, SEED_BLOCK, 0, s>>>(f, g, str_words, str_len, loc_genome, anchors,
+                                                                                                         seed_todo, seed_todo_n, grid1);
+                NVB_LAUNCH_CHECK();
+            }
+            if (g.bits == 2) pipe_seed_match_kernel<2, true><<<grid1, SEED_BLOCK, 0, s>>>(f, g, str_words, str_len, loc_genome, ranges, sizes, seed_todo, seed_todo_n,
+                                                                                          (const uint4*)anchors);
+            else             pipe_seed_match_kernel<4, true><<<grid1, SEED_BLOCK, 0, s>>>(f, g, str_words, str_len, loc_genome, ranges, sizes, seed_todo, seed_todo_n, nullptr);
             NVB_LAUNCH_CHECK();
             const uint32_t wgrid = (sm_count() * 16u + SEED_TODO_LISTS - 1u) / SEED_TODO_LISTS * SEED_TODO_LISTS;
             if (g.bits == 2) pipe_seed_match_wide_kernel<2><<<wgrid, SEED_BLOCK, 0, s>>>(f, g, str_words, loc_genome, ranges, sizes, seed_todo, seed_todo_n, grid1);
             else             pipe_seed_match_wide_kernel<4><<<wgrid, SEED_BLOCK, 0, s>>>(f, g, str_words, loc_genome, ranges, sizes, seed_todo, seed_todo_n, grid1);
         } else {
-            if (g.bits == 2) pipe_seed_match_kernel<2, false><<<grid, SEED_BLOCK, 0, s>>>(f, g, str_words, str_len, loc_genome, ranges, sizes, nullptr, nullptr);
-            else             pipe_seed_match_kernel<4, false><<<grid, SEED_BLOCK, 0, s>>>(f, g, str_words, str_len, loc_genome, ranges, sizes, nullptr, nullptr);
+            if (g.bits == 2) pipe_seed_match_kernel<2, false><<<grid, SEED_BLOCK, 0, s>>>(f, g, str_words, str_len, loc_genome, ranges, sizes, nullptr, nullptr, nullptr);
+            else             pipe_seed_match_kernel<4, false><<<grid, SEED_BLOCK, 0, s>>>(f, g, str_words, str_len, loc_genome, ranges, sizes, nullptr, nullptr, nullptr);
         }
         return launched();
     }
@@ -1306,10 +1367,12 @@
     c.eligible = c.per_read && P->type == NVB_LOCAL && g.bits == 2 && P->band_len <= 32 && !SC.d_qual_table && SC.match > 0 && SC.mismatch < 0 &&
                  SC.pattern_gap_open < 0 && SC.pattern_gap_ext <= 0 && SC.text_gap_open < 0 && SC.text_gap_ext <= 0;
     c.seed_split = c.per_read && c.f.sa_shift == 0u && c.f.ktab_k && g.seed_len > c.f.ktab_k && g_seed_split;
+    c.anchored = c.seed_split && g_seed_anchor && g.bits == 2 && d_genome && c.f.unique && c.f.unique_len == g.seed_len;
     size_t need = 0;
     NVB_TRY(c.carve(d_temp, need));
     if (!d_temp || *temp_bytes < need) { *temp_bytes = need; return NVB_E_TEMP_SIZE; }
     if (n_reads == 0) return NVB_OK;
+    g_seed_anchor_used = c.anchored ? 1 : 0;
 
     NVB_TRY(default_stage_events(&c.SE));
     NVB_TRY(c.stage(0));
@@ -1342,6 +1405,8 @@
 
 extern "C" void nvb_debug_pipeline_path(int path) { g_pipe_path = path; }
 extern "C" void nvb_debug_seed_split(int on) { g_seed_split = on; }
+extern "C" void nvb_debug_seed_anchor(int on) { g_seed_anchor = on; }
+extern "C" int nvb_debug_seed_anchor_used(void) { return g_seed_anchor_used; }
 extern "C" void nvb_debug_perfect_shortcut(int on) { g_perfect_shortcut = on; }
 extern "C" int nvb_debug_dp_jobs(uint32_t* n)
 {
diff --git a/nvbio_b200/fmindex.py b/nvbio_b200/fmindex.py
--- a/nvbio_b200/fmindex.py
+++ b/nvbio_b200/fmindex.py
@@ -37,6 +37,7 @@
         self.ktab_located = 0
         self.ktab_wide = False
         self.rows = None
+        self.unique, self.unique_len = None, 0
 
     def struct(self) -> FmIndexStruct:
         s = FmIndexStruct()
@@ -53,6 +54,8 @@
             s.ktab_located = 4
         if s.ktab_located in (2, 4) and self.rows is not None:
             s.ktab_located, s.d_rows = s.ktab_located + 1, self.rows.data_ptr()
+        if s.ktab_located == 5 and self.unique is not None:
+            s.ktab_located, s.d_unique, s.unique_len = 6, self.unique.data_ptr(), self.unique_len
         return s
 
     @property
@@ -61,7 +64,25 @@
 
     def nbytes(self):
         return (self.bwt_occ.numel() * 4 + (self.ssa.numel() * 4 if self.ssa is not None else 0) +
-                (self.ktab.numel() * 4 if self.ktab is not None else 0) + (self.rows.numel() * 4 if self.rows is not None else 0))
+                (self.ktab.numel() * 4 if self.ktab is not None else 0) + (self.rows.numel() * 4 if self.rows is not None else 0) +
+                (self.unique.numel() * 4 if self.unique is not None else 0))
+
+    def build_unique(self, L: int, text: torch.Tensor):
+        if self.unique is not None and self.unique_len == L:
+            return self
+        self.unique, self.unique_len = None, 0
+        if self.sa_interval != 1 or self.ssa is None or not 1 <= L <= 32:
+            return self
+        words = (self.length + 31) // 32
+        free, _ = torch.cuda.mem_get_info(self.device)
+        if words * 4 + ROWS_HEADROOM > free:
+            return self
+        assert text.is_cuda and text.dtype == torch.int32
+        bits = torch.empty(max(words, 1), dtype=torch.int32, device=self.device)
+        check(lib().nvb_fm_build_unique(C.byref(self.struct()), C.c_uint32(L), C.c_void_p(text.data_ptr()), C.c_void_p(bits.data_ptr()), _stream()),
+              "nvb_fm_build_unique")
+        self.unique, self.unique_len = bits, int(L)
+        return self
 
     def build_ktab(self, k: int = 12, located: bool = False, text: Optional[torch.Tensor] = None):
         self.ktab = None
diff --git a/nvbio_b200/pipeline.py b/nvbio_b200/pipeline.py
--- a/nvbio_b200/pipeline.py
+++ b/nvbio_b200/pipeline.py
@@ -90,11 +90,17 @@
         return p
 
 
+def _anchor_setup(fmi: FMIndexDevice, genome: Optional[torch.Tensor], params: SeedExtendParams, bits: int):
+    if fmi.sa_interval == 1 and fmi.ssa is not None and fmi.ktab_wide and fmi.rows is not None and genome is not None and bits == 2:
+        fmi.build_unique(params.seed_len, genome)
+
+
 class SeedExtendWorkspace:
 
     def __init__(self, fmi: FMIndexDevice, genome: torch.Tensor, reads: PackedStringSet, params: SeedExtendParams,
                  hit_capacity: int, keep_hits: bool = False, traceback: bool = False, mapq: Optional[MapqParams] = None):
         dev = fmi.device
+        _anchor_setup(fmi, genome, params, reads.bits)
         n = reads.count
         self.best_score = torch.empty(n, dtype=torch.int32, device=dev)
         self.best_pos = torch.empty(n, dtype=torch.int32, device=dev)
@@ -199,6 +205,7 @@
                  mapq: Optional[MapqParams] = None, traceback: bool = False, max_ops: Optional[int] = None):
         dev = fmi.device
         assert reads.count % 2 == 0
+        _anchor_setup(fmi, genome, params, reads.bits)
         self.n_pairs = n = reads.count // 2
         self.hit_capacity = hit_capacity
         self.pair_score = torch.empty(n, dtype=torch.int32, device=dev)
@@ -302,6 +309,7 @@
         if hit_capacity is None:
             hit_capacity = 32 * n_reads + 1024
         self._params_struct = params.struct()
+        _anchor_setup(fmi, genome, params, bits)
         s = fmi.struct()
         pp = pair.struct(n_reads // 2) if pair is not None else None
         self._h = C.c_void_p()
```

New measurement: 440.6 (median of 6 runs). 10.3% higher.
